# curioloop/rafting

Hardware: AMD Instinct MI355X
Metric: raft-group decisions/sec (AppendEntries+vote) (higher is better)
Workload: dtype int64

## Files before the change

include/raftgpu.h:

```cpp
#ifndef RAFTGPU_H
#define RAFTGPU_H

#include <stdint.h>
#include <stddef.h>

#ifdef __cplusplus
extern "C" {
#endif

#define RG_ABI_VERSION      6
#define RG_MIN_CLUSTER      2
#define RG_MAX_CLUSTER      15
#define RG_MAX_COMPACT_CLUSTER 7
#define RG_TERM_RUNS        4
#define RG_NO_NODE          (-1)

enum { RG_FOLLOWER = 0, RG_CANDIDATE = 1, RG_LEADER = 2 };

enum {
    RG_EV_NONE          = 0,
    RG_EV_AE_REQ        = 1,
    RG_EV_AE_ACK        = 2,
    RG_EV_IS_ACK        = 3,
    RG_EV_RV_REQ        = 4,
    RG_EV_PV_REQ        = 5,
    RG_EV_RV_REPLY      = 6,
    RG_EV_PV_REPLY      = 7,
    RG_EV_TIMEOUT       = 8,
    RG_EV_CLIENT_APPEND = 9,
    RG_EV_LOG_FLUSH     = 10,
    RG_EV_IS_REQ        = 11
};
#define RG_EV_IS_REQ_DEFINED 1

#define RG_HDR_KIND(h)        ((uint32_t)(h) & 0xFu)
#define RG_HDR_SLOT(h)        (((uint32_t)(h) >> 4) & 0xFu)
#define RG_HDR_FLAG(h)        (((uint32_t)(h) >> 8) & 0x1u)
#define RG_HDR_HINT(h)        (((uint32_t)(h) >> 9) & 0x1u)
#define RG_HDR_N(h)           ((uint32_t)(h) >> 12)
#define RG_HDR_MAKE(kind, slot, flag, n) \
    (((uint32_t)(kind) & 0xFu) | (((uint32_t)(slot) & 0xFu) << 4) | (((uint32_t)(flag) & 1u) << 8) | ((uint32_t)(n) << 12))
#define RG_HDR_HINT_BIT       (1u << 9)
#define RG_HDR_SAME_TERM      (1u << 10)
#define RG_MAX_ENTRIES        ((1u << 20) - 1)
#define RG_MAX_AE_ENTRIES     200u

typedef struct { uint32_t hdr; uint32_t aux; } rg_ev_head_t;
typedef struct { int64_t  x;   int64_t  y;   } rg_ev_pair_t;

typedef struct {
    int64_t  resp_term;
    uint32_t flags;
    uint32_t role_epoch;
} rg_reply_t;

typedef struct {
    int64_t commit_index;
    int64_t log_from;
} rg_logfx_t;

typedef struct {
    int64_t term;
    int32_t voted_for;
    int32_t role;
} rg_persist_t;

#define RG_F_SUCCESS      (1u << 0)
#define RG_F_REPLIED      (1u << 1)
#define RG_F_PERSIST      (1u << 2)
#define RG_F_ROLE_CHANGED (1u << 3)
#define RG_F_RESET_TIMER  (1u << 4)
#define RG_F_COMMIT       (1u << 5)
#define RG_F_LOG_TRUNC    (1u << 6)
#define RG_F_LOG_APPEND   (1u << 7)
#define RG_F_EMIT_SHIFT   8
#define RG_F_EMIT_MASK    (3u << 8)
#define RG_EMIT_NONE      0u
#define RG_EMIT_PREVOTE   1u
#define RG_EMIT_REQVOTE   2u
#define RG_EMIT_HEARTBEAT 3u
#define RG_F_ROLE_SHIFT   10
#define RG_F_ROLE_MASK    (3u << 10)
#define RG_F_TIMER_MUTED  (1u << 12)
#define RG_F_WIDE_VALUES  (1u << 13)
#define RG_F_STATUS_SHIFT 16
#define RG_F_STATUS(f)    (((f) >> RG_F_STATUS_SHIFT) & 0xFFu)
#define RG_F_EMIT(f)      (((f) & RG_F_EMIT_MASK) >> RG_F_EMIT_SHIFT)
#define RG_F_ROLE(f)      (((f) & RG_F_ROLE_MASK) >> RG_F_ROLE_SHIFT)

enum {
    RG_OK                       = 0,
    RG_A_TWO_LEADERS            = 1,
    RG_A_PREV_ZERO_MISMATCH     = 2,
    RG_A_EPOCH_TERM_MISMATCH    = 3,
    RG_A_IMPOSSIBLE_LOG         = 4,
    RG_A_COMMIT_ROLLBACK        = 5,
    RG_A_LOG_NOT_CONTINUOUS     = 6,
    RG_A_LEADER_SELF_AE         = 7,
    RG_A_SAME_TERM_LEADER       = 8,
    RG_A_LEADER_NOT_SELF_VOTE   = 9,
    RG_A_CAND_SELF_RV           = 10,
    RG_A_CAND_NOT_SELF_VOTE     = 11,
    RG_A_LEADER_UNCHANGED       = 12,
    RG_A_CAND_BALLOT            = 13,
    RG_A_MATCH_ROLLBACK         = 14,
    RG_A_IMPOSSIBLE_REPLICATION = 15,
    RG_NPE_MAJOR_NULL           = 16,
    RG_DROPPED_STALE_ROLE       = 17,
    RG_NOT_LEADER               = 18,
    RG_FLUSH_OUT_OF_BOUNDS      = 19,
    RG_A_INSTALL_BEFORE_AE      = 20,
    RG_A_NO_DOWNGRADE           = 21,
    RG_NEED_HOST                = 32,
    RG_SKIPPED_AFTER_NEED_HOST  = 33,
    RG_BAD_EVENT                = 34,
    RG_UNSUPPORTED_LOG_STATE    = 35
};

enum { RG_MEM_HOST = 0, RG_MEM_DEVICE = 1 };

typedef struct {
    uint32_t            rounds;
    uint32_t            count;
    const uint32_t     *gid;
    const rg_ev_head_t *head;
    const rg_ev_pair_t *ab;
    const rg_ev_pair_t *cd;
    const int64_t      *entry_terms;
    uint64_t            entry_count;
    const rg_ev_pair_t *hint;
} rg_batch_t;

typedef struct {
    rg_reply_t   *reply;
    rg_logfx_t   *logfx;
    rg_persist_t *persist;
} rg_outcome_t;

typedef struct {
    int64_t  *current_term;
    int32_t  *voted_for;
    int32_t  *role;
    int32_t  *current_leader;
    uint8_t  *timeout_detected;
    uint8_t  *repl_prepared;
    uint32_t *role_epoch;
    int32_t  *votes;
    uint32_t *elected_epoch;
    int64_t  *elected_term;
    int64_t  *commit_index;
    int64_t  *epoch_index;
    int64_t  *epoch_term;
    int64_t  *first_index;
    int64_t  *last_index;
    uint32_t *run_count;
    uint32_t *run_offset;
    int64_t  *run_start;
    int64_t  *run_term;
    int64_t  *peer_last_epoch;
    int64_t  *peer_next_index;
    int64_t  *peer_match_index;
    int32_t  *peer_rejection;
    uint8_t  *peer_pending;
} rg_group_state_t;

typedef struct rg_table rg_table_t;

int         rg_abi_version(void);
int         rg_table_create(int device, uint32_t groups, uint32_t cluster, uint32_t self_slot,
                            int pre_vote, rg_table_t **out);
int         rg_table_destroy(rg_table_t *t);
const char *rg_last_error(const rg_table_t *t);
enum { RG_OPT_REQUIRE_FENCED_TIMEOUTS = 1,
       RG_OPT_AUTO_INDEX_BASE = 2,
       RG_OPT_COMPACT_ANY_CLUSTER = 3,
       RG_OPT_DEVICE_IN_FLIGHT = 4 };
int         rg_table_option(rg_table_t *t, int option, int value);
uint32_t    rg_table_groups(const rg_table_t *t);
uint32_t    rg_table_cluster(const rg_table_t *t);

int rg_load_state(rg_table_t *t, uint32_t first, uint32_t count, const rg_group_state_t *src);
int rg_read_state(rg_table_t *t, uint32_t first, uint32_t count, rg_group_state_t *dst);

int rg_submit(rg_table_t *t, const rg_batch_t *in, const rg_outcome_t *out, int memspace);
int rg_sync(rg_table_t *t);

#define RG_PIPELINE_DEPTH 2
int rg_submit_async(rg_table_t *t, const rg_batch_t *in, const rg_outcome_t *out);
int rg_submit_wait(rg_table_t *t);

typedef struct { int32_t a, b, c, d; } rg_ev_quad32_t;
typedef struct {
    uint32_t              rounds, count;
    const uint32_t       *gid;
    const rg_ev_head_t   *head;
    const rg_ev_quad32_t *abcd;
    const int32_t        *entry_terms;
    uint64_t              entry_count;
} rg_batch32_t;
typedef struct {
    rg_reply_t   *reply;
    rg_logfx_t   *logfx;
    rg_persist_t *persist;
    uint32_t     *counts;
    uint32_t      logfx_cap, persist_cap;
} rg_outcome_packed_t;
int rg_submit_async_packed(rg_table_t *t, const rg_batch32_t *in, const rg_outcome_packed_t *out);

typedef struct rg_tick rg_tick_t;
int rg_tick_create(rg_table_t *t, const rg_batch32_t *in, const rg_outcome_packed_t *out, rg_tick_t **tick);
int rg_tick_launch(rg_tick_t *tick);
int rg_tick_wait(rg_tick_t *tick);
int rg_tick_destroy(rg_tick_t *tick);

int rg_submit32(rg_table_t *t, const rg_batch32_t *in, const rg_outcome_t *out, int memspace);
int64_t rg_batch32_pack(const rg_batch_t *in, rg_ev_head_t *head, rg_ev_quad32_t *abcd, int32_t *entry_terms);

int rg_index_base_set(rg_table_t *t, uint32_t first, uint32_t count, const int64_t *base);
int rg_index_base_get(rg_table_t *t, uint32_t first, uint32_t count, int64_t *base);
int rg_index_base_advance(const rg_batch_t *in, int32_t window, uint32_t groups, int64_t *index_base);
int rg_index_base_advance32(const rg_batch32_t *in, int32_t window, uint32_t groups, int64_t *index_base);
int64_t rg_batch32_pack_rel(const rg_batch_t *in, const int64_t *index_base, rg_ev_head_t *head, rg_ev_quad32_t *abcd, int32_t *entry_terms);
typedef struct { int32_t resp_term; uint32_t flags; int32_t commit_index; int32_t log_from; } rg_out32_t;
typedef struct { int32_t term; int32_t voted_for; uint32_t role_epoch; int32_t role; } rg_persist32_t;
typedef struct {
    rg_out32_t     *row;
    rg_persist32_t *persist;
    rg_outcome_t    wide;
} rg_outcome32_t;
int rg_submit32c(rg_table_t *t, const rg_batch32_t *in, const rg_outcome32_t *out, int memspace);
int rg_submit32c_sparse(rg_table_t *t, const rg_batch32_t *in, const rg_outcome32_t *out, int memspace);
int rg_submit32c_sparse_rounds(rg_table_t *t, const rg_batch32_t *in, const rg_outcome32_t *out, int memspace);
int rg_outcome32_unpack(const rg_outcome32_t *in, uint32_t rounds, uint32_t count, uint32_t *role_epoch, const rg_outcome_t *out);
int rg_outcome32_unpack_rel(const rg_outcome32_t *in, uint32_t rounds, uint32_t count, uint32_t *role_epoch, const int64_t *index_base, const rg_outcome_t *out);
const char *rg_step_kernel(rg_table_t *t, uint32_t count);

enum {
    RG_SEND_NONE      = 0,
    RG_SEND_APPEND    = 1,
    RG_SEND_SNAPSHOT  = 2,
    RG_SEND_GATED     = 3,
    RG_SEND_NEED_HOST = 4
};
#define RG_REPLICATE_LIMIT 50
#define RG_IN_FLIGHT_LIMIT 20

typedef struct {
    int64_t  term;
    int64_t  leader_commit;
    int64_t  epoch_index;
    int64_t  epoch_term;
    uint32_t role_epoch;
    uint32_t is_leader;
    uint64_t reserved;
} rg_send_head_t;

#define RG_SENT_TRIGGERED  1u
#define RG_SENT_HEARTBEAT  2u

typedef struct {
    int64_t  prev_index;
    int64_t  prev_term;
    int64_t  last_index;
    uint32_t count;
    uint32_t kind;
} rg_send_t;

int rg_replicate(rg_table_t *t, uint32_t count, const uint32_t *gid, const uint8_t *heartbeat, const uint16_t *in_flight,
                 rg_send_head_t *head, rg_send_t *send, int memspace);

int rg_timers_configure(rg_table_t *t, int64_t election_ms, int64_t heartbeat_ms, uint64_t seed);
int rg_timers_update(rg_table_t *t, uint32_t rounds, uint32_t count, const uint32_t *gid, const rg_reply_t *reply,
                     const int64_t *now, int memspace);
int rg_timers_expired(rg_table_t *t, int64_t now, uint32_t *out_gid, uint32_t capacity, uint32_t *out_count, int memspace);
int rg_timers_expired_epochs(rg_table_t *t, int64_t now, uint32_t *out_gid, uint32_t *out_epoch, uint32_t capacity, uint32_t *out_count,
                             int memspace);
int rg_timers_update32(rg_table_t *t, uint32_t rounds, const rg_out32_t *row, const rg_persist32_t *persist32, const int64_t *now, int memspace);
int rg_timers_arm(rg_table_t *t, int64_t now);
int rg_timers_read(rg_table_t *t, uint32_t first, uint32_t count, int64_t *deadline);

int rg_health_update(rg_table_t *t, uint32_t rounds, uint32_t count, const uint32_t *gid, const rg_ev_head_t *head,
                     const rg_reply_t *reply, const int64_t *now, int memspace);
int rg_health_update32(rg_table_t *t, uint32_t rounds, const rg_ev_head_t *head, const rg_out32_t *row, const int64_t *now, int memspace);
#define RG_HEALTH_NO_REQUEST 4u
int rg_health_failure(rg_table_t *t, uint32_t n, const uint32_t *gid, const uint8_t *slot, const uint8_t *flags, int64_t now);
int rg_ready(rg_table_t *t, int64_t now, int32_t critical_point, int64_t cool_down_ms, uint8_t *ready, int memspace);
int rg_health_read(rg_table_t *t, uint32_t first, uint32_t count, int64_t *request_success, int64_t *request_failure,
                   int32_t *recent_failure);
int rg_in_flight_read(rg_table_t *t, uint32_t first, uint32_t count, uint16_t *in_flight);
int rg_in_flight_set(rg_table_t *t, uint32_t first, uint32_t count, const uint16_t *in_flight);

typedef struct {
    uint32_t              rounds;
    const rg_ev_head_t   *head;
    const rg_ev_quad32_t *abcd;
    const int32_t        *entry_terms;
    uint64_t              entry_capacity;
    const int64_t        *now;
    const uint8_t        *heartbeat;
    const uint16_t       *in_flight;
    int32_t               critical_point;
    int64_t               cool_down_ms;
    rg_out32_t           *row;
    rg_persist32_t       *persist32;
    uint32_t             *expired_gid;
    uint32_t             *expired_epoch;
    uint32_t             *expired_count;
    uint32_t              expired_capacity;
    rg_send_head_t       *send_head;
    rg_send_t            *send;
    uint8_t              *ready;
} rg_tick2_io_t;
typedef struct rg_tick2 rg_tick2_t;
int rg_tick2_create(rg_table_t *t, const rg_tick2_io_t *io, rg_tick2_t **tick);
typedef struct {
    const uint32_t *gid;
    const uint32_t *count;
    uint32_t        capacity;
} rg_tick2_rows_t;
int rg_tick2_create_sparse(rg_table_t *t, const rg_tick2_io_t *io, const rg_tick2_rows_t *rows, rg_tick2_t **tick);
typedef struct {
    const uint32_t *gid;
    const uint32_t *count;
    const uint32_t *rounds;
    uint32_t        capacity;
} rg_tick2_rounds_t;
int rg_tick2_create_sparse_rounds(rg_table_t *t, const rg_tick2_io_t *io, const rg_tick2_rounds_t *rows, rg_tick2_t **tick);
int rg_tick2_launch(rg_tick2_t *tick);
int rg_tick2_wait(rg_tick2_t *tick);
int rg_tick2_destroy(rg_tick2_t *tick);

typedef struct {
    const uint32_t       *count;
    uint32_t              capacity;
    const uint32_t       *gid;
    const rg_ev_head_t   *head;
    const rg_ev_quad32_t *abcd;
    const uint32_t       *expired_gid, *expired_epoch, *expired_count;
    uint32_t              expired_capacity;
} rg_arrivals_t;
typedef struct {
    uint32_t        capacity;
    uint32_t        max_rounds;
    uint32_t       *gid, *count, *rounds;
    rg_ev_head_t   *head;
    rg_ev_quad32_t *abcd;
    uint32_t       *origin;
    uint32_t       *deferred;
    uint32_t        deferred_capacity;
    uint32_t       *stats;
} rg_assembled_t;
typedef struct rg_assembler rg_assembler_t;
int rg_assembler_create(rg_table_t *t, uint32_t max_events, uint32_t max_expired, rg_assembler_t **a);
int rg_assemble32(rg_assembler_t *a, const rg_arrivals_t *in, const rg_assembled_t *out, int memspace);
int rg_assembler_destroy(rg_assembler_t *a);

int rg_host_alloc(rg_table_t *t, size_t bytes, void **hptr);
int rg_host_free(rg_table_t *t, void *hptr);
int rg_dev_alloc(rg_table_t *t, size_t bytes, void **dptr);
int rg_dev_free(rg_table_t *t, void *dptr);
int rg_copy_to_device(rg_table_t *t, void *dst, const void *src, size_t bytes);
int rg_copy_to_host(rg_table_t *t, void *dst, const void *src, size_t bytes);
void *rg_stream(rg_table_t *t);

int rg_timing_enable(rg_table_t *t, int on);
int rg_timing_read(rg_table_t *t, uint64_t *launches, double *total_ms, int reset);
int rg_timing_begin(rg_table_t *t);
int rg_timing_end(rg_table_t *t, double *elapsed_ms);
#define RG_NUM_COUNTERS 8
int rg_counters_read(rg_table_t *t, uint64_t counters[RG_NUM_COUNTERS], int reset);
int rg_wide_body_workgroups(rg_table_t *t, uint64_t *count, int reset);
int rg_copy_bandwidth(rg_table_t *t, size_t bytes, int iters, double *gbps);

#ifdef __cplusplus
}
#endif
#endif
```

rafting_amd/abi.py:

```python
import ctypes as C

import numpy as np

ABI_VERSION = 6
MIN_CLUSTER, MAX_CLUSTER, MAX_COMPACT_CLUSTER = 2, 15, 7
TERM_RUNS = 4
NO_NODE = -1

FOLLOWER, CANDIDATE, LEADER = 0, 1, 2

EV_NONE, EV_AE_REQ, EV_AE_ACK, EV_IS_ACK, EV_RV_REQ, EV_PV_REQ = 0, 1, 2, 3, 4, 5
EV_RV_REPLY, EV_PV_REPLY, EV_TIMEOUT, EV_CLIENT_APPEND, EV_LOG_FLUSH, EV_IS_REQ = 6, 7, 8, 9, 10, 11
MAX_AE_ENTRIES = 200
PIPELINE_DEPTH = 2
HDR_HINT_BIT = 1 << 9
HDR_SAME_TERM = 1 << 10

F_SUCCESS, F_REPLIED, F_PERSIST, F_ROLE_CHANGED = 1 << 0, 1 << 1, 1 << 2, 1 << 3
F_RESET_TIMER, F_COMMIT, F_LOG_TRUNC, F_LOG_APPEND = 1 << 4, 1 << 5, 1 << 6, 1 << 7
F_EMIT_SHIFT, F_EMIT_MASK = 8, 3 << 8
EMIT_NONE, EMIT_PREVOTE, EMIT_REQVOTE, EMIT_HEARTBEAT = 0, 1, 2, 3
F_ROLE_SHIFT, F_ROLE_MASK = 10, 3 << 10
F_TIMER_MUTED = 1 << 12
F_WIDE_VALUES = 1 << 13
F_STATUS_SHIFT = 16

OK = 0
A_TWO_LEADERS, A_PREV_ZERO_MISMATCH, A_EPOCH_TERM_MISMATCH, A_IMPOSSIBLE_LOG = 1, 2, 3, 4
A_COMMIT_ROLLBACK, A_LOG_NOT_CONTINUOUS, A_LEADER_SELF_AE, A_SAME_TERM_LEADER = 5, 6, 7, 8
A_LEADER_NOT_SELF_VOTE, A_CAND_SELF_RV, A_CAND_NOT_SELF_VOTE, A_LEADER_UNCHANGED = 9, 10, 11, 12
A_CAND_BALLOT, A_MATCH_ROLLBACK, A_IMPOSSIBLE_REPLICATION, NPE_MAJOR_NULL = 13, 14, 15, 16
DROPPED_STALE_ROLE, NOT_LEADER, FLUSH_OUT_OF_BOUNDS = 17, 18, 19
A_INSTALL_BEFORE_AE, A_NO_DOWNGRADE = 20, 21
NEED_HOST, SKIPPED_AFTER_NEED_HOST, BAD_EVENT, UNSUPPORTED_LOG_STATE = 32, 33, 34, 35

MEM_HOST, MEM_DEVICE = 0, 1
OPT_REQUIRE_FENCED_TIMEOUTS = 1
OPT_AUTO_INDEX_BASE = 2
OPT_COMPACT_ANY_CLUSTER = 3
OPT_DEVICE_IN_FLIGHT = 4
SENT_TRIGGERED, SENT_HEARTBEAT = 1, 2
HEALTH_UNREACHABLE, HEALTH_REJECT, HEALTH_NO_REQUEST = 1, 2, 4
NUM_COUNTERS = 8

HEAD_DT = np.dtype([("hdr", "<u4"), ("aux", "<u4")])
PAIR_DT = np.dtype([("x", "<i8"), ("y", "<i8")])
REPLY_DT = np.dtype([("resp_term", "<i8"), ("flags", "<u4"), ("role_epoch", "<u4")])
LOGFX_DT = np.dtype([("commit_index", "<i8"), ("log_from", "<i8")])
PERSIST_DT = np.dtype([("term", "<i8"), ("voted_for", "<i4"), ("role", "<i4")])
SEND_HEAD_DT = np.dtype([("term", "<i8"), ("leader_commit", "<i8"), ("epoch_index", "<i8"), ("epoch_term", "<i8"),
                         ("role_epoch", "<u4"), ("is_leader", "<u4"), ("reserved", "<u8")])
SEND_DT = np.dtype([("prev_index", "<i8"), ("prev_term", "<i8"), ("last_index", "<i8"), ("count", "<u4"), ("kind", "<u4")])
SEND_NONE, SEND_APPEND, SEND_SNAPSHOT, SEND_GATED, SEND_NEED_HOST = 0, 1, 2, 3, 4
REPLICATE_LIMIT, IN_FLIGHT_LIMIT = 50, 20
assert SEND_HEAD_DT.itemsize == 48 and SEND_DT.itemsize == 32
assert HEAD_DT.itemsize == 8 and PAIR_DT.itemsize == 16 and REPLY_DT.itemsize == 16
assert LOGFX_DT.itemsize == 16 and PERSIST_DT.itemsize == 16


def hdr_make(kind, slot=0, flag=0, n=0):
    return (
        (np.uint32(kind) & np.uint32(0xF))
        | ((np.asarray(slot).astype(np.uint32) & np.uint32(0xF)) << np.uint32(4))
        | ((np.asarray(flag).astype(np.uint32) & np.uint32(1)) << np.uint32(8))
        | (np.asarray(n).astype(np.uint32) << np.uint32(12))
    ).astype(np.uint32)


def flags_status(flags):
    return (np.asarray(flags) >> F_STATUS_SHIFT) & 0xFF


def flags_role(flags):
    return (np.asarray(flags) & F_ROLE_MASK) >> F_ROLE_SHIFT


def flags_emit(flags):
    return (np.asarray(flags) & F_EMIT_MASK) >> F_EMIT_SHIFT


class CBatch(C.Structure):
    _fields_ = [
        ("rounds", C.c_uint32),
        ("count", C.c_uint32),
        ("gid", C.c_void_p),
        ("head", C.c_void_p),
        ("ab", C.c_void_p),
        ("cd", C.c_void_p),
        ("entry_terms", C.c_void_p),
        ("entry_count", C.c_uint64),
        ("hint", C.c_void_p),
    ]


class COutcome(C.Structure):
    _fields_ = [("reply", C.c_void_p), ("logfx", C.c_void_p), ("persist", C.c_void_p)]


class CBatch32(C.Structure):
    _fields_ = [("rounds", C.c_uint32), ("count", C.c_uint32), ("gid", C.c_void_p), ("head", C.c_void_p), ("abcd", C.c_void_p),
                ("entry_terms", C.c_void_p), ("entry_count", C.c_uint64)]


class COutcome32(C.Structure):
    _fields_ = [("row", C.c_void_p), ("persist", C.c_void_p), ("wide", COutcome)]


class COutcomePacked(C.Structure):
    _fields_ = [("reply", C.c_void_p), ("logfx", C.c_void_p), ("persist", C.c_void_p), ("counts", C.c_void_p),
                ("logfx_cap", C.c_uint32), ("persist_cap", C.c_uint32)]


class CTick2Io(C.Structure):
    _fields_ = [("rounds", C.c_uint32), ("head", C.c_void_p), ("abcd", C.c_void_p), ("entry_terms", C.c_void_p), ("entry_capacity", C.c_uint64),
                ("now", C.c_void_p), ("heartbeat", C.c_void_p), ("in_flight", C.c_void_p), ("critical_point", C.c_int32), ("cool_down_ms", C.c_int64),
                ("row", C.c_void_p), ("persist32", C.c_void_p), ("expired_gid", C.c_void_p), ("expired_epoch", C.c_void_p), ("expired_count", C.c_void_p),
                ("expired_capacity", C.c_uint32), ("send_head", C.c_void_p), ("send", C.c_void_p), ("ready", C.c_void_p)]


class CTick2Rows(C.Structure):
    _fields_ = [("gid", C.c_void_p), ("count", C.c_void_p), ("capacity", C.c_uint32)]


class CTick2Rounds(C.Structure):
    _fields_ = [("gid", C.c_void_p), ("count", C.c_void_p), ("rounds", C.c_void_p), ("capacity", C.c_uint32)]


class CArrivals(C.Structure):
    _fields_ = [("count", C.c_void_p), ("capacity", C.c_uint32), ("gid", C.c_void_p), ("head", C.c_void_p), ("abcd", C.c_void_p),
                ("expired_gid", C.c_void_p), ("expired_epoch", C.c_void_p), ("expired_count", C.c_void_p), ("expired_capacity", C.c_uint32)]


class CAssembled(C.Structure):
    _fields_ = [("capacity", C.c_uint32), ("max_rounds", C.c_uint32), ("gid", C.c_void_p), ("count", C.c_void_p), ("rounds", C.c_void_p),
                ("head", C.c_void_p), ("abcd", C.c_void_p), ("origin", C.c_void_p), ("deferred", C.c_void_p), ("deferred_capacity", C.c_uint32),
                ("stats", C.c_void_p)]


ORIGIN_NONE, ORIGIN_EXPIRED = 0xFFFFFFFF, 0x80000000
EXPIRED_UNTRUSTED = 0xFFFFFFFF


_STATE_FIELDS = [
    ("current_term", np.int64, 1),
    ("voted_for", np.int32, 1),
    ("role", np.int32, 1),
    ("current_leader", np.int32, 1),
    ("timeout_detected", np.uint8, 1),
    ("repl_prepared", np.uint8, 1),
    ("role_epoch", np.uint32, 1),
    ("votes", np.int32, 1),
    ("elected_epoch", np.uint32, 1),
    ("elected_term", np.int64, 1),
    ("commit_index", np.int64, 1),
    ("epoch_index", np.int64, 1),
    ("epoch_term", np.int64, 1),
    ("first_index", np.int64, 1),
    ("last_index", np.int64, 1),
    ("run_count", np.uint32, 1),
    ("run_offset", np.uint32, 1),
    ("run_start", np.int64, "runs"),
    ("run_term", np.int64, "runs"),
    ("peer_last_epoch", np.int64, "peers"),
    ("peer_next_index", np.int64, "peers"),
    ("peer_match_index", np.int64, "peers"),
    ("peer_rejection", np.int32, "peers"),
    ("peer_pending", np.uint8, "peers"),
]


class CGroupState(C.Structure):
    _fields_ = [(name, C.c_void_p) for name, _, _ in _STATE_FIELDS]


def _ptr(a):
    return None if a is None else a.ctypes.data


class GroupState:

    def __init__(self, count, cluster, runs_total=None):
        self.count, self.cluster, self.followers = count, cluster, cluster - 1
        nruns = count * TERM_RUNS if runs_total is None else runs_total
        for name, dt, shape in _STATE_FIELDS:
            n = count if shape == 1 else (nruns if shape == "runs" else count * self.followers)
            setattr(self, name, np.zeros(n, dtype=dt))
        self.voted_for[:] = NO_NODE
        self.current_leader[:] = NO_NODE
        self.role_epoch[:] = 1
        self.votes[:] = 1
        self.run_offset[:] = np.arange(count, dtype=np.uint32) * TERM_RUNS if runs_total is None else 0

    def set_log(self, g, first, runs, last):
# ... 157 lines not shown
```

rafting_amd/csrc/raftgpu.cpp:

```cpp
#include <hip/hip_runtime.h>

#include <algorithm>
#include <cstdarg>
#include <cstdint>
#include <cstdio>
#include <cstdlib>
#include <cstring>
#include <string>
#include <unordered_map>
#include <vector>

#include "rg_device.hpp"
#include "rg_assemble.hpp"

using rg::DevTable;
using rg::I64x2;

struct Staging {
    void *ptr = nullptr;
    size_t cap = 0;
};

struct PipeSlot {
    Staging gid, head, ab, cd, hint, terms, reply, logfx, persist;
    Staging abcd32, terms32, counts;
    hipEvent_t up = nullptr, done = nullptr, down = nullptr;
};

struct rg_table {
    int device = 0;
    uint32_t G = 0, P = 0, self = 0, F = 0;
    int pre_vote = 0;
    hipStream_t stream = nullptr;
    DevTable dt{};
    unsigned long long *counters = nullptr;
    unsigned long long *wide_bodies = nullptr;
    size_t counter_slots = 0;
    int fast_paths = 1;
    int force_wide = 0;
    int require_fence = 0;
    int has_bases = 0;
    int auto_window = 0;
    int compact_any_cluster = 0;
    Staging st_abcd32, st_terms32, st_out32, st_persist32;
    int lanes = -1;
    uint32_t simds = 1024;
    Staging st_gid, st_head, st_ab, st_cd, st_hint, st_terms, st_reply, st_logfx, st_persist, st_hb, st_fl, st_sh, st_ss;
    bool timing = false;
    std::vector<std::pair<hipEvent_t, hipEvent_t>> ev_pool;
    size_t ev_used = 0;
    uint64_t t_launches = 0;
    double t_total_ms = 0.0;
    hipEvent_t region0 = nullptr, region1 = nullptr;
    int64_t *timer_deadline = nullptr;
    uint32_t *timer_epoch = nullptr;
    unsigned long long *tick_masks = nullptr;
    uint32_t *tick_ticket = nullptr;
    uint64_t config_gen = 0;
    std::vector<struct rg_tick *> ticks;
    std::vector<struct rg_tick2 *> ticks2;
    std::vector<struct rg_assembler *> assemblers;
    uint32_t *timer_counts = nullptr;
    int64_t election_ms = 900, heartbeat_ms = 300;
    uint64_t timer_seed = 0;
    Staging st_tgid, st_hgid, st_hslot, st_hflag, st_ready;
    int64_t *health_ok = nullptr, *health_fail = nullptr;
    int32_t *health_recent = nullptr;
    uint16_t *in_flight = nullptr;
    Staging st_hdone;
    hipStream_t s_in = nullptr, s_out = nullptr;
    PipeSlot pipe[RG_PIPELINE_DEPTH];
    uint64_t pipe_head = 0, pipe_tail = 0;
    std::string err;
};

static thread_local std::string g_create_err;

static int fail(rg_table *t, int code, const char *fmt, ...)
{
    char buf[512];
    va_list ap;
    va_start(ap, fmt);
    vsnprintf(buf, sizeof buf, fmt, ap);
    va_end(ap);
    if (t) t->err = buf; else g_create_err = buf;
    return code;
}

#define HIP_TRY(t, expr)                                                                              \
    do {                                                                                              \
        hipError_t e_ = (expr);                                                                       \
        if (e_ != hipSuccess) return fail((t), -2, "%s failed: %s", #expr, hipGetErrorString(e_));    \
    } while (0)

static int wait_oldest(rg_table *t)
{
    if (t->pipe_tail == t->pipe_head) return 1;
    HIP_TRY(t, hipEventSynchronize(t->pipe[t->pipe_tail % RG_PIPELINE_DEPTH].down));
    t->pipe_tail += 1;
    return 0;
}

static int bind(rg_table *t, bool drain = true)
{
    HIP_TRY(t, hipSetDevice(t->device));
    while (drain && t->pipe_tail != t->pipe_head)
        if (int rc = wait_oldest(t); rc < 0) return rc;
    return 0;
}

static int reserve(rg_table *t, Staging &s, size_t bytes)
{
    if (bytes <= s.cap) return 0;
    if (s.ptr) HIP_TRY(t, hipFree(s.ptr));
    s.ptr = nullptr; s.cap = 0;
    size_t cap = bytes + bytes / 4 + 4096;
    HIP_TRY(t, hipMalloc(&s.ptr, cap));
    s.cap = cap;
    return 0;
}

static int drain_timing(rg_table *t)
{
    if (t->ev_used == 0) return 0;
    HIP_TRY(t, hipStreamSynchronize(t->stream));
    for (size_t i = 0; i < t->ev_used; i++) {
        float ms = 0.f;
        HIP_TRY(t, hipEventElapsedTime(&ms, t->ev_pool[i].first, t->ev_pool[i].second));
        t->t_total_ms += ms;
        t->t_launches += 1;
    }
    t->ev_used = 0;
    return 0;
}

extern "C" {

int rg_abi_version(void) { return RG_ABI_VERSION; }

const char *rg_last_error(const rg_table_t *t) { return t ? t->err.c_str() : g_create_err.c_str(); }
uint32_t rg_table_groups(const rg_table_t *t) { return t ? t->G : 0; }
uint32_t rg_table_cluster(const rg_table_t *t) { return t ? t->P : 0; }

int rg_table_option(rg_table_t *t, int option, int value)
{
    if (!t) return -1;
    switch (option) {
    case RG_OPT_REQUIRE_FENCED_TIMEOUTS:
        if (t->require_fence != (value != 0)) t->config_gen += 1;
        t->require_fence = value != 0;
        return 0;
    case RG_OPT_AUTO_INDEX_BASE:
        if (value < 0 || value >= (1 << 30)) return fail(t, -1, "rg_table_option: RG_OPT_AUTO_INDEX_BASE window %d outside [0, 2^30)", value);
        if (t->auto_window != value) t->config_gen += 1;
        if (value != 0 && !t->has_bases) t->has_bases = 1;
        t->auto_window = value;
        return 0;
    case RG_OPT_COMPACT_ANY_CLUSTER:
        if (value != 0 && value != 1) return fail(t, -1, "rg_table_option: RG_OPT_COMPACT_ANY_CLUSTER takes 0 or 1 (%d given)", value);
        if (t->compact_any_cluster != value) t->config_gen += 1;
        t->compact_any_cluster = value;
        return 0;
    case RG_OPT_DEVICE_IN_FLIGHT: {
        if (value != 0 && value != 1) return fail(t, -1, "rg_table_option: RG_OPT_DEVICE_IN_FLIGHT takes 0 or 1 (%d given)", value);
        if ((t->in_flight != nullptr) == (value == 1)) return 0;
        if (bind(t)) return -2;
        HIP_TRY(t, hipStreamSynchronize(t->stream));
        if (value == 1) {
            const size_t bytes = (size_t)t->G * t->F * sizeof(uint16_t);
            uint16_t *c = nullptr;
            HIP_TRY(t, hipMalloc((void **)&c, bytes));
            if (hipError_t e = hipMemsetAsync(c, 0, bytes, t->stream); e != hipSuccess || (e = hipStreamSynchronize(t->stream)) != hipSuccess) {
                (void)hipFree(c);
                return fail(t, -2, "rg_table_option: RG_OPT_DEVICE_IN_FLIGHT: %s", hipGetErrorString(e));
            }
            t->in_flight = c;
        } else {
            HIP_TRY(t, hipFree(t->in_flight));
            t->in_flight = nullptr;
        }
        t->config_gen += 1;
        return 0;
    }
    default: return fail(t, -1, "rg_table_option: unknown option %d", option);
    }
}

static void tick_release(struct rg_tick *k);
static void tick2_release(struct rg_tick2 *k);
static void assembler_release(struct rg_assembler *a);

int rg_table_destroy(rg_table_t *t)
{
    if (!t) return 0;
    (void)hipSetDevice(t->device);
    if (t->stream) (void)hipStreamSynchronize(t->stream);
    for (struct rg_tick *k : t->ticks) tick_release(k);
    for (struct rg_tick2 *k : t->ticks2) tick2_release(k);
    for (struct rg_assembler *a : t->assemblers) assembler_release(a);
    t->ticks.clear(); t->ticks2.clear(); t->assemblers.clear();
    void *cols[] = {t->dt.term_commit, t->dt.epoch, t->dt.window, t->dt.ident, t->dt.elect, t->dt.runs,
                    t->dt.peer_en, t->dt.peer_m, t->dt.ibase, t->wide_bodies, t->counters, t->st_gid.ptr, t->st_head.ptr, t->st_ab.ptr,
                    t->st_cd.ptr, t->st_hint.ptr, t->st_terms.ptr, t->st_reply.ptr, t->st_logfx.ptr,
                    t->st_persist.ptr, t->st_hb.ptr, t->st_fl.ptr, t->st_sh.ptr, t->st_ss.ptr, t->timer_deadline, t->timer_epoch, t->tick_masks, t->tick_ticket,
                    t->timer_counts, t->st_tgid.ptr, t->st_hgid.ptr, t->st_hslot.ptr, t->st_hflag.ptr, t->st_ready.ptr, t->health_ok,
                    t->health_fail, t->health_recent, t->in_flight, t->st_hdone.ptr, t->st_abcd32.ptr, t->st_terms32.ptr, t->st_out32.ptr, t->st_persist32.ptr};
    for (void *c : cols) if (c) (void)hipFree(c);
    for (PipeSlot &sl : t->pipe) {
        if (sl.down) (void)hipEventSynchronize(sl.down);
        for (Staging *st : {&sl.gid, &sl.head, &sl.ab, &sl.cd, &sl.hint, &sl.terms, &sl.reply, &sl.logfx, &sl.persist, &sl.abcd32, &sl.terms32, &sl.counts})
            if (st->ptr) (void)hipFree(st->ptr);
        for (hipEvent_t ev : {sl.up, sl.done, sl.down}) if (ev) (void)hipEventDestroy(ev);
    }
    if (t->s_in) (void)hipStreamDestroy(t->s_in);
    if (t->s_out) (void)hipStreamDestroy(t->s_out);
    for (auto &e : t->ev_pool) { (void)hipEventDestroy(e.first); (void)hipEventDestroy(e.second); }
    if (t->region0) { (void)hipEventDestroy(t->region0); (void)hipEventDestroy(t->region1); }
    if (t->stream) (void)hipStreamDestroy(t->stream);
    delete t;
    return 0;
}

int rg_table_create(int device, uint32_t groups, uint32_t cluster, uint32_t self_slot, int pre_vote, rg_table_t **out)
{
    if (!out) return fail(nullptr, -1, "rg_table_create: out is NULL");
    *out = nullptr;
    if (groups == 0) return fail(nullptr, -1, "rg_table_create: groups must be > 0");
    if (cluster < RG_MIN_CLUSTER || cluster > RG_MAX_CLUSTER)
        return fail(nullptr, -1, "rg_table_create: cluster size %u outside [%d, %d]", cluster, RG_MIN_CLUSTER, RG_MAX_CLUSTER);
    if (self_slot >= cluster) return fail(nullptr, -1, "rg_table_create: self_slot %u >= cluster %u", self_slot, cluster);
    int ndev = 0;
    hipError_t e = hipGetDeviceCount(&ndev);
    if (e != hipSuccess || ndev == 0)
        return fail(nullptr, -2, "rg_table_create: no HIP device (%s) — libraftgpu has no CPU path", hipGetErrorString(e));
    if (device < 0 || device >= ndev) return fail(nullptr, -1, "rg_table_create: device %d of %d", device, ndev);

    rg_table *t = new rg_table();
    t->device = device; t->G = groups; t->P = cluster; t->self = self_slot; t->F = cluster - 1;
    t->pre_vote = pre_vote != 0;
#define CREATE_TRY(expr)                                                                   \
    do {                                                                                   \
        hipError_t e2_ = (expr);                                                           \
        if (e2_ != hipSuccess) {                                                           \
            fail(nullptr, -2, "%s failed: %s", #expr, hipGetErrorString(e2_));             \
            rg_table_destroy(t);                                                           \
            return -2;                                                                     \
        }                                                                                  \
    } while (0)
    CREATE_TRY(hipSetDevice(device));
    CREATE_TRY(hipStreamCreateWithFlags(&t->stream, hipStreamNonBlocking));
    const size_t G = groups, F = t->F;
    CREATE_TRY(hipMalloc((void **)&t->dt.term_commit, G * sizeof(I64x2)));
    CREATE_TRY(hipMalloc((void **)&t->dt.epoch, G * sizeof(I64x2)));
    CREATE_TRY(hipMalloc((void **)&t->dt.window, G * sizeof(I64x2)));
    CREATE_TRY(hipMalloc((void **)&t->dt.ident, G * sizeof(rg::Ident)));
    CREATE_TRY(hipMalloc((void **)&t->dt.elect, G * sizeof(rg::Elect)));
    CREATE_TRY(hipMalloc((void **)&t->dt.runs, G * rg::K * sizeof(I64x2)));
    CREATE_TRY(hipMalloc((void **)&t->dt.peer_en, G * F * sizeof(I64x2)));
    CREATE_TRY(hipMalloc((void **)&t->dt.peer_m, G * F * sizeof(rg::Match)));
    CREATE_TRY(hipMalloc((void **)&t->dt.ibase, G * sizeof(int64_t)));
    CREATE_TRY(hipMalloc((void **)&t->wide_bodies, sizeof(unsigned long long)));
    CREATE_TRY(hipMemsetAsync(t->wide_bodies, 0, sizeof(unsigned long long), t->stream));
    {
        hipDeviceProp_t prop;
        CREATE_TRY(hipGetDeviceProperties(&prop, device));
        t->simds = (uint32_t)prop.multiProcessorCount * 4u;
    }
    t->lanes = -1;
    if (const char *e = getenv("RG_SPLIT")) t->lanes = atoi(e) != 0 ? 0 : 64;
    if (const char *e = getenv("RG_FAST")) t->fast_paths = atoi(e) != 0;
    if (const char *e = getenv("RG_FORCE_WIDE")) t->force_wide = atoi(e) != 0;
    t->counter_slots = (G + 63) / 64 + 1;
    CREATE_TRY(hipMalloc((void **)&t->counters, t->counter_slots * RG_NUM_COUNTERS * sizeof(unsigned long long)));
    t->dt.groups = groups;
    CREATE_TRY(hipMalloc((void **)&t->timer_deadline, G * sizeof(int64_t)));
    CREATE_TRY(hipMalloc((void **)&t->timer_counts, ((G + 255) / 256 * 4 + 1) * sizeof(uint32_t)));
    CREATE_TRY(hipMemsetAsync(t->timer_deadline, 0, G * sizeof(int64_t), t->stream));
    CREATE_TRY(hipMalloc((void **)&t->tick_masks, ((G + 255) / 256 * 4) * sizeof(unsigned long long)));
    CREATE_TRY(hipMemsetAsync(t->tick_masks, 0, ((G + 255) / 256 * 4) * sizeof(unsigned long long), t->stream));
    CREATE_TRY(hipMalloc((void **)&t->tick_ticket, sizeof(uint32_t)));
    CREATE_TRY(hipMemsetAsync(t->tick_ticket, 0, sizeof(uint32_t), t->stream));
    CREATE_TRY(hipMalloc((void **)&t->timer_epoch, G * sizeof(uint32_t)));
    CREATE_TRY(hipMemsetAsync(t->timer_epoch, 0, G * sizeof(uint32_t), t->stream));
    CREATE_TRY(hipMalloc((void **)&t->health_ok, G * F * sizeof(int64_t)));
    CREATE_TRY(hipMalloc((void **)&t->health_fail, G * F * sizeof(int64_t)));
    CREATE_TRY(hipMalloc((void **)&t->health_recent, G * F * sizeof(int32_t)));
    CREATE_TRY(hipMemsetAsync(t->health_ok, 0, G * F * sizeof(int64_t), t->stream));
    CREATE_TRY(hipMemsetAsync(t->health_fail, 0, G * F * sizeof(int64_t), t->stream));
    CREATE_TRY(hipMemsetAsync(t->health_recent, 0, G * F * sizeof(int32_t), t->stream));
    CREATE_TRY(hipMemsetAsync(t->dt.term_commit, 0, G * sizeof(I64x2), t->stream));
    CREATE_TRY(hipMemsetAsync(t->dt.epoch, 0, G * sizeof(I64x2), t->stream));
    CREATE_TRY(hipMemsetAsync(t->dt.window, 0, G * sizeof(I64x2), t->stream));
    CREATE_TRY(hipMemsetAsync(t->dt.runs, 0, G * rg::K * sizeof(I64x2), t->stream));
    CREATE_TRY(hipMemsetAsync(t->dt.peer_en, 0, G * F * sizeof(I64x2), t->stream));
    CREATE_TRY(hipMemsetAsync(t->dt.peer_m, 0, G * F * sizeof(rg::Match), t->stream));
    CREATE_TRY(hipMemsetAsync(t->dt.ibase, 0, G * sizeof(int64_t), t->stream));
    CREATE_TRY(hipMemsetAsync(t->counters, 0, t->counter_slots * RG_NUM_COUNTERS * sizeof(unsigned long long), t->stream));
    {
        std::vector<rg::Ident> id(G, rg::Ident{RG_NO_NODE, RG_NO_NODE, 1u, 0u});
        std::vector<rg::Elect> el(G, rg::Elect{0, 0u, 1});
        CREATE_TRY(hipMemcpyAsync(t->dt.ident, id.data(), G * sizeof(rg::Ident), hipMemcpyHostToDevice, t->stream));
        CREATE_TRY(hipMemcpyAsync(t->dt.elect, el.data(), G * sizeof(rg::Elect), hipMemcpyHostToDevice, t->stream));
        CREATE_TRY(hipStreamSynchronize(t->stream));
    }
#undef CREATE_TRY
    *out = t;
    return 0;
}


static int step_lanes(const rg_table *t, uint32_t count)
{
    if (t->lanes >= 0) return t->lanes;
    const uint32_t wavefronts = (count + 63u) / 64u;
    return wavefronts <= t->simds ? 0 : 64;
}

static bool state_complete(const rg_group_state_t *s)
{
    return s->current_term && s->voted_for && s->role && s->current_leader && s->timeout_detected && s->repl_prepared &&
           s->role_epoch && s->votes && s->elected_epoch && s->elected_term && s->commit_index && s->epoch_index &&
           s->epoch_term && s->first_index && s->last_index && s->run_count && s->run_offset && s->run_start && s->run_term &&
           s->peer_last_epoch && s->peer_next_index && s->peer_match_index && s->peer_rejection && s->peer_pending;
}

int rg_load_state(rg_table_t *t, uint32_t first, uint32_t count, const rg_group_state_t *s)
{
    if (!t) return -1;
    if (!s || !state_complete(s)) return fail(t, -1, "rg_load_state: src or one of its columns is NULL");
    if ((uint64_t)first + count > t->G) return fail(t, -1, "rg_load_state: range [%u, %u) exceeds %u groups", first, first + count, t->G);
    if (count == 0) return 0;
    if (bind(t)) return -2;
    const size_t n = count, F = t->F, G = t->G;
    std::vector<I64x2> tc(n), ep(n), win(n), runs(n * rg::K), en(n * F);
    std::vector<rg::Ident> id(n);
    std::vector<rg::Elect> el(n);
    std::vector<rg::Match> pm(n * F);
    for (size_t i = 0; i < n; i++) {
        const int32_t role = s->role[i];
        if (role < RG_FOLLOWER || role > RG_LEADER) return fail(t, -1, "rg_load_state: group %zu role %d", first + i, role);
        if (s->voted_for[i] < RG_NO_NODE || s->voted_for[i] >= (int32_t)t->P || s->current_leader[i] < RG_NO_NODE ||
            s->current_leader[i] >= (int32_t)t->P)
            return fail(t, -1, "rg_load_state: group %zu node slot out of range", first + i);
        const uint32_t total = s->run_count[i], off = s->run_offset[i];
        const uint32_t rc = total > (uint32_t)rg::K ? (uint32_t)rg::K : total;
        int64_t fi = 0, la = 0;
        if (total) {
            fi = s->first_index[i]; la = s->last_index[i];
            if (s->run_start[off] != fi || la < s->run_start[off + total - 1])
                return fail(t, -1, "rg_load_state: group %zu runs do not span [first,last]", first + i);
            if (fi != s->epoch_index[i] && fi != s->epoch_index[i] + 1)
                return fail(t, -1, "rg_load_state: group %zu first index %lld is neither epoch.index nor epoch.index+1",
                            first + i, (long long)fi);
            for (uint32_t k = 1; k < total; k++)
                if (s->run_start[off + k] <= s->run_start[off + k - 1] || s->run_term[off + k] == s->run_term[off + k - 1])
                    return fail(t, -1, "rg_load_state: group %zu runs are not maximal ascending runs", first + i);
        }
        tc[i] = I64x2{s->current_term[i], s->commit_index[i]};
        ep[i] = I64x2{s->epoch_index[i], s->epoch_term[i]};
        win[i] = I64x2{fi, la};
        uint32_t pend = 0;
        for (size_t j = 0; j < F; j++) {
            en[j * n + i] = I64x2{s->peer_last_epoch[i * F + j], s->peer_next_index[i * F + j]};
            pm[j * n + i] = rg::Match{s->peer_match_index[i * F + j], s->peer_rejection[i * F + j], 0};
            if (s->peer_pending[i * F + j]) pend |= 1u << j;
        }
        for (uint32_t k = 0; k < (uint32_t)rg::K; k++) {
            const bool have = k < rc;
            runs[(size_t)k * n + i] = have ? I64x2{s->run_start[off + total - rc + k], s->run_term[off + total - rc + k]} : I64x2{0, 0};
        }
        const uint32_t meta = (uint32_t)role | (s->timeout_detected[i] ? rg::META_TD : 0u) |
                              (s->repl_prepared[i] ? rg::META_PREP : 0u) | (rc << rg::META_RC_SHIFT) |
                              (pend << rg::META_PEND_SHIFT);
        id[i] = rg::Ident{s->voted_for[i], s->current_leader[i], s->role_epoch[i], meta};
        el[i] = rg::Elect{s->elected_term[i], s->elected_epoch[i], s->votes[i]};
    }
    hipStream_t st = t->stream;
    HIP_TRY(t, hipMemcpyAsync(t->dt.term_commit + first, tc.data(), n * sizeof(I64x2), hipMemcpyHostToDevice, st));
    HIP_TRY(t, hipMemcpyAsync(t->dt.epoch + first, ep.data(), n * sizeof(I64x2), hipMemcpyHostToDevice, st));
    HIP_TRY(t, hipMemcpyAsync(t->dt.window + first, win.data(), n * sizeof(I64x2), hipMemcpyHostToDevice, st));
    HIP_TRY(t, hipMemcpyAsync(t->dt.ident + first, id.data(), n * sizeof(rg::Ident), hipMemcpyHostToDevice, st));
    HIP_TRY(t, hipMemcpyAsync(t->dt.elect + first, el.data(), n * sizeof(rg::Elect), hipMemcpyHostToDevice, st));
    for (size_t k = 0; k < (size_t)rg::K; k++)
        HIP_TRY(t, hipMemcpyAsync(t->dt.runs + k * G + first, runs.data() + k * n, n * sizeof(I64x2), hipMemcpyHostToDevice, st));
    for (size_t j = 0; j < F; j++) {
        HIP_TRY(t, hipMemcpyAsync(t->dt.peer_en + j * G + first, en.data() + j * n, n * sizeof(I64x2), hipMemcpyHostToDevice, st));
        HIP_TRY(t, hipMemcpyAsync(t->dt.peer_m + j * G + first, pm.data() + j * n, n * sizeof(rg::Match), hipMemcpyHostToDevice, st));
    }
    HIP_TRY(t, hipMemsetAsync(t->timer_deadline + first, 0, n * sizeof(int64_t), st));
    HIP_TRY(t, hipMemcpyAsync(t->timer_epoch + first, s->role_epoch, n * sizeof(uint32_t), hipMemcpyHostToDevice, st));
    for (size_t j = 0; j < F; j++) {
        HIP_TRY(t, hipMemsetAsync(t->health_ok + j * G + first, 0, n * sizeof(int64_t), st));
        HIP_TRY(t, hipMemsetAsync(t->health_fail + j * G + first, 0, n * sizeof(int64_t), st));
        HIP_TRY(t, hipMemsetAsync(t->health_recent + j * G + first, 0, n * sizeof(int32_t), st));
        if (t->in_flight) HIP_TRY(t, hipMemsetAsync(t->in_flight + j * G + first, 0, n * sizeof(uint16_t), st));
    }
    HIP_TRY(t, hipStreamSynchronize(st));
    return 0;
}

int rg_read_state(rg_table_t *t, uint32_t first, uint32_t count, rg_group_state_t *d)
{
    if (!t) return -1;
    if (!d || !state_complete(d)) return fail(t, -1, "rg_read_state: dst or one of its columns is NULL");
    if ((uint64_t)first + count > t->G) return fail(t, -1, "rg_read_state: range exceeds %u groups", t->G);
    if (count == 0) return 0;
    if (bind(t)) return -2;
    const size_t n = count, F = t->F, G = t->G;
    std::vector<I64x2> tc(n), ep(n), win(n), runs(n * rg::K), en(n * F);
    std::vector<rg::Ident> id(n);
    std::vector<rg::Elect> el(n);
    std::vector<rg::Match> pm(n * F);
    hipStream_t st = t->stream;
    HIP_TRY(t, hipMemcpyAsync(tc.data(), t->dt.term_commit + first, n * sizeof(I64x2), hipMemcpyDeviceToHost, st));
    HIP_TRY(t, hipMemcpyAsync(ep.data(), t->dt.epoch + first, n * sizeof(I64x2), hipMemcpyDeviceToHost, st));
    HIP_TRY(t, hipMemcpyAsync(win.data(), t->dt.window + first, n * sizeof(I64x2), hipMemcpyDeviceToHost, st));
    HIP_TRY(t, hipMemcpyAsync(id.data(), t->dt.ident + first, n * sizeof(rg::Ident), hipMemcpyDeviceToHost, st));
    HIP_TRY(t, hipMemcpyAsync(el.data(), t->dt.elect + first, n * sizeof(rg::Elect), hipMemcpyDeviceToHost, st));
    for (size_t k = 0; k < (size_t)rg::K; k++)
        HIP_TRY(t, hipMemcpyAsync(runs.data() + k * n, t->dt.runs + k * G + first, n * sizeof(I64x2), hipMemcpyDeviceToHost, st));
    for (size_t j = 0; j < F; j++) {
        HIP_TRY(t, hipMemcpyAsync(en.data() + j * n, t->dt.peer_en + j * G + first, n * sizeof(I64x2), hipMemcpyDeviceToHost, st));
        HIP_TRY(t, hipMemcpyAsync(pm.data() + j * n, t->dt.peer_m + j * G + first, n * sizeof(rg::Match), hipMemcpyDeviceToHost, st));
    }
    HIP_TRY(t, hipStreamSynchronize(st));
    for (size_t i = 0; i < n; i++) {
        const uint32_t meta = id[i].meta;
        const uint32_t rc = (meta >> rg::META_RC_SHIFT) & 7u;
        d->current_term[i] = tc[i].x; d->commit_index[i] = tc[i].y;
        d->epoch_index[i] = ep[i].x; d->epoch_term[i] = ep[i].y;
        d->first_index[i] = rc ? win[i].x : 0; d->last_index[i] = rc ? win[i].y : 0;
        d->voted_for[i] = id[i].voted_for; d->current_leader[i] = id[i].leader; d->role_epoch[i] = id[i].role_epoch;
        d->role[i] = (int32_t)(meta & rg::META_ROLE);
        d->timeout_detected[i] = (meta & rg::META_TD) ? 1 : 0;
        d->repl_prepared[i] = (meta & rg::META_PREP) ? 1 : 0;
        d->elected_term[i] = el[i].elected_term; d->elected_epoch[i] = el[i].elected_epoch; d->votes[i] = el[i].votes;
        d->run_count[i] = rc;
        d->run_offset[i] = (uint32_t)(i * rg::K);
        for (uint32_t k = 0; k < (uint32_t)rg::K; k++) {
            d->run_start[i * rg::K + k] = k < rc ? runs[(size_t)k * n + i].x : 0;
            d->run_term[i * rg::K + k] = k < rc ? runs[(size_t)k * n + i].y : 0;
        }
        const uint32_t pend = (meta >> rg::META_PEND_SHIFT) & rg::META_PEND_MASK;
        for (size_t j = 0; j < F; j++) {
            d->peer_last_epoch[i * F + j] = en[j * n + i].x;
            d->peer_next_index[i * F + j] = en[j * n + i].y;
            d->peer_match_index[i * F + j] = pm[j * n + i].match_index;
            d->peer_rejection[i * F + j] = pm[j * n + i].rejection;
            d->peer_pending[i * F + j] = (pend >> j) & 1u;
        }
// ... 749 lines not shown
    p.reply = (rg_reply_t *)t->st_reply.ptr; p.logfx = (I64x2 *)t->st_logfx.ptr; p.persist = (rg_persist_t *)t->st_persist.ptr;
    HIP_TRY(t, hipMemsetAsync(t->st_logfx.ptr, 0, rows * sizeof(I64x2), s));
    HIP_TRY(t, hipMemsetAsync(t->st_persist.ptr, 0, rows * sizeof(rg_persist_t), s));
    if (int rc = launch(t, p, sparse)) return rc;
    HIP_TRY(t, hipMemcpyAsync(out->reply, t->st_reply.ptr, rows * sizeof(rg_reply_t), hipMemcpyDeviceToHost, s));
    HIP_TRY(t, hipMemcpyAsync(out->logfx, t->st_logfx.ptr, rows * sizeof(I64x2), hipMemcpyDeviceToHost, s));
    HIP_TRY(t, hipMemcpyAsync(out->persist, t->st_persist.ptr, rows * sizeof(rg_persist_t), hipMemcpyDeviceToHost, s));
    HIP_TRY(t, hipStreamSynchronize(s));
    return 0;
}

int rg_submit32(rg_table_t *t, const rg_batch32_t *in, const rg_outcome_t *out, int memspace)
{
    if (!t) return -1;
    if (int rc = compact_ok(t, "rg_submit32")) return rc;
    if (!in || !out) return fail(t, -1, "rg_submit32: NULL batch or outcome");
    if (!in->head || !in->abcd) return fail(t, -1, "rg_submit32: head and abcd are required");
    rg_batch_t wide{};
    wide.rounds = in->rounds; wide.count = in->count; wide.gid = in->gid; wide.head = in->head;
    wide.ab = wide.cd = reinterpret_cast<const rg_ev_pair_t *>(in->abcd);
    wide.entry_terms = reinterpret_cast<const int64_t *>(in->entry_terms); wide.entry_count = in->entry_count;
    if (int rc = check_batch(t, &wide, out, memspace == RG_MEM_HOST)) return rc;
    if (in->count == 0) return 0;
    if (bind(t)) return -2;
    const bool sparse = in->gid != nullptr;
    const size_t rows = (size_t)in->rounds * in->count;
    rg::StepParams p = step_params(t, &wide);
    if (memspace == RG_MEM_DEVICE) {
        p.gid = in->gid; p.head = in->head; p.abcd32 = (const rg::I32x4 *)in->abcd;
        p.entry_terms32 = in->entry_count ? in->entry_terms : nullptr;
        p.reply = out->reply; p.logfx = (I64x2 *)out->logfx; p.persist = out->persist;
        return launch(t, p, sparse);
    }
    if (memspace != RG_MEM_HOST) return fail(t, -1, "rg_submit32: unknown memspace %d", memspace);
    hipStream_t s = t->stream;
    if (reserve(t, t->st_head, rows * sizeof(rg_ev_head_t)) || reserve(t, t->st_abcd32, rows * sizeof(rg_ev_quad32_t)) ||
        reserve(t, t->st_reply, rows * sizeof(rg_reply_t)) || reserve(t, t->st_logfx, rows * sizeof(I64x2)) ||
        reserve(t, t->st_persist, rows * sizeof(rg_persist_t)))
        return -2;
    HIP_TRY(t, hipMemcpyAsync(t->st_head.ptr, in->head, rows * sizeof(rg_ev_head_t), hipMemcpyHostToDevice, s));
    HIP_TRY(t, hipMemcpyAsync(t->st_abcd32.ptr, in->abcd, rows * sizeof(rg_ev_quad32_t), hipMemcpyHostToDevice, s));
    p.head = (const rg_ev_head_t *)t->st_head.ptr; p.abcd32 = (const rg::I32x4 *)t->st_abcd32.ptr;
    if (sparse) {
        if (reserve(t, t->st_gid, in->count * sizeof(uint32_t))) return -2;
        HIP_TRY(t, hipMemcpyAsync(t->st_gid.ptr, in->gid, in->count * sizeof(uint32_t), hipMemcpyHostToDevice, s));
        p.gid = (const uint32_t *)t->st_gid.ptr;
    }
    if (in->entry_count) {
        if (reserve(t, t->st_terms32, in->entry_count * sizeof(int32_t))) return -2;
        HIP_TRY(t, hipMemcpyAsync(t->st_terms32.ptr, in->entry_terms, in->entry_count * sizeof(int32_t), hipMemcpyHostToDevice, s));
        p.entry_terms32 = (const int32_t *)t->st_terms32.ptr;
    }
    p.reply = (rg_reply_t *)t->st_reply.ptr; p.logfx = (I64x2 *)t->st_logfx.ptr; p.persist = (rg_persist_t *)t->st_persist.ptr;
    HIP_TRY(t, hipMemsetAsync(t->st_logfx.ptr, 0, rows * sizeof(I64x2), s));
    HIP_TRY(t, hipMemsetAsync(t->st_persist.ptr, 0, rows * sizeof(rg_persist_t), s));
    if (int rc = launch(t, p, sparse)) return rc;
    HIP_TRY(t, hipMemcpyAsync(out->reply, t->st_reply.ptr, rows * sizeof(rg_reply_t), hipMemcpyDeviceToHost, s));
    HIP_TRY(t, hipMemcpyAsync(out->logfx, t->st_logfx.ptr, rows * sizeof(I64x2), hipMemcpyDeviceToHost, s));
    HIP_TRY(t, hipMemcpyAsync(out->persist, t->st_persist.ptr, rows * sizeof(rg_persist_t), hipMemcpyDeviceToHost, s));
    HIP_TRY(t, hipStreamSynchronize(s));
    return 0;
}

int rg_wide_body_workgroups(rg_table_t *t, uint64_t *count, int reset)
{
    if (!t || !count) return -1;
    if (bind(t)) return -2;
    unsigned long long v = 0;
    HIP_TRY(t, hipMemcpyAsync(&v, t->wide_bodies, sizeof v, hipMemcpyDeviceToHost, t->stream));
    if (reset) HIP_TRY(t, hipMemsetAsync(t->wide_bodies, 0, sizeof v, t->stream));
    HIP_TRY(t, hipStreamSynchronize(t->stream));
    *count = v;
    return 0;
}

int rg_index_base_set(rg_table_t *t, uint32_t first, uint32_t count, const int64_t *base)
{
    if (!t) return -1;
    if (!base) return fail(t, -1, "rg_index_base_set: NULL base");
    if ((uint64_t)first + count > t->G) return fail(t, -1, "rg_index_base_set: groups [%u, %u) of %u", first, first + count, t->G);
    for (uint32_t i = 0; i < count; i++)
        if (base[i] < 0) return fail(t, -1, "rg_index_base_set: base[%u] = %lld is negative", i, (long long)base[i]);
    for (uint32_t i = 0; i < count; i++)
        if (base[i] != 0 && !t->has_bases) { t->has_bases = 1; t->config_gen += 1; }
    if (count == 0) return 0;
    if (bind(t)) return -2;
    HIP_TRY(t, hipMemcpyAsync(t->dt.ibase + first, base, (size_t)count * sizeof(int64_t), hipMemcpyHostToDevice, t->stream));
    HIP_TRY(t, hipStreamSynchronize(t->stream));
    return 0;
}

int rg_index_base_get(rg_table_t *t, uint32_t first, uint32_t count, int64_t *base)
{
    if (!t) return -1;
    if (!base) return fail(t, -1, "rg_index_base_get: NULL base");
    if ((uint64_t)first + count > t->G) return fail(t, -1, "rg_index_base_get: groups [%u, %u) of %u", first, first + count, t->G);
    if (count == 0) return 0;
    if (bind(t)) return -2;
    HIP_TRY(t, hipMemcpyAsync(base, t->dt.ibase + first, (size_t)count * sizeof(int64_t), hipMemcpyDeviceToHost, t->stream));
    HIP_TRY(t, hipStreamSynchronize(t->stream));
    return 0;
}

extern "C++" template <class Flush>
int advance_bases(uint32_t rounds, uint32_t count, const uint32_t *gid, const rg_ev_head_t *head, int32_t window, uint32_t groups, int64_t *index_base,
                         Flush flush)
{
    if (!head || !index_base || window < 1 || window >= (1 << 30)) return -1;
    if (gid ? count > groups : count != groups) return -2;
    if (gid)
        for (uint32_t i = 0; i < count; i++)
            if (gid[i] >= groups) return -2;
    std::vector<int64_t> top(gid ? count : groups, 0);
    for (uint32_t r = 0; r < rounds; r++)
        for (uint32_t i = 0; i < count; i++) {
            const size_t row = (size_t)r * count + i;
            if (RG_HDR_KIND(head[row].hdr) != RG_EV_LOG_FLUSH) continue;
            const int64_t a = flush(row, gid ? gid[i] : i);
            if (a > top[i]) top[i] = a;
        }
    for (uint32_t i = 0; i < (uint32_t)top.size(); i++) {
        int64_t &base = index_base[gid ? gid[i] : i];
        if (top[i] - window > base) base = top[i] - window;
    }
    return 0;
}

int rg_index_base_advance(const rg_batch_t *in, int32_t window, uint32_t groups, int64_t *index_base)
{
    if (!in || !in->ab) return -1;
    return advance_bases(in->rounds, in->count, in->gid, in->head, window, groups, index_base, [&](size_t row, uint32_t) { return (int64_t)in->ab[row].x; });
}

int rg_index_base_advance32(const rg_batch32_t *in, int32_t window, uint32_t groups, int64_t *index_base)
{
    if (!in || !in->abcd) return -1;
    return advance_bases(in->rounds, in->count, in->gid, in->head, window, groups, index_base, [&](size_t row, uint32_t g) {
        const int32_t a = in->abcd[row].a;
        return a <= 0 ? (int64_t)0 : (int64_t)a + index_base[g];
    });
}

static uint32_t host_index_fields(uint32_t kind)
{
    switch (kind) {
    case RG_EV_AE_REQ: return 0xAu;
    case RG_EV_AE_ACK: return 0x6u;
    case RG_EV_IS_ACK: case RG_EV_RV_REQ: case RG_EV_PV_REQ: case RG_EV_IS_REQ: return 0x2u;
    case RG_EV_LOG_FLUSH: return 0x1u;
    default: return 0u;
    }
}

static int submit32c(rg_table_t *t, const rg_batch32_t *in, const rg_outcome32_t *out, int memspace, bool sparse, const char *who, bool list_rounds = false)
{
    if (!t) return -1;
    if (int rc = compact_ok(t, who)) return rc;
    if (!in || !out) return fail(t, -1, "%s: NULL batch or outcome", who);
    if (!in->head || !in->abcd || !out->row || !out->persist) return fail(t, -1, "%s: head, abcd, row and persist are required", who);
    if (!sparse && in->gid) return fail(t, -1, "rg_submit32c: dense batches only (gid must be NULL); a list of groups goes through rg_submit32c_sparse");
    if (sparse && !in->gid) return fail(t, -1, "%s: gid is required (dense batches go through rg_submit32c)", who);
    const int wides = (out->wide.reply != nullptr) + (out->wide.logfx != nullptr) + (out->wide.persist != nullptr);
    if (wides != 0 && wides != 3) return fail(t, -1, "%s: the overflow columns come as all three or none", who);
    rg_batch_t wide{};
    wide.rounds = in->rounds; wide.count = in->count; wide.gid = in->gid; wide.head = in->head;
    wide.ab = wide.cd = reinterpret_cast<const rg_ev_pair_t *>(in->abcd);
    wide.entry_terms = reinterpret_cast<const int64_t *>(in->entry_terms); wide.entry_count = in->entry_count;
    rg_reply_t dummy_r; rg_logfx_t dummy_l; rg_persist_t dummy_p;
    const rg_outcome_t shape{&dummy_r, &dummy_l, &dummy_p};
    if (int rc = check_batch(t, &wide, &shape, memspace == RG_MEM_HOST, list_rounds)) return rc;
    if (in->count == 0) return 0;
    if (bind(t)) return -2;
    const size_t rows = (size_t)in->rounds * in->count;
    rg::StepParams p = step_params(t, &wide);
    if (memspace == RG_MEM_DEVICE) {
        p.gid = in->gid; p.head = in->head; p.abcd32 = (const rg::I32x4 *)in->abcd;
        p.entry_terms32 = in->entry_count ? in->entry_terms : nullptr;
        p.out32 = (rg::I32x4 *)out->row; p.persist32 = (rg::I32x4 *)out->persist;
        p.reply = out->wide.reply; p.logfx = (I64x2 *)out->wide.logfx; p.persist = out->wide.persist;
        return launch(t, p, sparse);
    }
    if (memspace != RG_MEM_HOST) return fail(t, -1, "%s: unknown memspace %d", who, memspace);
    hipStream_t s = t->stream;
    if (reserve(t, t->st_head, rows * sizeof(rg_ev_head_t)) || reserve(t, t->st_abcd32, rows * sizeof(rg_ev_quad32_t)) ||
        reserve(t, t->st_out32, rows * sizeof(rg_out32_t)) || reserve(t, t->st_persist32, rows * sizeof(rg_persist32_t)))
        return -2;
    if (wides && (reserve(t, t->st_reply, rows * sizeof(rg_reply_t)) || reserve(t, t->st_logfx, rows * sizeof(I64x2)) ||
                  reserve(t, t->st_persist, rows * sizeof(rg_persist_t))))
        return -2;
    HIP_TRY(t, hipMemcpyAsync(t->st_head.ptr, in->head, rows * sizeof(rg_ev_head_t), hipMemcpyHostToDevice, s));
    HIP_TRY(t, hipMemcpyAsync(t->st_abcd32.ptr, in->abcd, rows * sizeof(rg_ev_quad32_t), hipMemcpyHostToDevice, s));
    p.head = (const rg_ev_head_t *)t->st_head.ptr; p.abcd32 = (const rg::I32x4 *)t->st_abcd32.ptr;
    if (sparse) {
        if (reserve(t, t->st_gid, in->count * sizeof(uint32_t))) return -2;
        HIP_TRY(t, hipMemcpyAsync(t->st_gid.ptr, in->gid, in->count * sizeof(uint32_t), hipMemcpyHostToDevice, s));
        p.gid = (const uint32_t *)t->st_gid.ptr;
    }
    if (in->entry_count) {
        if (reserve(t, t->st_terms32, in->entry_count * sizeof(int32_t))) return -2;
        HIP_TRY(t, hipMemcpyAsync(t->st_terms32.ptr, in->entry_terms, in->entry_count * sizeof(int32_t), hipMemcpyHostToDevice, s));
        p.entry_terms32 = (const int32_t *)t->st_terms32.ptr;
    }
    p.out32 = (rg::I32x4 *)t->st_out32.ptr; p.persist32 = (rg::I32x4 *)t->st_persist32.ptr;
    HIP_TRY(t, hipMemsetAsync(t->st_persist32.ptr, 0, rows * sizeof(rg_persist32_t), s));
    if (wides) {
        p.reply = (rg_reply_t *)t->st_reply.ptr; p.logfx = (I64x2 *)t->st_logfx.ptr; p.persist = (rg_persist_t *)t->st_persist.ptr;
        HIP_TRY(t, hipMemsetAsync(t->st_reply.ptr, 0, rows * sizeof(rg_reply_t), s));
        HIP_TRY(t, hipMemsetAsync(t->st_logfx.ptr, 0, rows * sizeof(I64x2), s));
        HIP_TRY(t, hipMemsetAsync(t->st_persist.ptr, 0, rows * sizeof(rg_persist_t), s));
    }
    if (int rc = launch(t, p, sparse)) return rc;
    HIP_TRY(t, hipMemcpyAsync(out->row, t->st_out32.ptr, rows * sizeof(rg_out32_t), hipMemcpyDeviceToHost, s));
    HIP_TRY(t, hipMemcpyAsync(out->persist, t->st_persist32.ptr, rows * sizeof(rg_persist32_t), hipMemcpyDeviceToHost, s));
    if (wides) {
        HIP_TRY(t, hipMemcpyAsync(out->wide.reply, t->st_reply.ptr, rows * sizeof(rg_reply_t), hipMemcpyDeviceToHost, s));
        HIP_TRY(t, hipMemcpyAsync(out->wide.logfx, t->st_logfx.ptr, rows * sizeof(I64x2), hipMemcpyDeviceToHost, s));
        HIP_TRY(t, hipMemcpyAsync(out->wide.persist, t->st_persist.ptr, rows * sizeof(rg_persist_t), hipMemcpyDeviceToHost, s));
    }
    HIP_TRY(t, hipStreamSynchronize(s));
    return 0;
}

int rg_submit32c(rg_table_t *t, const rg_batch32_t *in, const rg_outcome32_t *out, int memspace)
{
    return submit32c(t, in, out, memspace, false, "rg_submit32c");
}

int rg_submit32c_sparse(rg_table_t *t, const rg_batch32_t *in, const rg_outcome32_t *out, int memspace)
{
    return submit32c(t, in, out, memspace, true, "rg_submit32c_sparse");
}

int rg_submit32c_sparse_rounds(rg_table_t *t, const rg_batch32_t *in, const rg_outcome32_t *out, int memspace)
{
    return submit32c(t, in, out, memspace, true, "rg_submit32c_sparse_rounds", true);
}

int rg_outcome32_unpack(const rg_outcome32_t *in, uint32_t rounds, uint32_t count, uint32_t *role_epoch, const rg_outcome_t *out)
{
    return rg_outcome32_unpack_rel(in, rounds, count, role_epoch, nullptr, out);
}

int rg_outcome32_unpack_rel(const rg_outcome32_t *in, uint32_t rounds, uint32_t count, uint32_t *role_epoch, const int64_t *index_base, const rg_outcome_t *out)
{
    if (!in || !in->row || !in->persist || !role_epoch || !out || !out->reply || !out->logfx || !out->persist) return -1;
    auto absolute = [&](int32_t v, uint32_t i) { return v == 0 ? (int64_t)0 : (int64_t)v + (index_base ? index_base[i] : 0); };
    for (uint32_t r = 0; r < rounds; r++) {
        for (uint32_t i = 0; i < count; i++) {
            const size_t row = (size_t)r * count + i;
            const rg_out32_t c = in->row[row];
            const uint32_t flags = c.flags & ~RG_F_WIDE_VALUES;
            const bool has_lfx = (flags & (RG_F_COMMIT | RG_F_LOG_APPEND | RG_F_LOG_TRUNC)) != 0 || RG_F_STATUS(flags) == RG_NEED_HOST;
            const bool has_from = (flags & (RG_F_LOG_APPEND | RG_F_LOG_TRUNC)) != 0 || RG_F_STATUS(flags) == RG_NEED_HOST;
            const bool has_per = (flags & RG_F_PERSIST) != 0;
            if (c.flags & RG_F_WIDE_VALUES) {
                if (!in->wide.reply || !in->wide.logfx || !in->wide.persist) return -3;
                out->reply[row] = in->wide.reply[row];
                out->logfx[row] = has_lfx ? in->wide.logfx[row] : rg_logfx_t{0, 0};
                out->persist[row] = has_per ? in->wide.persist[row] : rg_persist_t{0, 0, 0};
                if (out->reply[row].flags != flags) return -4;
                role_epoch[i] = out->reply[row].role_epoch;
                continue;
            }
            if (has_per) role_epoch[i] = in->persist[row].role_epoch;
            out->reply[row] = rg_reply_t{(flags & RG_F_REPLIED) ? (int64_t)c.resp_term : 0, flags, role_epoch[i]};
            out->logfx[row] = has_lfx ? rg_logfx_t{absolute(c.commit_index, i), has_from ? absolute(c.log_from, i) : 0} : rg_logfx_t{0, 0};
            out->persist[row] = has_per ? rg_persist_t{(int64_t)in->persist[row].term, in->persist[row].voted_for, in->persist[row].role}
                                        : rg_persist_t{0, 0, 0};
        }
    }
    return 0;
}

int64_t rg_batch32_pack(const rg_batch_t *in, rg_ev_head_t *head, rg_ev_quad32_t *abcd, int32_t *entry_terms)
{
    return rg_batch32_pack_rel(in, nullptr, head, abcd, entry_terms);
}

int64_t rg_batch32_pack_rel(const rg_batch_t *in, const int64_t *index_base, rg_ev_head_t *head, rg_ev_quad32_t *abcd, int32_t *entry_terms)
{
    if (!in || !in->head || !in->ab || !in->cd || !head || !abcd) return -1;
    if (in->hint) return -2;
    const size_t rows = (size_t)in->rounds * in->count;
    auto fits = [](int64_t v) { return v >= 0 && v < (int64_t)1 << 31; };
    uint64_t out_terms = 0;
    for (size_t r = 0; r < rows; r++) {
        const uint32_t hdr = in->head[r].hdr & ~(RG_HDR_HINT_BIT | RG_HDR_SAME_TERM | (1u << 11)), aux = in->head[r].aux;
        int64_t a = in->ab[r].x, b = in->ab[r].y, c = in->cd[r].x, d = in->cd[r].y;
        if (RG_HDR_KIND(hdr) == RG_EV_NONE) a = b = c = d = 0;
        if (index_base) {
            const size_t i = r % in->count;
            const int64_t base = index_base[in->gid ? in->gid[i] : i];
            const uint32_t ix = host_index_fields(RG_HDR_KIND(hdr));
            int64_t *f[4] = {&a, &b, &c, &d};
            for (int k = 0; k < 4; k++)
                if (((ix >> k) & 1u) && *f[k] != 0) { if (*f[k] <= base) return -3; *f[k] -= base; }
        }
        if (!fits(a) || !fits(b) || !fits(c) || !fits(d)) return -3;
        abcd[r] = rg_ev_quad32_t{(int32_t)a, (int32_t)b, (int32_t)c, (int32_t)d};
        head[r].hdr = hdr; head[r].aux = aux;
        const uint32_t n = RG_HDR_N(hdr);
        if (RG_HDR_KIND(hdr) != RG_EV_AE_REQ || n == 0) continue;
        if (!in->entry_terms || (uint64_t)aux + n > in->entry_count) { head[r].aux = 0xFFFFFFFFu; continue; }
        const int64_t *e = in->entry_terms + aux;
        bool same = true;
        for (uint32_t k = 0; k < n; k++) { if (!fits(e[k])) return -3; same = same && e[k] == e[0]; }
        if (same) {
            head[r].hdr = hdr | RG_HDR_SAME_TERM; head[r].aux = (uint32_t)e[0];
        } else {
            if (!entry_terms) return -4;
            head[r].aux = (uint32_t)out_terms;
            for (uint32_t k = 0; k < n; k++) entry_terms[out_terms + k] = (int32_t)e[k];
            out_terms += n;
        }
    }
    return (int64_t)out_terms;
}

int rg_replicate(rg_table_t *t, uint32_t count, const uint32_t *gid, const uint8_t *heartbeat, const uint16_t *in_flight,
                 rg_send_head_t *head, rg_send_t *send, int memspace)
{
    if (!t) return -1;
    if (!head || !send) return fail(t, -1, "rg_replicate: head and send are required");
    if (gid ? count > t->G : count != t->G) return fail(t, -1, "rg_replicate: %u rows for %u groups", count, t->G);
    if (count == 0) return 0;
    if (bind(t)) return -2;
    rg::ReplicateParams p{};
    p.t = t->dt; p.count = count;
    if (memspace == RG_MEM_DEVICE) {
        p.gid = gid; p.heartbeat = heartbeat; p.in_flight = in_flight; p.head = head; p.send = send;
        HIP_TRY(t, rg::launch_replicate(p, (int)t->F, t->stream));
        return 0;
// ... 269 lines not shown
        if (reserve(t, t->st_hdone, n * sizeof(uint16_t))) return -2;
        HIP_TRY(t, hipMemcpyAsync(t->st_hdone.ptr, done.data(), n * sizeof(uint16_t), hipMemcpyHostToDevice, s));
    }
    HIP_TRY(t, rg::launch_health_failure(p, n, (const uint32_t *)t->st_hgid.ptr, (const uint8_t *)t->st_hslot.ptr,
                                         (const uint8_t *)t->st_hflag.ptr, t->in_flight ? (const uint16_t *)t->st_hdone.ptr : nullptr, s));
    HIP_TRY(t, hipStreamSynchronize(s));
    return 0;
}

int rg_ready(rg_table_t *t, int64_t now, int32_t critical_point, int64_t cool_down_ms, uint8_t *ready, int memspace)
{
    if (!t || !ready) return -1;
    if (bind(t)) return -2;
    hipStream_t s = t->stream;
    uint8_t *d_ready = ready;
    if (memspace == RG_MEM_HOST) {
        if (reserve(t, t->st_ready, t->G)) return -2;
        d_ready = (uint8_t *)t->st_ready.ptr;
    } else if (memspace != RG_MEM_DEVICE) {
        return fail(t, -1, "rg_ready: unknown memspace %d", memspace);
    }
    HIP_TRY(t, rg::launch_ready(health_params(t), now, critical_point, cool_down_ms, d_ready, s));
    if (memspace == RG_MEM_HOST) {
        HIP_TRY(t, hipMemcpyAsync(ready, d_ready, t->G, hipMemcpyDeviceToHost, s));
        HIP_TRY(t, hipStreamSynchronize(s));
    }
    return 0;
}

int rg_health_read(rg_table_t *t, uint32_t first, uint32_t count, int64_t *request_success, int64_t *request_failure,
                   int32_t *recent_failure)
{
    if (!t || !request_success || !request_failure || !recent_failure) return -1;
    if ((uint64_t)first + count > t->G) return fail(t, -1, "rg_health_read: range exceeds %u groups", t->G);
    if (count == 0) return 0;
    if (bind(t)) return -2;
    const size_t n = count, F = t->F, G = t->G;
    std::vector<int64_t> ok(n * F), fl(n * F);
    std::vector<int32_t> rc(n * F);
    for (size_t j = 0; j < F; j++) {
        HIP_TRY(t, hipMemcpyAsync(ok.data() + j * n, t->health_ok + j * G + first, n * sizeof(int64_t), hipMemcpyDeviceToHost, t->stream));
        HIP_TRY(t, hipMemcpyAsync(fl.data() + j * n, t->health_fail + j * G + first, n * sizeof(int64_t), hipMemcpyDeviceToHost, t->stream));
        HIP_TRY(t, hipMemcpyAsync(rc.data() + j * n, t->health_recent + j * G + first, n * sizeof(int32_t), hipMemcpyDeviceToHost, t->stream));
    }
    HIP_TRY(t, hipStreamSynchronize(t->stream));
    for (size_t i = 0; i < n; i++)
        for (size_t j = 0; j < F; j++) {
            request_success[i * F + j] = ok[j * n + i]; request_failure[i * F + j] = fl[j * n + i]; recent_failure[i * F + j] = rc[j * n + i];
        }
    return 0;
}

static int in_flight_copy(rg_table_t *t, uint32_t first, uint32_t count, uint16_t *out, const uint16_t *in, const char *who)
{
    if (!t) return -1;
    if (!t->in_flight) return fail(t, -1, "%s: the table does not keep in-flight counts (rg_table_option RG_OPT_DEVICE_IN_FLIGHT is 0)", who);
    if (!out && !in) return fail(t, -1, "%s: in_flight is NULL", who);
    if ((uint64_t)first + count > t->G) return fail(t, -1, "%s: range exceeds %u groups", who, t->G);
    if (count == 0) return 0;
    if (bind(t)) return -2;
    const size_t n = count, F = t->F, G = t->G;
    std::vector<uint16_t> col(n * F);
    if (in)
        for (size_t i = 0; i < n; i++)
            for (size_t j = 0; j < F; j++) col[j * n + i] = in[i * F + j];
    for (size_t j = 0; j < F; j++) {
        if (in) HIP_TRY(t, hipMemcpyAsync(t->in_flight + j * G + first, col.data() + j * n, n * sizeof(uint16_t), hipMemcpyHostToDevice, t->stream));
        else    HIP_TRY(t, hipMemcpyAsync(col.data() + j * n, t->in_flight + j * G + first, n * sizeof(uint16_t), hipMemcpyDeviceToHost, t->stream));
    }
    HIP_TRY(t, hipStreamSynchronize(t->stream));
    if (out)
        for (size_t i = 0; i < n; i++)
            for (size_t j = 0; j < F; j++) out[i * F + j] = col[j * n + i];
    return 0;
}

int rg_in_flight_read(rg_table_t *t, uint32_t first, uint32_t count, uint16_t *in_flight)
{
    return in_flight_copy(t, first, count, in_flight, nullptr, "rg_in_flight_read");
}

int rg_in_flight_set(rg_table_t *t, uint32_t first, uint32_t count, const uint16_t *in_flight)
{
    return in_flight_copy(t, first, count, nullptr, in_flight, "rg_in_flight_set");
}

const char *rg_step_kernel(rg_table_t *t, uint32_t count)
{
    if (!t) return "";
    return step_lanes(t, count) == 0 ? "rg::step_split_kernel" : "rg::step_kernel";
}

int rg_sync(rg_table_t *t)
{
    if (!t) return -1;
    if (bind(t)) return -2;
    HIP_TRY(t, hipStreamSynchronize(t->stream));
    return 0;
}


int rg_host_alloc(rg_table_t *t, size_t bytes, void **hptr)
{
    if (!t || !hptr) return -1;
    if (bind(t)) return -2;
    HIP_TRY(t, hipHostMalloc(hptr, bytes ? bytes : 16, hipHostMallocDefault));
    return 0;
}

int rg_host_free(rg_table_t *t, void *hptr)
{
    if (!t) return -1;
    if (bind(t)) return -2;
    HIP_TRY(t, hipStreamSynchronize(t->stream));
    HIP_TRY(t, hipHostFree(hptr));
    return 0;
}

int rg_dev_alloc(rg_table_t *t, size_t bytes, void **dptr)
{
    if (!t || !dptr) return -1;
    if (bind(t)) return -2;
    HIP_TRY(t, hipMalloc(dptr, bytes ? bytes : 16));
    return 0;
}

int rg_dev_free(rg_table_t *t, void *dptr)
{
    if (!t) return -1;
    if (bind(t)) return -2;
    HIP_TRY(t, hipStreamSynchronize(t->stream));
    HIP_TRY(t, hipFree(dptr));
    return 0;
}

int rg_copy_to_device(rg_table_t *t, void *dst, const void *src, size_t bytes)
{
    if (!t) return -1;
    if (bind(t)) return -2;
    HIP_TRY(t, hipMemcpyAsync(dst, src, bytes, hipMemcpyHostToDevice, t->stream));
    HIP_TRY(t, hipStreamSynchronize(t->stream));
    return 0;
}

int rg_copy_to_host(rg_table_t *t, void *dst, const void *src, size_t bytes)
{
    if (!t) return -1;
    if (bind(t)) return -2;
    HIP_TRY(t, hipMemcpyAsync(dst, src, bytes, hipMemcpyDeviceToHost, t->stream));
    HIP_TRY(t, hipStreamSynchronize(t->stream));
    return 0;
}

void *rg_stream(rg_table_t *t) { return t ? (void *)t->stream : nullptr; }


int rg_timing_enable(rg_table_t *t, int on)
{
    if (!t) return -1;
    if (bind(t)) return -2;
    if (drain_timing(t)) return -2;
    t->timing = on != 0;
    return 0;
}

int rg_timing_read(rg_table_t *t, uint64_t *launches, double *total_ms, int reset)
{
    if (!t) return -1;
    if (bind(t)) return -2;
    if (drain_timing(t)) return -2;
    if (launches) *launches = t->t_launches;
    if (total_ms) *total_ms = t->t_total_ms;
    if (reset) { t->t_launches = 0; t->t_total_ms = 0.0; }
    return 0;
}

int rg_timing_begin(rg_table_t *t)
{
    if (!t) return -1;
    if (bind(t)) return -2;
    if (!t->region0) { HIP_TRY(t, hipEventCreate(&t->region0)); HIP_TRY(t, hipEventCreate(&t->region1)); }
    HIP_TRY(t, hipEventRecord(t->region0, t->stream));
    return 0;
}

int rg_timing_end(rg_table_t *t, double *elapsed_ms)
{
    if (!t || !elapsed_ms) return -1;
    if (bind(t)) return -2;
    if (!t->region0) return fail(t, -1, "rg_timing_end without rg_timing_begin");
    HIP_TRY(t, hipEventRecord(t->region1, t->stream));
    HIP_TRY(t, hipEventSynchronize(t->region1));
    float ms = 0.f;
    HIP_TRY(t, hipEventElapsedTime(&ms, t->region0, t->region1));
    *elapsed_ms = ms;
    return 0;
}

int rg_counters_read(rg_table_t *t, uint64_t counters[RG_NUM_COUNTERS], int reset)
{
    if (!t || !counters) return -1;
    if (bind(t)) return -2;
    const size_t n = t->counter_slots * RG_NUM_COUNTERS;
    std::vector<unsigned long long> host(n);
    HIP_TRY(t, hipMemcpyAsync(host.data(), t->counters, n * sizeof(unsigned long long), hipMemcpyDeviceToHost, t->stream));
    if (reset) HIP_TRY(t, hipMemsetAsync(t->counters, 0, n * sizeof(unsigned long long), t->stream));
    HIP_TRY(t, hipStreamSynchronize(t->stream));
#ifdef RG_PROBE_HWID
    if (const char *path = getenv("RG_DUMP_COUNTERS")) {
        if (FILE *f = fopen(path, "wb")) { fwrite(host.data(), sizeof(unsigned long long), n, f); fclose(f); }
    }
#endif
    for (int i = 0; i < RG_NUM_COUNTERS; i++) counters[i] = 0;
    for (size_t s = 0; s < t->counter_slots; s++)
        for (int i = 0; i < RG_NUM_COUNTERS; i++) counters[i] += host[s * RG_NUM_COUNTERS + i];
    return 0;
}

int rg_copy_bandwidth(rg_table_t *t, size_t bytes, int iters, double *gbps)
{
    if (!t || !gbps || iters < 1) return -1;
    if (bind(t)) return -2;
    bytes &= ~(size_t)15;
    if (bytes == 0) return fail(t, -1, "rg_copy_bandwidth: bytes must be >= 16");
    void *src = nullptr, *dst = nullptr;
    HIP_TRY(t, hipMalloc(&src, bytes));
    HIP_TRY(t, hipMalloc(&dst, bytes));
    HIP_TRY(t, hipMemsetAsync(src, 1, bytes, t->stream));
    hipEvent_t a, b;
    HIP_TRY(t, hipEventCreate(&a));
    HIP_TRY(t, hipEventCreate(&b));
    HIP_TRY(t, rg::launch_copy(src, dst, bytes, t->stream));
    HIP_TRY(t, hipEventRecord(a, t->stream));
    for (int i = 0; i < iters; i++) HIP_TRY(t, rg::launch_copy(src, dst, bytes, t->stream));
    HIP_TRY(t, hipEventRecord(b, t->stream));
    HIP_TRY(t, hipStreamSynchronize(t->stream));
    float ms = 0.f;
    HIP_TRY(t, hipEventElapsedTime(&ms, a, b));
    *gbps = 2.0 * (double)bytes * iters / ((double)ms * 1e-3) / 1e9;
    (void)hipEventDestroy(a); (void)hipEventDestroy(b);
    (void)hipFree(src); (void)hipFree(dst);
    return 0;
}

}
```

rafting_amd/csrc/rg_device.hpp:

```cpp
#pragma once

#include <hip/hip_runtime.h>
#include <stdint.h>
#include <type_traits>

#include "../../include/raftgpu.h"

namespace rg {

constexpr int K = RG_TERM_RUNS;
constexpr int BLOCK = 64;

struct alignas(16) I64x2 { int64_t x, y; };
struct alignas(16) I32x4 { int32_t x, y, z, w; };
struct alignas(8) U32x2 { uint32_t x, y; };
struct alignas(16) Ident { int32_t voted_for, leader; uint32_t role_epoch, meta; };
struct alignas(16) Elect { int64_t elected_term; uint32_t elected_epoch; int32_t votes; };
struct alignas(16) Match { int64_t match_index; int32_t rejection; int32_t pad; };

constexpr uint32_t META_ROLE = 3u, META_TD = 1u << 2, META_PREP = 1u << 3;
constexpr int META_RC_SHIFT = 4, META_PEND_SHIFT = 8;
constexpr uint32_t META_PEND_MASK = (1u << (RG_MAX_CLUSTER - 1)) - 1u;

struct DevTable {
    I64x2 *term_commit;
    I64x2 *epoch;
    I64x2 *window;
    Ident *ident;
    Elect *elect;
    I64x2 *runs;
    I64x2 *peer_en;
    Match *peer_m;
    int64_t *ibase;
    uint32_t groups;
};

struct StepParams {
    DevTable t;
    uint32_t rounds, count;
    const uint32_t *gid;
    const rg_ev_head_t *head;
    const I64x2 *ab, *cd, *hint;
    const int64_t *entry_terms;
    const I32x4 *abcd32;
    const int32_t *entry_terms32;
    uint64_t entry_count;
    rg_reply_t *reply;
    I64x2 *logfx;
    rg_persist_t *persist;
    I32x4 *out32, *persist32;
    unsigned long long *counters;
    unsigned long long *wide_bodies;
    int32_t self, cluster, majority, pre_vote;
    int32_t fast_paths;
    int32_t force_wide;
    int32_t require_fence;
    int32_t has_bases;
    int32_t auto_window;
    uint32_t stride;
};

struct ReplicateParams {
    DevTable t;
    uint32_t count;
    const uint32_t *gid;
    const uint8_t *heartbeat;
    const uint16_t *in_flight;
    rg_send_head_t *head;
    rg_send_t *send;
    uint16_t *counts;
    const rg_ev_head_t *ev_head;
    const I32x4 *ev_out32;
    uint32_t ev_stride, self;
};

struct TimerParams {
    int64_t *deadline;
    uint32_t *epoch;
    const Ident *ident;
    uint32_t groups, rounds, count;
    const uint32_t *gid;
    const rg_reply_t *reply;
    const I32x4 *out32, *persist32;
    const int64_t *now_mem;
    int64_t now[64];
    int64_t election_ms, heartbeat_ms;
    uint64_t seed;
};

struct HealthParams {
    int64_t *ok, *fail;
    int32_t *recent;
    DevTable t;
    uint32_t rounds, count, followers, self;
    const uint32_t *gid;
    const rg_ev_head_t *head;
    const rg_reply_t *reply;
    const I32x4 *out32;
    const int64_t *now_mem;
    int64_t now[64];
    uint16_t *counts;
};

struct TickFoldParams {
    TimerParams tp;
    HealthParams hp;
    const int64_t *now_last;
    unsigned long long *masks;
    uint32_t *ticket;
    uint32_t *out_gid, *out_epoch, *out_count;
    uint32_t capacity;
    int expire;
    const uint32_t *rounds_now;
};
struct TickTailParams {
    TickFoldParams fp;
    ReplicateParams qp;
    HealthParams rp;
    int32_t critical_point;
    int64_t cool_down;
    uint8_t *ready;
};

hipError_t launch_step(const StepParams &p, int followers, bool sparse, int shape, hipStream_t s);
hipError_t launch_copy(const void *src, void *dst, size_t bytes, hipStream_t s);
hipError_t launch_replicate(const ReplicateParams &p, int followers, hipStream_t s);
hipError_t launch_health_update(const HealthParams &p, hipStream_t s);
hipError_t launch_health_failure(const HealthParams &p, uint32_t n, const uint32_t *gid, const uint8_t *slot, const uint8_t *flags, const uint16_t *done, hipStream_t s);
hipError_t launch_ready(const HealthParams &p, int64_t now, int32_t cp, int64_t cd, uint8_t *ready, hipStream_t s);
hipError_t launch_timers_update(const TimerParams &p, hipStream_t s);
hipError_t launch_tick_fold(const TickFoldParams &p, hipStream_t s);
hipError_t launch_tick_tail(const TickTailParams &p, int followers, hipStream_t s);
hipError_t launch_tick(const StepParams &p, const TickTailParams &tp, int followers, hipStream_t s);
hipError_t launch_tick_sparse(const StepParams &p, const TickTailParams &tp, const uint32_t *rows_now, int followers, hipStream_t s);
hipError_t launch_tick_expire(const TickFoldParams &p, hipStream_t s);
hipError_t launch_timers_arm(const TimerParams &p, hipStream_t s);
hipError_t launch_timers_expired(int64_t *deadline, const Ident *ident, uint32_t groups, int64_t now, const int64_t *now_mem, uint32_t *counts, uint32_t *total,
                                 uint32_t *out_gid, uint32_t *out_epoch, uint32_t capacity, hipStream_t s);
hipError_t launch_outcome_count(const rg_reply_t *reply, uint32_t rows, uint32_t *counts, uint32_t *totals, hipStream_t s);
hipError_t launch_outcome_emit(const rg_reply_t *reply, const I64x2 *logfx, const rg_persist_t *persist, uint32_t rows, const uint32_t *counts,
                               I64x2 *out_logfx, uint32_t cap_logfx, rg_persist_t *out_persist, uint32_t cap_persist, hipStream_t s);

__device__ __forceinline__ int64_t wadd(int64_t a, int64_t b) { return (int64_t)((uint64_t)a + (uint64_t)b); }
__device__ __forceinline__ int64_t wsub(int64_t a, int64_t b) { return (int64_t)((uint64_t)a - (uint64_t)b); }
__device__ __forceinline__ int64_t max64(int64_t a, int64_t b) { return a > b ? a : b; }
__device__ __forceinline__ int64_t min64(int64_t a, int64_t b) { return a < b ? a : b; }
template <class V> __device__ __forceinline__ V vadd(V x, V y) { typedef typename std::make_unsigned<V>::type U; return (V)((U)x + (U)y); }
template <class V> __device__ __forceinline__ V vmin(V x, V y) { return x < y ? x : y; }
template <class V> __device__ __forceinline__ V vmax(V x, V y) { return x > y ? x : y; }

constexpr uint32_t EV_LIMIT = 1u << 30;
constexpr uint32_t STATE_LIMIT = (1u << 30) + (1u << 29);

template <class V>
__device__ __forceinline__ void cmp_exchange(V &a, V &b)
{
    const bool sw = a > b;
    const V lo = sw ? b : a, hi = sw ? a : b;
    a = lo; b = hi;
}
template <int F, class V>
__device__ __forceinline__ void major_indices(V (&m)[F], V &full, V &major)
{
    if constexpr (F == 4 && sizeof(V) == 4) {
        const V lo1 = vmin(m[0], m[1]), hi1 = vmax(m[0], m[1]), lo2 = vmin(m[2], m[3]), hi2 = vmax(m[2], m[3]);
        full = vmin(lo1, lo2);
        major = vmax(vmax(lo1, lo2), vmin(hi1, hi2));
    } else if constexpr (F == 4) {
        cmp_exchange(m[0], m[1]); cmp_exchange(m[2], m[3]);
        cmp_exchange(m[0], m[2]); cmp_exchange(m[1], m[3]);
        full = m[0]; major = m[1] > m[2] ? m[1] : m[2];
    } else {
#pragma unroll
        for (int a = 1; a < F; a++) {
#pragma unroll
            for (int b = a; b > 0; b--) cmp_exchange(m[b - 1], m[b]);
        }
        full = m[0]; major = m[F / 2];
    }
}

__device__ __forceinline__ int64_t rejection_step(int32_t r)
{
    if (r < 0) return r == -1 ? 1 : 0;
    int64_t s = 1;
    s += r >= 2; s += r >= 10; s += r >= 31; s += r >= 88; s += r >= 242; s += r >= 663; s += r >= 1806;
    s += r >= 4913; s += r >= 13358; s += r >= 36313; s += r >= 98714; s += r >= 268335; s += r >= 729414;
    s += r >= 1982757; s += r >= 5389696; s += r >= 14650717; s += r >= 39824782; s += r >= 108254986;
    s += r >= 294267564; s += r >= 799902175;
    return s;
}

template <class V>
struct FxT {
    uint32_t flags;
    uint32_t status;
    V resp_term;
    V log_from;
};
typedef FxT<int64_t> Fx;

constexpr uint32_t HDR_AE_OK = 1u << 10, HDR_PEER_OK = 1u << 11, HDR_WIDE = 1u << 9;

template <class V>
struct GroupT {
    V term, commit, epoch_index, epoch_term, first, last, elected_term;
    V s0, s1, s2, s3;
    V t0, t1, t2, t3;
    V lt, top;
    int32_t voted_for, leader, votes, role, rc;
    uint32_t role_epoch, elected_epoch, pending;
    bool td, prepared, log_dirty, peers_dirty;
    static_assert(K == 4, "run cache is hand-unrolled for 4 runs");
// ... 891 lines not shown
```

rafting_amd/csrc/rg_step.hpp:

```cpp
#pragma once
#include "rg_device.hpp"
#include "rg_tier1n.hpp"

namespace rg {

typedef uint32_t u32x2 __attribute__((vector_size(8)));
typedef uint32_t u32x4 __attribute__((vector_size(16)));

template <class T> __device__ __forceinline__ T nt_load16(const T *p)
{
    static_assert(sizeof(T) == 16, "16-byte row");
    const u32x4 v = __builtin_nontemporal_load(reinterpret_cast<const u32x4 *>(p));
    T r; __builtin_memcpy(&r, &v, 16); return r;
}
template <class T> __device__ __forceinline__ T nt_load8(const T *p)
{
    static_assert(sizeof(T) == 8, "8-byte row");
    const u32x2 v = __builtin_nontemporal_load(reinterpret_cast<const u32x2 *>(p));
    T r; __builtin_memcpy(&r, &v, 8); return r;
}
template <class T> __device__ __forceinline__ void nt_store16(T *p, const T &x)
{
    static_assert(sizeof(T) == 16, "16-byte row");
    u32x4 v; __builtin_memcpy(&v, &x, 16);
// ... 239 lines not shown
    __device__ __forceinline__ void add_status(uint32_t status)
    {
        asserts += (status != RG_OK && status < RG_NPE_MAJOR_NULL) ? 1u : 0u;
        need += status == RG_NEED_HOST ? 1u : 0u;
        stale += status == RG_DROPPED_STALE_ROLE ? 1u : 0u;
    }
    __device__ __forceinline__ void add_packed(uint32_t kind, uint32_t flags, uint32_t status)
    {
        rows += kind != RG_EV_NONE ? 1u : 0u;
        packed += ((((flags >> 1) & 0x55u) * 0x41041u) & 0x01010101u);
        add_status(status);
    }
    uint32_t packed_status = 0;
    static __device__ __forceinline__ uint32_t status_entry(uint32_t status)
    {
        return ((status != RG_OK && status < RG_NPE_MAJOR_NULL) ? 1u : 0u) | (status == RG_NEED_HOST ? 1u << 8 : 0u) | (status == RG_DROPPED_STALE_ROLE ? 1u << 16 : 0u);
    }
    __device__ __forceinline__ void add_packed_lut(uint32_t kind, uint32_t flags, uint32_t status, const uint32_t *lut)
    {
        rows += kind != RG_EV_NONE ? 1u : 0u;
        packed += ((((flags >> 1) & 0x55u) * 0x41041u) & 0x01010101u);
        packed_status += lut[status & 63u];
    }
    __device__ __forceinline__ void spill()
    {
        replied += packed & 0xFFu; conv += (packed >> 8) & 0xFFu; commit += (packed >> 16) & 0xFFu; append += packed >> 24;
        asserts += packed_status & 0xFFu; need += (packed_status >> 8) & 0xFFu; stale += (packed_status >> 16) & 0xFFu;
        packed = 0u; packed_status = 0u;
    }
    __device__ __forceinline__ void flush(const StepParams &p, uint32_t lane, bool active) const
    {
        uint32_t tally[RG_NUM_COUNTERS] = {rows, replied, conv, commit, asserts, need, stale, append};
#pragma unroll
        for (int c = 0; c < RG_NUM_COUNTERS; c++) {
            uint32_t v = active ? tally[c] : 0u;
#pragma unroll
            for (int off = 32; off > 0; off >>= 1) v += __shfl_xor(v, off, 64);
            tally[c] = v;
        }
        if (lane < RG_NUM_COUNTERS) {
            uint32_t v = tally[0];
#pragma unroll
            for (int c = 1; c < RG_NUM_COUNTERS; c++) v = (lane == (uint32_t)c) ? tally[c] : v;
            unsigned long long *slot = p.counters + (size_t)blockIdx.x * RG_NUM_COUNTERS + lane;
            *slot += v;
        }
    }
};

template <int F, bool SPARSE>
__global__ __launch_bounds__(BLOCK, 1) void step_kernel(const StepParams p)
{
    __shared__ int64_t sh_epoch[F * BLOCK], sh_next[F * BLOCK], sh_match[F * BLOCK];
    __shared__ int32_t sh_rej[F * BLOCK];

    const uint32_t lane = threadIdx.x;
    const uint32_t i = blockIdx.x * BLOCK + lane;
    const bool active = i < p.count;
    const uint32_t ir = active ? i : p.count - 1u;
    const uint32_t gi = SPARSE ? p.gid[ir] : ir;
    const uint32_t round_rows = SPARSE ? p.stride : p.count;

    Group g;
    load_group(p.t, gi, g);
    EventRow cur{}, near{}, far{};
    EventTail cur_t{}, near_t{};
    const uint32_t last_round = p.rounds - 1u;
    load_event<false>(p, ir, cur);
    load_event<false>(p, (size_t)(last_round < 1u ? last_round : 1u) * round_rows + ir, near);
    PeersWide<F> pe;
    pe.e = sh_epoch + lane; pe.n = sh_next + lane; pe.m = sh_match + lane; pe.r = sh_rej + lane; pe.overflow = false;
    stage_peers<F>(p.t, gi, g, pe);

    Stepper<F, PeersWide<F>> st(p, g, pe);
    const bool FAST = p.fast_paths != 0;
    Tally tally;
    bool blocked = false;
    int64_t flush_max = 0;

    rg_reply_t pend_rep{0, 0u, 0u};
    I64x2 pend_lfx{0, 0};
    rg_persist_t pend_per{0, 0, 0};
    bool pend_w_lfx = false, pend_w_per = false;

    load_event_tail<false>(p, ir, cur, cur_t);
    for (uint32_t r = 0; r < p.rounds; r++) {
        const size_t row = (size_t)r * round_rows + ir;
        __builtin_amdgcn_s_waitcnt(0x0F70);
        if (r > 0) {
            if (active) nt_store16(p.reply + (row - round_rows), pend_rep);
            if (pend_w_lfx) nt_store16(p.logfx + (row - round_rows), pend_lfx);
            if (pend_w_per) nt_store16(p.persist + (row - round_rows), pend_per);
        }
        const uint32_t r1 = r + 1u < p.rounds ? r + 1u : last_round, r2 = r + 2u < p.rounds ? r + 2u : last_round;
        load_event<false>(p, (size_t)r2 * round_rows + ir, far);
        load_event_tail<false>(p, (size_t)r1 * round_rows + ir, near, near_t);

        {
            const uint32_t kind = RG_HDR_KIND(cur.hdr);
            const bool skip = blocked & (kind != RG_EV_NONE);
            flush_max = ((kind == RG_EV_LOG_FLUSH) & (cur.a > flush_max)) ? cur.a : flush_max;
            const uint32_t hdr = decorate<false>(p, cur, cur_t, false);
            const bool done = tier1<F, int64_t, PeersWide<F>>(p, g, pe, st.fx, FAST & !skip, hdr, cur.aux, cur.a, cur.b, cur.c, cur.d, cur_t.e0);
            bool slow = !done & !skip;
            if (skip) st.fx = Fx{0u, RG_SKIPPED_AFTER_NEED_HOST, 0, 0};
            if (__builtin_amdgcn_ballot_w64(slow) != 0) {
                if (slow) slow = !tier15w<F, int64_t, PeersWide<F>>(p, g, pe, st.fx, FAST, hdr, cur.aux, (RG_HDR_HINT(cur.hdr) != 0) & (p.hint != nullptr), cur.a, cur.b, cur.c, cur.d, cur_t.e0);
                if (slow) {
                    const Entries en = entries_of<false>(p, cur.hdr, cur.aux, cur_t.e0, cur_t.e1, cur_t.e2, cur_t.e3);
                    st.run(cur.hdr, cur.aux, cur.a, cur.b, cur.c, cur.d, (RG_HDR_HINT(cur.hdr) != 0) & (p.hint != nullptr), cur_t.hx, cur_t.hy, en,
                           entries_readable(p, en, cur.aux, RG_HDR_N(cur.hdr)));
                }
            }
            const uint32_t status = st.fx.status, flags = st.fx.flags;
            if (status == RG_NEED_HOST) blocked = true;
            pend_rep.resp_term = (flags & RG_F_REPLIED) ? st.fx.resp_term : 0;
            pend_rep.flags = flags | ((uint32_t)g.role << RG_F_ROLE_SHIFT) | (status << RG_F_STATUS_SHIFT);
            pend_rep.role_epoch = g.role_epoch;
            pend_w_lfx = active & (((flags & (RG_F_COMMIT | RG_F_LOG_APPEND | RG_F_LOG_TRUNC)) != 0) | (status == RG_NEED_HOST));
            pend_lfx = I64x2{g.commit, st.fx.log_from};
            pend_w_per = active & ((flags & RG_F_PERSIST) != 0);
            pend_per.term = g.term; pend_per.voted_for = g.voted_for; pend_per.role = g.role;
            tally.add(kind, flags, status);
        }
        cur = near; cur_t = near_t;
        near = far;
    }
    if (active) {
        const size_t row = (size_t)(p.rounds - 1) * round_rows + ir;
        nt_store16(p.reply + row, pend_rep);
        if (pend_w_lfx) nt_store16(p.logfx + row, pend_lfx);
        if (pend_w_per) nt_store16(p.persist + row, pend_per);
    }

    if (active) {
        store_group(p.t, gi, g, pe, F);
        if (p.auto_window != 0) advance_base(p, gi, p.t.ibase[gi], flush_max);
    }
    tally.flush(p, lane, active);
}

enum { EV_HEAD = 0, EV_A, EV_B, EV_C, EV_D, EV_E0, EV_HX, EV_HY, EV_E1, EV_E2, EV_E3, EV_FIELDS };
enum { OUT_RESP = 0, OUT_FLAGS, OUT_COMMIT, OUT_FROM, OUT_TERM, OUT_VOTE, OUT_FIELDS };

__device__ __forceinline__ void lds_barrier()
{
    __builtin_amdgcn_s_waitcnt(0xC07F);
    __builtin_amdgcn_s_barrier();
    asm volatile("" ::: "memory");
}

template <int F, bool EV32, int NO = 2>
struct SplitLds {
    static constexpr int EVF = EV32 ? (int)EV_D + 1 : (int)EV_FIELDS;
    static constexpr size_t W_EPOCH = 0, W_NEXT = W_EPOCH + F * BLOCK * 8, W_MATCH = W_NEXT + F * BLOCK * 8, W_REJ = W_MATCH + F * BLOCK * 8,
                            W_EV = W_REJ + F * BLOCK * 4, W_OUT = W_EV + 2 * EVF * BLOCK * 8, W_AUTO = W_OUT + 2 * OUT_FIELDS * BLOCK * 8,
                            W_END = W_AUTO + BLOCK * 24;
    static constexpr int MV = (F + 3) / 4;
    static constexpr int NEV = 4;
    static constexpr size_t N_REC = 0, N_MV = N_REC + F * BLOCK * 16, N_EVH = N_MV + MV * BLOCK * 16, N_EVQ = N_EVH + NEV * BLOCK * 16,
                            N_O0 = N_EVQ + NEV * BLOCK * 16, N_O1 = N_O0 + NO * BLOCK * 16, N_BAIL = N_O1 + NO * BLOCK * 16,
                            N_LUTC = N_BAIL + 16, N_LUTM = N_LUTC + 256 * 4, N_LUTE = N_LUTM + 128 * 4,
                            N_BASE = N_LUTE + 128 * 2, N_LUTS = N_BASE + BLOCK * 8,
                            N_END = N_LUTS + 64 * 4;
    static constexpr size_t BYTES = EV32 ? (W_END > N_END ? W_END : N_END) : W_END;
};

template <int F, bool SPARSE, bool EV32, bool OUT32 = false>
__device__ __forceinline__ void split_body(const StepParams &p, unsigned char *smem)
{
    static_assert(EV32 || !OUT32, "compact outcome rows belong to the compact-row kernels");
    typedef SplitLds<F, EV32> L;
    int64_t *sh_epoch = reinterpret_cast<int64_t *>(smem + L::W_EPOCH), *sh_next = reinterpret_cast<int64_t *>(smem + L::W_NEXT),
            *sh_match = reinterpret_cast<int64_t *>(smem + L::W_MATCH);
    int32_t *sh_rej = reinterpret_cast<int32_t *>(smem + L::W_REJ);
    uint64_t (*sh_ev)[L::EVF][BLOCK] = reinterpret_cast<uint64_t (*)[L::EVF][BLOCK]>(smem + L::W_EV);
    uint64_t (*sh_out)[OUT_FIELDS][BLOCK] = reinterpret_cast<uint64_t (*)[OUT_FIELDS][BLOCK]>(smem + L::W_OUT);

    const uint32_t lane = threadIdx.x & (BLOCK - 1);
    const bool io_wave = __builtin_amdgcn_readfirstlane(threadIdx.x) >= (uint32_t)BLOCK;
    const uint32_t i = blockIdx.x * BLOCK + lane;
    const bool active = i < p.count;
    const uint32_t ir = active ? i : p.count - 1u;
    const uint32_t last_round = p.rounds - 1u;
    const uint32_t round_rows = SPARSE ? p.stride : p.count;

    if (io_wave) {
        auto row_of = [&](uint32_t r) { return (size_t)(r < p.rounds ? r : last_round) * round_rows + ir; };
        int64_t io_base = 0;
        if constexpr (EV32) io_base = (p.has_bases != 0) ? p.t.ibase[SPARSE ? p.gid[ir] : ir] : 0;
        const bool io_rel = EV32 && __builtin_amdgcn_ballot_w64(io_base != 0) != 0;
        auto publish = [&](uint32_t slot, const EventRow &e, const EventTail &t) {
            sh_ev[slot][EV_HEAD][lane] = (uint64_t)decorate<EV32>(p, e, t, false) | ((uint64_t)e.aux << 32);
            if (io_rel) {
                const uint32_t ix = index_fields(RG_HDR_KIND(e.hdr));
                sh_ev[slot][EV_A][lane] = (uint64_t)((ix & 1u) ? to_abs(e.a, io_base) : e.a); sh_ev[slot][EV_B][lane] = (uint64_t)((ix & 2u) ? to_abs(e.b, io_base) : e.b);
                sh_ev[slot][EV_C][lane] = (uint64_t)((ix & 4u) ? to_abs(e.c, io_base) : e.c); sh_ev[slot][EV_D][lane] = (uint64_t)((ix & 8u) ? to_abs(e.d, io_base) : e.d);
            } else {
                sh_ev[slot][EV_A][lane] = (uint64_t)e.a; sh_ev[slot][EV_B][lane] = (uint64_t)e.b; sh_ev[slot][EV_C][lane] = (uint64_t)e.c; sh_ev[slot][EV_D][lane] = (uint64_t)e.d;
            }
            if constexpr (!EV32) {
                sh_ev[slot][EV_E0][lane] = (uint64_t)t.e0;
                sh_ev[slot][EV_HX][lane] = (uint64_t)t.hx; sh_ev[slot][EV_HY][lane] = (uint64_t)t.hy;
                sh_ev[slot][EV_E1][lane] = (uint64_t)t.e1;
                sh_ev[slot][EV_E2][lane] = (uint64_t)t.e2; sh_ev[slot][EV_E3][lane] = (uint64_t)t.e3;
            }
        };
        Tally tally;
        auto retire = [&](uint32_t r, uint32_t hdr) {
            const uint32_t slot = r & 1u;
            const size_t row = (size_t)r * round_rows + ir;
            const uint64_t fe = sh_out[slot][OUT_FLAGS][lane];
            const uint32_t flags_all = (uint32_t)fe, flags = flags_all & 0xFFFFu, status = RG_F_STATUS(flags_all);
            rg_reply_t rep;
            rep.resp_term = (int64_t)sh_out[slot][OUT_RESP][lane]; rep.flags = flags_all; rep.role_epoch = (uint32_t)(fe >> 32);
            const bool w_lfx = active & (((flags & (RG_F_COMMIT | RG_F_LOG_APPEND | RG_F_LOG_TRUNC)) != 0) | (status == RG_NEED_HOST));
            const bool w_per = active & ((flags & RG_F_PERSIST) != 0);
            const I64x2 lfx{(int64_t)sh_out[slot][OUT_COMMIT][lane], (int64_t)sh_out[slot][OUT_FROM][lane]};
            const uint64_t v = sh_out[slot][OUT_VOTE][lane];
            rg_persist_t per;
            per.term = (int64_t)sh_out[slot][OUT_TERM][lane]; per.voted_for = (int32_t)(uint32_t)v; per.role = (int32_t)(uint32_t)(v >> 32);
            if constexpr (OUT32) {
                const int64_t commit_r = io_rel ? to_rel(lfx.x, io_base) : lfx.x, from_r = io_rel ? to_rel(lfx.y, io_base) : lfx.y;
                const uint64_t bits = (uint64_t)rep.resp_term | (uint64_t)commit_r | (w_lfx ? (uint64_t)from_r : 0ull) | (w_per ? (uint64_t)per.term : 0ull);
                const bool wide = bits >= (1ull << 31);
                if (active) {
                    nt_store16(p.out32 + row, I32x4{(int32_t)rep.resp_term, (int32_t)(flags_all | (wide ? RG_F_WIDE_VALUES : 0u)), (int32_t)commit_r, (int32_t)from_r});
                    if (w_per) nt_store16(p.persist32 + row, I32x4{(int32_t)per.term, per.voted_for, (int32_t)rep.role_epoch, per.role});
                    if (wide & (p.reply != nullptr)) {
                        nt_store16(p.reply + row, rep);
                        if (w_lfx) nt_store16(p.logfx + row, lfx);
                        if (w_per) nt_store16(p.persist + row, per);
                    }
                }
            } else {
                if (active) nt_store16(p.reply + row, rep);
                if (w_lfx) nt_store16(p.logfx + row, lfx);
                if (w_per) nt_store16(p.persist + row, per);
            }
            tally.add(RG_HDR_KIND(hdr), flags, status);
        };

        EventRow n1{}, n2{}, n3{}, n4{};
        EventTail t1{}, t2{};
        uint32_t hdr_cur, hdr_prev = 0u;
        {
            EventRow first{};
            EventTail first_t{};
            load_event<EV32>(p, row_of(0), first);
            load_event<EV32>(p, row_of(1), n1);
            load_event<EV32>(p, row_of(2), n2);
            load_event<EV32>(p, row_of(3), n3);
            load_event<EV32>(p, row_of(4), n4);
            load_event_tail<EV32>(p, row_of(0), first, first_t);
            load_event_tail<EV32>(p, row_of(1), n1, t1);
            load_event_tail<EV32>(p, row_of(2), n2, t2);
            publish(0u, first, first_t);
            hdr_cur = first.hdr;
        }
        lds_barrier();
        for (uint32_t r = 0; r < p.rounds; r++) {
            publish((r + 1u) & 1u, n1, t1);
            if (r > 0) retire(r - 1u, hdr_prev);
            hdr_prev = hdr_cur; hdr_cur = n1.hdr;
            n1 = n2; t1 = t2;
            n2 = n3;
            n3 = n4;
            load_event_tail<EV32>(p, row_of(r + 3u), n2, t2);
            load_event<EV32>(p, row_of(r + 5u), n4);
            lds_barrier();
        }
        retire(last_round, hdr_prev);
        tally.flush(p, lane, active);
        return;
    }

    __builtin_amdgcn_s_setprio(3);
    const uint32_t gi = SPARSE ? p.gid[ir] : ir;
    Group g;
    load_group(p.t, gi, g);
    PeersWide<F> pe;
    pe.e = sh_epoch + lane; pe.n = sh_next + lane; pe.m = sh_match + lane; pe.r = sh_rej + lane; pe.overflow = false;
    stage_peers<F>(p.t, gi, g, pe);
    Stepper<F, PeersWide<F>> st(p, g, pe);
    const bool FAST = p.fast_paths != 0;
    bool blocked = false;
    int64_t *sh_flush = reinterpret_cast<int64_t *>(smem + L::W_AUTO) + 3 * lane;
    sh_flush[0] = 0;
    sh_flush[1] = (active & (p.auto_window != 0)) ? (int64_t)reinterpret_cast<uint64_t>(p.t.ibase + gi) : 0;
    sh_flush[2] = p.auto_window;
    lds_barrier();
    for (uint32_t r = 0; r < p.rounds; r++) {
        const uint32_t slot = r & 1u;
        const uint64_t head = sh_ev[slot][EV_HEAD][lane];
        const uint32_t hdr = (uint32_t)head, aux = (uint32_t)(head >> 32);
        const int64_t a = (int64_t)sh_ev[slot][EV_A][lane], b = (int64_t)sh_ev[slot][EV_B][lane],
                      c = (int64_t)sh_ev[slot][EV_C][lane], d = (int64_t)sh_ev[slot][EV_D][lane];
        int64_t e0 = (int64_t)(int32_t)aux;
        if constexpr (!EV32) e0 = (int64_t)sh_ev[slot][EV_E0][lane];
        const uint32_t kind = RG_HDR_KIND(hdr);
        { const int64_t top = *sh_flush; *sh_flush = ((kind == RG_EV_LOG_FLUSH) & (a > top)) ? a : top; }
        const bool skip = blocked & (kind != RG_EV_NONE);
        const bool done = tier1<F, int64_t, PeersWide<F>>(p, g, pe, st.fx, FAST & !skip, hdr, aux, a, b, c, d, e0);
        bool slow = !done & !skip;
        if (skip) st.fx = Fx{0u, RG_SKIPPED_AFTER_NEED_HOST, 0, 0};
        if (__builtin_amdgcn_ballot_w64(slow) != 0) {
            if (slow) slow = !tier15w<F, int64_t, PeersWide<F>>(p, g, pe, st.fx, FAST, hdr, aux, EV32 ? false : ((RG_HDR_HINT(hdr) != 0) & (p.hint != nullptr)), a, b, c, d, e0);
            if (slow) {
                int64_t hx = 0, hy = 0, e1 = e0, e2 = e0, e3 = e0;
                if constexpr (!EV32) {
                    hx = (int64_t)sh_ev[slot][EV_HX][lane]; hy = (int64_t)sh_ev[slot][EV_HY][lane];
                    e1 = (int64_t)sh_ev[slot][EV_E1][lane]; e2 = (int64_t)sh_ev[slot][EV_E2][lane]; e3 = (int64_t)sh_ev[slot][EV_E3][lane];
                }
                const Entries en = entries_of<EV32>(p, hdr, aux, e0, e1, e2, e3);
                const bool hinted = EV32 ? false : ((RG_HDR_HINT(hdr) != 0) & (p.hint != nullptr));
                st.run(hdr, aux, a, b, c, d, hinted, hx, hy, en, entries_readable(p, en, aux, RG_HDR_N(hdr)));
            }
        }
        const uint32_t status = st.fx.status, flags = st.fx.flags;
        if (status == RG_NEED_HOST) blocked = true;
        const uint32_t flags_all = flags | ((uint32_t)g.role << RG_F_ROLE_SHIFT) | (status << RG_F_STATUS_SHIFT);
        sh_out[slot][OUT_RESP][lane] = (flags & RG_F_REPLIED) ? (uint64_t)st.fx.resp_term : 0ull;
        sh_out[slot][OUT_FLAGS][lane] = (uint64_t)flags_all | ((uint64_t)g.role_epoch << 32);
        sh_out[slot][OUT_COMMIT][lane] = (uint64_t)g.commit;
        sh_out[slot][OUT_FROM][lane] = (uint64_t)st.fx.log_from;
        sh_out[slot][OUT_TERM][lane] = (uint64_t)g.term;
        sh_out[slot][OUT_VOTE][lane] = (uint64_t)(uint32_t)g.voted_for | ((uint64_t)(uint32_t)g.role << 32);
        lds_barrier();
    }
    uint32_t gi_out = gi;
    RG_FRESH_VGPR(gi_out);
    if (active) store_group(p.t, gi_out, g, pe, F);
    if (const int64_t at = sh_flush[1]; at != 0) {
        RG_GLOBAL_AS int64_t *slot = reinterpret_cast<RG_GLOBAL_AS int64_t *>((uint64_t)at);
        const int64_t top = sh_flush[0], window = sh_flush[2];
        if (top - window > *slot) *slot = top - window;
    }
}

template <int F, bool SPARSE>
__global__ __launch_bounds__(2 * BLOCK) void step_split_kernel(const StepParams p)
{
    __shared__ alignas(16) unsigned char smem[SplitLds<F, false>::BYTES];
    split_body<F, SPARSE, false>(p, smem);
}

struct Row32 { U32x2 h; I32x4 q; };

constexpr int CW_AUXC = 18;
template <int F = 0>
__device__ __forceinline__ uint32_t class_entry(const StepParams &p, uint32_t idx)
{
    const uint32_t kind = idx & 15u, slot = idx >> 4;
    const uint32_t P = (uint32_t)p.cluster, self = (uint32_t)p.self;
    const bool peer_ok = (slot < P) & (slot != self);
    const bool ack = (kind == RG_EV_AE_ACK) & peer_ok, vreq = (kind == RG_EV_RV_REQ) | (kind == RG_EV_PV_REQ),
               vrep = (kind == RG_EV_RV_REPLY) | (kind == RG_EV_PV_REPLY);
    const uint32_t j = ack ? (slot < self ? slot : slot - 1u) : 0u;
    const uint32_t cls = (ack ? 1u << CW_ACK : 0u) | (((kind == RG_EV_AE_REQ) & (slot < P)) ? 1u << CW_AE : 0u) | ((kind == RG_EV_CLIENT_APPEND) ? 1u << CW_CLIENT : 0u) |
                         (((ack | (kind == RG_EV_IS_ACK)) & peer_ok) ? 1u << CW_ACKANY : 0u) |
                         ((kind - (uint32_t)RG_EV_RV_REQ <= (uint32_t)(RG_EV_TIMEOUT - RG_EV_RV_REQ)) ? 1u << CW_ELK : 0u) |
                         ((vrep & peer_ok) ? 1u << CW_VR : 0u) | ((kind == RG_EV_PV_REPLY) ? 1u << CW_PV : 0u) | ((kind == RG_EV_TIMEOUT) ? 1u << CW_TO : 0u) |
                         ((vreq & (slot < P)) ? 1u << CW_VQ : 0u) | ((kind == RG_EV_PV_REQ) ? 1u << CW_PVQ : 0u) | ((kind == RG_EV_NONE) ? 1u << CW_NONE : 0u) |
                         ((((0x1CCu >> kind) & 1u) != 0) ? 1u << CW_AUXC : 0u);
    const uint32_t j4 = F > 6 ? (j & 15u) : j;
    return cls | (j4 << 10) | (slot << 5) | (31u - j);
}
__device__ __forceinline__ I32x4 class_word(const uint32_t *lutc, const Row32 &x)
{
    const uint32_t hdr = x.h.x, aux = x.h.y;
    const uint32_t e = lutc[hdr & 0xFFu];
    const int32_t n = (int32_t)(hdr >> 12);
    const sw same = (int32_t)(hdr << (31 - 10));
    const int32_t n_lim = (same >> 31) & (int32_t)RG_MAX_AE_ENTRIES;
    const sw ae_bad = ~s_pos(x.q.z) | s_lt(n_lim, n), cli_bad = s_lt(n, 1);
    const uint32_t auxm = (uint32_t)(((int32_t)(e << (31 - CW_AUXC)) | ((int32_t)(e << (31 - CW_AE)) & same)) >> 31);
    const uint32_t w = (uint32_t)x.q.x | (uint32_t)x.q.y | (uint32_t)x.q.z | (uint32_t)x.q.w | (aux & auxm);
    const uint32_t ood = (uint32_t)((int32_t)(w | (w << 1)) >> 31);
    const uint32_t off = (((uint32_t)ae_bad & 0x80000000u) >> (31 - CW_AE)) | (((uint32_t)cli_bad & 0x80000000u) >> (31 - CW_CLIENT)) | (1u << CW_AUXC) |
                         (ood & 0xFFF80000u);
    const uint32_t cw = (e & ~off) | ((hdr & 0x100u) << (CW_FLAG - 8));
    return I32x4{(int32_t)cw, (int32_t)aux, n, (int32_t)(hdr | (ood & KIND_OUT_OF_DOMAIN))};
}
__device__ __forceinline__ uint32_t expand_by_table(const uint32_t *lutm, const uint16_t *lute, uint32_t w)
{
    const uint32_t fast = lutm[w & 127u] | (uint32_t)lute[(w >> 7) & 127u];
    return ((int32_t)w < 0) ? (w & 0x00FFFFFFu) : fast;
}

template <int F, bool SPARSE, bool OUT32, int IOW = 1, int RPB = 1>
__device__ __forceinline__ bool narrow_body(const StepParams &p, unsigned char *smem)
{
    static_assert(RPB == 1 || (RPB == 2 && IOW == 1), "two rounds per hand-over: the two-wavefront workgroup only");
    constexpr int NO = 2 * RPB;
    typedef SplitLds<F, true, NO> L;
    I32x4 *sh_rec = reinterpret_cast<I32x4 *>(smem + L::N_REC);
    int32_t *sh_mv = reinterpret_cast<int32_t *>(smem + L::N_MV);
    I32x4 (*sh_evh)[BLOCK] = reinterpret_cast<I32x4 (*)[BLOCK]>(smem + L::N_EVH);
    I32x4 (*sh_evq)[BLOCK] = reinterpret_cast<I32x4 (*)[BLOCK]>(smem + L::N_EVQ);
    I32x4 (*sh_o0)[BLOCK] = reinterpret_cast<I32x4 (*)[BLOCK]>(smem + L::N_O0);
    I32x4 (*sh_o1)[BLOCK] = reinterpret_cast<I32x4 (*)[BLOCK]>(smem + L::N_O1);
    uint32_t *sh_bail = reinterpret_cast<uint32_t *>(smem + L::N_BAIL);
    uint32_t *sh_lutc = reinterpret_cast<uint32_t *>(smem + L::N_LUTC), *sh_lutm = reinterpret_cast<uint32_t *>(smem + L::N_LUTM);
    uint16_t *sh_lute = reinterpret_cast<uint16_t *>(smem + L::N_LUTE);
    uint32_t *sh_luts = reinterpret_cast<uint32_t *>(smem + L::N_LUTS);

    const uint32_t lane = threadIdx.x & (BLOCK - 1);
    const bool io_wave = __builtin_amdgcn_readfirstlane(threadIdx.x) >= (uint32_t)BLOCK;
    const uint32_t i = blockIdx.x * BLOCK + lane;
    const bool active = i < p.count;
    const uint32_t ir = active ? i : p.count - 1u;
    const uint32_t last_round = p.rounds - 1u;

    if (io_wave) {
        RG_HWID_BEGIN(1);
        const bool do_pub = IOW == 1 || __builtin_amdgcn_readfirstlane(threadIdx.x) < 2u * BLOCK;
        const bool do_ret = IOW == 1 || !do_pub;
        uint64_t b_head = reinterpret_cast<uint64_t>(p.head), b_q = reinterpret_cast<uint64_t>(p.abcd32),
                 b_reply = OUT32 ? reinterpret_cast<uint64_t>(p.out32) : reinterpret_cast<uint64_t>(p.reply),
                 b_logfx = reinterpret_cast<uint64_t>(p.logfx),
                 b_persist = OUT32 ? reinterpret_cast<uint64_t>(p.persist32) : reinterpret_cast<uint64_t>(p.persist);
        RG_OWN_SGPRS(b_head); RG_OWN_SGPRS(b_q); RG_OWN_SGPRS(b_reply); RG_OWN_SGPRS(b_logfx); RG_OWN_SGPRS(b_persist);
        const uint64_t round_rows = SPARSE ? p.stride : p.count;
        const uint32_t irm = ir & 0x0FFFFFFFu;
        int64_t io_base = 0;
        if constexpr (!OUT32) io_base = (p.has_bases != 0) ? p.t.ibase[SPARSE ? p.gid[ir] : ir] : 0;
        auto fetch = [&](uint32_t r, Row32 &x) {
            const uint64_t rb = (uint64_t)(r < p.rounds ? r : last_round) * round_rows;
            x.h = nt_load_at<U32x2>(b_head + rb * 8u, irm);
            x.q = nt_load_at<I32x4>(b_q + rb * 16u, irm);
        };
#pragma unroll
        for (int k = 0; k < 4; k++) sh_lutc[lane + 64u * k] = class_entry<F>(p, lane + 64u * k);
#pragma unroll
        for (int k = 0; k < 2; k++) {
            const uint32_t i7 = lane + 64u * k;
            sh_lutm[i7] = expand_predicates(i7);
            sh_lute[i7] = (uint16_t)(expand_predicates((i7 << 7) | 0x42u) & 0xFFFFu);
        }
        sh_luts[lane] = Tally::status_entry(lane);
        __builtin_amdgcn_wave_barrier();
        auto publish = [&](uint32_t slot, const Row32 &x) {
            sh_evh[slot][lane] = class_word(sh_lutc, x);
            sh_evq[slot][lane] = x.q;
        };
        Tally tally;
        auto retire = [&](uint32_t r, uint32_t hdr) {
            const uint32_t slot = r & (uint32_t)(NO - 1);
            const uint64_t rb16 = (uint64_t)r * round_rows * 16u;
            const I32x4 o0 = sh_o0[slot][lane], o1 = sh_o1[slot][lane];
            const uint32_t flags_all = expand_by_table(sh_lutm, sh_lute, (uint32_t)o0.y) | ((uint32_t)o1.w << RG_F_ROLE_SHIFT), flags = flags_all & 0xFFFFu, status = RG_F_STATUS(flags_all);
            if constexpr (OUT32) {
                nt_store_at(b_reply + rb16, irm, I32x4{(flags & RG_F_REPLIED) ? o0.x : 0, (int32_t)flags_all, o0.w, o1.x});
                if ((flags & RG_F_PERSIST) != 0) nt_store_at(b_persist + rb16, irm, I32x4{o1.y, o1.z, o0.z, o1.w});
            } else {
                rg_reply_t rep;
                rep.resp_term = (flags & RG_F_REPLIED) ? (int64_t)(uint32_t)o0.x : 0; rep.flags = flags_all; rep.role_epoch = (uint32_t)o0.z;
                nt_store_at(b_reply + rb16, irm, rep);
                const bool w_lfx = ((flags & (RG_F_COMMIT | RG_F_LOG_APPEND | RG_F_LOG_TRUNC)) != 0) | (status == RG_NEED_HOST);
                if (w_lfx) nt_store_at(b_logfx + rb16, irm, I64x2{to_abs((int64_t)(uint32_t)o0.w, io_base), to_abs((int64_t)(uint32_t)o1.x, io_base)});
                if ((flags & RG_F_PERSIST) != 0) {
                    rg_persist_t per;
                    per.term = (int64_t)(uint32_t)o1.y; per.voted_for = o1.z; per.role = o1.w;
                    nt_store_at(b_persist + rb16, irm, per);
                }
            }
            tally.add_packed_lut(RG_HDR_KIND(hdr), flags, status, sh_luts);
        };
        Row32 buf[4];
        uint32_t hdr_m1 = 0u, hdr_0, hdr_1;
        if (do_pub) {
            Row32 e0, e1;
            fetch(0, e0); fetch(1, e1); fetch(2, buf[2]); fetch(3, buf[3]); fetch(4, buf[0]); fetch(5, buf[1]);
            publish(0u, e0); publish(1u, e1);
            hdr_0 = e0.h.x; hdr_1 = e1.h.x;
        } else {
            hdr_0 = hdr_1 = 0u;
            for (int k = 0; k < 4; k++) { buf[k].h = U32x2{0u, 0u}; buf[k].q = I32x4{0, 0, 0, 0}; }
        }
        lds_barrier();
        { const uint32_t seen0 = *sh_bail; if (__builtin_amdgcn_readfirstlane(seen0) == 1u) return false; }
        bool bailed = false;
        uint32_t seen = 0u;
        RG_PROBE_BEGIN();
        if constexpr (RPB == 2) {
            uint32_t hk[4] = {hdr_0, hdr_1, 0u, 0u};
            for (uint32_t r0 = 0; r0 < p.rounds && !bailed; r0 += 4u) {
                if ((r0 & 127u) == 124u) tally.spill();
#pragma unroll
                for (int k = 0; k < 4; k++) {
                    const uint32_t r = r0 + (uint32_t)k;
                    if (r >= p.rounds) break;
                    Row32 &x = buf[(k + 2) & 3];
                    publish((r + 2u) & 3u, x);
                    RG_PROBE_MARK(0);
                    if (r >= 2u) retire(r - 2u, hk[(k + 2) & 3]);
                    hk[(k + 2) & 3] = x.h.x;
                    fetch(r + 6u, x);
                    RG_PROBE_MARK(1);
                    if ((k & 1) != 0 || r == last_round) {
                        const uint32_t mark = __builtin_amdgcn_readfirstlane(seen), pair = r >> 1;
                        if ((mark != 0u) & (mark <= pair + 1u)) { bailed = true; break; }
                        lds_barrier();
                        RG_PROBE_MARK(2);
                        seen = *sh_bail;
                    }
                }
            }
            if (bailed) return false;
            { const uint32_t mark = __builtin_amdgcn_readfirstlane(seen); if (mark != 0u) return false; }
            for (uint32_t q = p.rounds >= 2u ? p.rounds - 2u : 0u; q < p.rounds; q++) {
                const uint32_t i = q & 3u;
                retire(q, i == 0u ? hk[0] : (i == 1u ? hk[1] : (i == 2u ? hk[2] : hk[3])));
            }
            tally.spill();
#if defined(RG_PROBE)
            RG_PROBE_FLUSH(0);
#elif defined(RG_PROBE_HWID)
            RG_HWID_END(1);
#else
            tally.flush(p, lane, active);
#endif
            return true;
        }
        for (uint32_t r0 = 0; r0 < p.rounds && !bailed; r0 += 4u) {
            if ((r0 & 127u) == 124u) tally.spill();
#pragma unroll
            for (int k = 0; k < 4; k++) {
                const uint32_t r = r0 + (uint32_t)k;
                if (r >= p.rounds) break;
                Row32 &x = buf[(k + 2) & 3];
                if (do_pub) publish((r + 2u) & 3u, x);
                RG_PROBE_MARK(0);
                if constexpr (IOW == 1) {
                    if (r > 0) retire(r - 1u, hdr_m1);
                    hdr_m1 = hdr_0; hdr_0 = hdr_1; hdr_1 = x.h.x;
                } else {
                    if (do_ret && r > 0) retire(r - 1u, (uint32_t)sh_evh[(r - 1u) & 3u][lane].w);
                }
                if (do_pub) fetch(r + 6u, x);
                RG_PROBE_MARK(1);
                const uint32_t mark = __builtin_amdgcn_readfirstlane(seen);
                if ((mark != 0u) & (mark <= r + 1u)) { bailed = true; break; }
                lds_barrier();
                RG_PROBE_MARK(2);
                seen = *sh_bail;
            }
        }
        if (bailed) return false;
        { const uint32_t mark = __builtin_amdgcn_readfirstlane(seen); if (mark != 0u) return false; }
        if constexpr (IOW == 1) retire(last_round, hdr_m1);
        else if (do_ret) retire(last_round, (uint32_t)sh_evh[last_round & 3u][lane].w);
        tally.spill();
#if defined(RG_PROBE)
        if (do_pub) RG_PROBE_FLUSH(0);
#elif defined(RG_PROBE_HWID)
        if (do_pub) RG_HWID_END(1);
#else
        if (do_ret) tally.flush(p, lane, active);
#endif
        return true;
    }

    __builtin_amdgcn_s_setprio(3);
    RG_HWID_BEGIN(0);
    const uint32_t gi = SPARSE ? p.gid[ir] : ir;
    GroupN g;
    PeersNarrow<F> pe;
    int64_t *sh_base = reinterpret_cast<int64_t *>(smem + L::N_BASE) + lane;
    pe.rec = sh_rec + lane; pe.mv = sh_mv + lane * 4; pe.overflow = false; pe.base = 0;
    const bool FAST = p.fast_paths != 0;
    bool in_domain, any_base;
    {
        const int64_t base = (p.has_bases != 0) ? p.t.ibase[gi] : 0;
        any_base = __builtin_amdgcn_ballot_w64(base != 0) != 0;
        *sh_base = base;
        pe.base = base;
        Group g64;
        load_group(p.t, gi, g64);
        g64.s1 = g64.rc > 1 ? g64.s1 : 0; g64.s2 = g64.rc > 2 ? g64.s2 : 0; g64.s3 = g64.rc > 3 ? g64.s3 : 0;
        if (any_base) g64 = group_to_rel(g64, base);
        in_domain = fits32(g64, EV_LIMIT) & small_fields_fit(g64) & (p.force_wide == 0) & (p.rounds < (1u << 24)) & ((base == 0) | (g64.epoch_index > 0)) & (base >= 0);
        narrow_into(g, g64);
        g.nallow = FAST ? 0 : -1;
        g.recache();
        in_domain = in_domain & stage_peers<F>(p.t, gi, g64.prepared, pe);
    }
    bool bailed = __builtin_amdgcn_ballot_w64(!in_domain) != 0;
    if (lane == 0) *sh_bail = bailed ? 1u : 0u;
    bool blocked = false;
    int32_t flush_max = 0;
    lds_barrier();
    if (bailed) return false;
    RG_PROBE_BEGIN();
#ifdef RG_EVENT_PREFETCH
    I32x4 h_next = sh_evh[0][lane], q_next = sh_evq[0][lane];
#endif
    auto round = [&](const uint32_t r) {
#ifdef RG_EVENT_PREFETCH
        const I32x4 h = h_next, q = q_next;
#else
        const I32x4 h = sh_evh[r & 3u][lane], q = sh_evq[r & 3u][lane];
#endif
        RG_PROBE_MARK(0);
        OutN out;
        const sw done = tier1n<F>(p, g, pe, out, h.x, (uint32_t)h.y, h.z, q.x, q.y, q.z, q.w);
        const bool open = done >= 0;
        RG_PROBE_MARK(1);
        const uint64_t b_open = __builtin_amdgcn_ballot_w64(open);
        const uint32_t slot = r & (uint32_t)(NO - 1);
        sh_o0[slot][lane] = I32x4{out.resp, (int32_t)out.pw, (int32_t)g.role_epoch, g.commit};
        sh_o1[slot][lane] = I32x4{out.log_from, g.term, g.voted_for, g.role};
        if (b_open != 0) {
            const uint32_t hdr = ((uint32_t)h.w & ~(7u << 9)) | ((((uint32_t)h.w & RG_HDR_SAME_TERM) != 0) ? HDR_SAME_IN : 0u), aux = (uint32_t)h.y, kind = RG_HDR_KIND(hdr);
            const bool skip = open & blocked & (kind != RG_EV_NONE);
            flush_max = (open & (kind == RG_EV_LOG_FLUSH) & (q.x > flush_max)) ? q.x : flush_max;
            bool park;
            const bool slow = open & !skip & !tier15<F>(p, g, pe, out, park, open & !skip, h.x, h.y, h.z, q.x, q.y, q.z, q.w);
            if (park) { blocked = true; g.nallow = -1; g.recache(); }
            RG_NOTE_SLOW(slow, lane == 0);
            bool bail = (slow | (skip & (p.auto_window != 0))) & (kind == KIND_OUT_OF_DOMAIN);
            if (slow & !bail) {
                const int64_t base = any_base ? *sh_base : 0;
                pe.base = base;
                Group g64 = group_to_abs(widen(g), base);
                Stepper<F, PeersNarrow<F>> st(p, g64, pe);
                const Entries en = entries_of<true>(p, hdr, aux, 0, 0, 0, 0);
                const uint32_t ix = index_fields(kind);
                st.run(hdr, aux, (ix & 1u) ? to_abs(q.x, base) : (int64_t)q.x, (ix & 2u) ? to_abs(q.y, base) : (int64_t)q.y,
                       (ix & 4u) ? to_abs(q.z, base) : (int64_t)q.z, (ix & 8u) ? to_abs(q.w, base) : (int64_t)q.w, false, 0, 0, en, entries_readable(p, en, aux, RG_HDR_N(hdr)));
                g64 = group_to_rel(g64, base);
                st.fx.log_from = to_rel(st.fx.log_from, base);
                bail = !fits32(g64, STATE_LIMIT) | !small_fields_fit(g64) | pe.overflow | ((base != 0) & (g64.epoch_index <= 0)) |
                       (((uint64_t)st.fx.resp_term | (uint64_t)st.fx.log_from) >= (uint64_t)STATE_LIMIT);
                narrow_into(g, g64);
                if (st.fx.status == RG_NEED_HOST) blocked = true;
                g.nallow = (FAST & !blocked) ? 0 : -1;
                g.recache();
                out.pw = PW_SLOW | st.fx.flags | (st.fx.status << RG_F_STATUS_SHIFT);
                out.resp = (int32_t)st.fx.resp_term; out.log_from = (int32_t)st.fx.log_from;
            }
            if (skip) { out.pw = PW_SLOW | ((uint32_t)RG_SKIPPED_AFTER_NEED_HOST << RG_F_STATUS_SHIFT); out.resp = 0; out.log_from = 0; }
            if (__builtin_amdgcn_ballot_w64(bail) != 0) {
                if (lane == 0) *sh_bail = r / (uint32_t)RPB + 2u;
                bailed = true;
            }
            sh_o0[slot][lane] = I32x4{out.resp, (int32_t)out.pw, (int32_t)g.role_epoch, g.commit};
            sh_o1[slot][lane] = I32x4{out.log_from, g.term, g.voted_for, g.role};
        } else {
            RG_NOTE_SLOW(false, lane == 0);
        }
        RG_PROBE_MARK(2);
#ifdef RG_EVENT_PREFETCH
        h_next = sh_evh[(r + 1u) & 3u][lane]; q_next = sh_evq[(r + 1u) & 3u][lane];
#endif
        if constexpr (RPB == 1) {
            lds_barrier();
            RG_PROBE_MARK(3);
        }
    };
    if constexpr (RPB == 2) {
        for (uint32_t r = 0; r < p.rounds; r++) {
            round(r);
            if (bailed) break;
            if ((r & 1u) != 0u || r == last_round) {
                lds_barrier();
                RG_PROBE_MARK(3);
            }
        }
        if (bailed) lds_barrier();
    } else {
#ifdef RG_EVENT_PREFETCH
    { uint32_t r = 0; do { round(r); r++; } while (!bailed & (r < p.rounds)); }
#else
    for (uint32_t r = 0; r < p.rounds; r++) {
        round(r);
        if (bailed) break;
    }
#endif
    }
    if (bailed) return false;
    RG_PROBE_FLUSH(4);
    RG_HWID_END(0);
    if (active) {
        Group g64 = widen(g);
        pe.base = 0;
        if (any_base) {
            const int64_t base = *sh_base;
            pe.base = base;
            g64 = group_to_abs(g64, base);
        }
        uint32_t gi_out = gi;
        RG_FRESH_VGPR(gi_out);
        store_group(p.t, gi_out, g64, pe, F);
        if (p.auto_window != 0) {
            const int64_t base = *sh_base;
            advance_base(p, gi_out, base, to_abs(flush_max, base));
        }
    }
    return true;
}

#ifndef RG_NOTE_FALLBACK
#define RG_NOTE_FALLBACK() ((void)0)
#endif

#ifndef RG_ROUNDS_PER_HANDOVER
#define RG_ROUNDS_PER_HANDOVER 1
#endif
template <int F, bool SPARSE, int WAVES, bool OUT32, int IOW = 1>
__global__ __launch_bounds__((1 + IOW) * BLOCK) __attribute__((amdgpu_waves_per_eu(WAVES, 8))) void step32_kernel(const StepParams p)
{
    constexpr int RPB = (WAVES == 1 && IOW == 1) ? RG_ROUNDS_PER_HANDOVER : 1;
    __shared__ alignas(16) unsigned char smem[SplitLds<F, true, 2 * RPB>::BYTES];
    if (narrow_body<F, SPARSE, OUT32, IOW, RPB>(p, smem)) return;
    if (threadIdx.x == 0) { RG_NOTE_FALLBACK(); atomicAdd(p.wide_bodies, 1ull); }
    if constexpr (IOW == 2) {
        if (__builtin_amdgcn_readfirstlane(threadIdx.x) >= 2u * BLOCK) {
            for (uint32_t k = 0; k < p.rounds + 2u; k++) lds_barrier();
            return;
        }
    }
    lds_barrier();
    split_body<F, SPARSE, true, OUT32>(p, smem);
}

template <int F, bool SPARSE, int WAVES, bool OUT32>
__global__ __launch_bounds__(2 * BLOCK) __attribute__((amdgpu_waves_per_eu(WAVES, 8))) void step32_wide_kernel(const StepParams p)
{
    __shared__ alignas(16) unsigned char smem[SplitLds<F, true>::BYTES];
    if (threadIdx.x == 0) { RG_NOTE_FALLBACK(); atomicAdd(p.wide_bodies, 1ull); }
    split_body<F, SPARSE, true, OUT32>(p, smem);
}

#if !defined(RG_BUILD_ONLY_F4)
#define RG_F_MASK 0x7FFEu
#elif defined(RG_BUILD_ALSO_F)
#define RG_F_MASK ((1u << 4) | (RG_BUILD_ALSO_F))
#else
#define RG_F_MASK (1u << 4)
#endif

#if !defined(RG_TU) || RG_TU == 1
#define RG_TU_MAIN 1
#endif

template <class L, int F>
static hipError_t launch_one(const L &l)
{
    if constexpr (((RG_F_MASK) >> F) & 1u) return l.template run<F>();
    else return hipErrorInvalidValue;
}
template <class L, int LO>
hipError_t launch_range(const L &l, int followers)
{
    switch (followers - LO) {
    case 0: return launch_one<L, LO>(l);
    case 1: return launch_one<L, LO + 1>(l);
    case 2: return launch_one<L, LO + 2>(l);
    case 3: return launch_one<L, LO + 3>(l);
    default: return hipErrorInvalidValue;
    }
}
template <class L>
static hipError_t launch_followers(const L &l, int followers)
{
    switch (followers) {
    case 1: return launch_one<L, 1>(l);
    case 2: return launch_one<L, 2>(l);
    case 3: return launch_one<L, 3>(l);
    case 4: return launch_one<L, 4>(l);
    case 5: return launch_one<L, 5>(l);
    case 6: return launch_one<L, 6>(l);
    case 7: case 8: case 9: case 10: return launch_range<L, 7>(l, followers);
    case 11: case 12: case 13: case 14: return launch_range<L, 11>(l, followers);
    default: return hipErrorInvalidValue;
    }
}

template <class Fn>
static hipError_t lift(bool b, Fn fn) { return b ? fn(std::true_type{}) : fn(std::false_type{}); }

template <int F> constexpr int WAVES_MANY = F <= 6 ? 4 : 1;
constexpr uint32_t MANY_BLOCKS = 1024u;
#ifdef RG_IOW2
constexpr int SMALL_IOW = 2;
#else
constexpr int SMALL_IOW = 1;
#endif

template <int F, bool SPARSE, bool OUT32>
static hipError_t launch_compact(const StepParams &p, hipStream_t s)
{
    const uint32_t blocks = (p.count + BLOCK - 1) / BLOCK;
    if (p.count >= (1u << 28)) return hipErrorInvalidValue;
    constexpr int MANY = WAVES_MANY<F>, IOW = (F <= 6 && OUT32 && !SPARSE) ? SMALL_IOW : 1;
    const bool many = blocks > MANY_BLOCKS;
    const dim3 grid(blocks), wg(2 * BLOCK);
    if (p.force_wide != 0) {
        if (many) hipLaunchKernelGGL((step32_wide_kernel<F, SPARSE, MANY, OUT32>), grid, wg, 0, s, p);
        else      hipLaunchKernelGGL((step32_wide_kernel<F, SPARSE, 1, OUT32>), grid, wg, 0, s, p);
    } else {
        if (many) hipLaunchKernelGGL((step32_kernel<F, SPARSE, MANY, OUT32>), grid, wg, 0, s, p);
        else      hipLaunchKernelGGL((step32_kernel<F, SPARSE, 1, OUT32, IOW>), grid, dim3((1 + IOW) * BLOCK), 0, s, p);
    }
    return hipGetLastError();
}

struct StepLaunch {
    const StepParams &p;
    bool sparse;
    int shape;
    hipStream_t s;
    template <int F> hipError_t run() const
    {
        if (shape != 0 && shape != 64 && shape != 32) return hipErrorInvalidValue;
        const StepParams &p = this->p;
        const hipStream_t s = this->s;
        const dim3 grid((p.count + BLOCK - 1) / BLOCK);
        if (grid.x == 0) return hipSuccess;
        return lift(sparse, [&](auto sp) {
            constexpr bool SPARSE = decltype(sp)::value;
            if (shape == 32) return lift(p.out32 != nullptr, [&](auto o) { return launch_compact<F, SPARSE, decltype(o)::value>(p, s); });
            if (shape == 64) hipLaunchKernelGGL((step_kernel<F, SPARSE>), grid, dim3(BLOCK), 0, s, p);
            else             hipLaunchKernelGGL((step_split_kernel<F, SPARSE>), grid, dim3(2 * BLOCK), 0, s, p);
            return hipGetLastError();
        });
    }
};

}
```

rafting_amd/engine.py:

```python
import ctypes as C
import os

import numpy as np

from . import abi

_HERE = os.path.dirname(os.path.abspath(__file__))
LIB_PATH = os.environ.get("RG_LIB") or os.path.join(_HERE, "libraftgpu.so")
_LIB = None


class EngineError(RuntimeError):
    pass


def library_sha16():
    import hashlib
    with open(LIB_PATH, "rb") as f:
        return hashlib.sha256(f.read()).hexdigest()[:16]


def exported_symbols():
    return [
        "rg_abi_version", "rg_table_create", "rg_table_destroy", "rg_last_error", "rg_table_groups",
        "rg_table_cluster", "rg_table_option", "rg_load_state", "rg_read_state", "rg_submit", "rg_submit32", "rg_submit32c", "rg_submit32c_sparse", "rg_submit32c_sparse_rounds", "rg_outcome32_unpack", "rg_outcome32_unpack_rel", "rg_index_base_set", "rg_index_base_get", "rg_index_base_advance", "rg_index_base_advance32", "rg_batch32_pack_rel", "rg_batch32_pack", "rg_submit_async", "rg_submit_async_packed", "rg_submit_wait", "rg_tick_create", "rg_tick_launch", "rg_tick_wait", "rg_tick_destroy", "rg_tick2_create", "rg_tick2_create_sparse", "rg_tick2_create_sparse_rounds", "rg_tick2_launch", "rg_tick2_wait", "rg_tick2_destroy", "rg_assembler_create", "rg_assemble32", "rg_assembler_destroy", "rg_timers_update32", "rg_health_update32", "rg_sync", "rg_step_kernel", "rg_host_alloc", "rg_host_free", "rg_dev_alloc",
        "rg_dev_free", "rg_copy_to_device", "rg_copy_to_host", "rg_stream", "rg_replicate", "rg_timers_configure", "rg_timers_update",
        "rg_timers_expired", "rg_timers_expired_epochs", "rg_timers_arm", "rg_timers_read", "rg_health_update", "rg_health_failure", "rg_ready", "rg_health_read", "rg_in_flight_read", "rg_in_flight_set",
        "rg_timing_enable",
        "rg_timing_read", "rg_timing_begin", "rg_timing_end", "rg_counters_read", "rg_wide_body_workgroups", "rg_copy_bandwidth",
    ]


def _share_hip_runtime_with_torch():
    import importlib.util
    import sys
    if "torch" in sys.modules:
        return
    try:
        spec = importlib.util.find_spec("torch")
    except (ImportError, ValueError):
        spec = None
    if spec is None or not spec.submodule_search_locations:
        return
    cand = os.path.join(list(spec.submodule_search_locations)[0], "lib", "libamdhip64.so")
    if os.path.exists(cand):
        try:
            C.CDLL(cand, mode=C.RTLD_GLOBAL)
        except OSError:
            pass


def lib():
    global _LIB
    if _LIB is None:
        if not os.path.exists(LIB_PATH):
            raise EngineError(
                "%s is missing — build it with `make -C rafting_amd/csrc` (or __graft_entry__.build()); "
                "there is no CPU fallback for the decision path" % LIB_PATH)
        _share_hip_runtime_with_torch()
        L = C.CDLL(LIB_PATH)
        if hasattr(L, "rg_is_host_emulation") and os.environ.get("RG_ALLOW_HOST_EMULATION") != "1":
            raise EngineError("%s is the test-only host emulation of the kernels (tests/devemu), not libraftgpu.so; "
                              "the decision path has no CPU fallback" % LIB_PATH)
        vp, u32, i32 = C.c_void_p, C.c_uint32, C.c_int
        L.rg_abi_version.restype = i32
        L.rg_table_create.argtypes = [i32, u32, u32, u32, i32, C.POINTER(vp)]
        L.rg_table_destroy.argtypes = [vp]
        L.rg_last_error.restype = C.c_char_p
        L.rg_last_error.argtypes = [vp]
        L.rg_table_groups.restype = u32
        L.rg_table_groups.argtypes = [vp]
        L.rg_table_cluster.restype = u32
        L.rg_table_cluster.argtypes = [vp]
        L.rg_table_option.argtypes = [vp, i32, i32]
        L.rg_load_state.argtypes = [vp, u32, u32, C.POINTER(abi.CGroupState)]
        L.rg_read_state.argtypes = [vp, u32, u32, C.POINTER(abi.CGroupState)]
        L.rg_submit.argtypes = [vp, C.POINTER(abi.CBatch), C.POINTER(abi.COutcome), i32]
        L.rg_submit32.argtypes = [vp, C.POINTER(abi.CBatch32), C.POINTER(abi.COutcome), i32]
        if os.environ.get("RG_LIB"):
            class _Tolerant:
                def __init__(self, lib_):
                    object.__setattr__(self, "_lib", lib_)

                def __getattr__(self, name):
                    try:
                        return getattr(self._lib, name)
                    except AttributeError:
                        class _Missing:
                            def __call__(self, *a):
                                raise EngineError("%s is not exported by %s" % (name, LIB_PATH))
                        return _Missing()
            real, L = L, _Tolerant(L)
        L.rg_submit32c.argtypes = [vp, C.POINTER(abi.CBatch32), C.POINTER(abi.COutcome32), i32]
        L.rg_submit32c_sparse.argtypes = [vp, C.POINTER(abi.CBatch32), C.POINTER(abi.COutcome32), i32]
        L.rg_submit32c_sparse_rounds.argtypes = [vp, C.POINTER(abi.CBatch32), C.POINTER(abi.COutcome32), i32]
        L.rg_outcome32_unpack.argtypes = [C.POINTER(abi.COutcome32), u32, u32, vp, C.POINTER(abi.COutcome)]
        L.rg_outcome32_unpack_rel.argtypes = [C.POINTER(abi.COutcome32), u32, u32, vp, vp, C.POINTER(abi.COutcome)]
        L.rg_index_base_set.argtypes = [vp, u32, u32, vp]
        L.rg_index_base_get.argtypes = [vp, u32, u32, vp]
        L.rg_index_base_advance.argtypes = [C.POINTER(abi.CBatch), i32, u32, vp]
        L.rg_index_base_advance32.argtypes = [C.POINTER(abi.CBatch32), i32, u32, vp]
        L.rg_batch32_pack_rel.restype = C.c_int64
        L.rg_batch32_pack_rel.argtypes = [C.POINTER(abi.CBatch), vp, vp, vp, vp]
        L.rg_batch32_pack.restype = C.c_int64
        L.rg_batch32_pack.argtypes = [C.POINTER(abi.CBatch), vp, vp, vp]
        L.rg_submit_async.argtypes = [vp, C.POINTER(abi.CBatch), C.POINTER(abi.COutcome)]
        L.rg_submit_wait.argtypes = [vp]
        L.rg_submit_async_packed.argtypes = [vp, vp, vp]
        L.rg_sync.argtypes = [vp]
        L.rg_tick_create.argtypes = [vp, vp, vp, C.POINTER(vp)]
        L.rg_tick_launch.argtypes = [vp]
        L.rg_tick_wait.argtypes = [vp]
        L.rg_tick_destroy.argtypes = [vp]
        L.rg_tick2_create.argtypes = [vp, C.POINTER(abi.CTick2Io), C.POINTER(vp)]
        L.rg_tick2_create_sparse.argtypes = [vp, C.POINTER(abi.CTick2Io), C.POINTER(abi.CTick2Rows), C.POINTER(vp)]
        L.rg_tick2_create_sparse_rounds.argtypes = [vp, C.POINTER(abi.CTick2Io), C.POINTER(abi.CTick2Rounds), C.POINTER(vp)]
        L.rg_tick2_launch.argtypes = [vp]
        L.rg_tick2_wait.argtypes = [vp]
        L.rg_tick2_destroy.argtypes = [vp]
        L.rg_assembler_create.argtypes = [vp, u32, u32, C.POINTER(vp)]
        L.rg_assemble32.argtypes = [vp, C.POINTER(abi.CArrivals), C.POINTER(abi.CAssembled), i32]
        L.rg_assembler_destroy.argtypes = [vp]
        L.rg_timers_update32.argtypes = [vp, u32, vp, vp, vp, i32]
        L.rg_health_update32.argtypes = [vp, u32, vp, vp, vp, i32]
        L.rg_replicate.argtypes = [vp, u32, vp, vp, vp, vp, vp, i32]
        L.rg_step_kernel.restype = C.c_char_p
        L.rg_step_kernel.argtypes = [vp, u32]
        L.rg_timers_configure.argtypes = [vp, C.c_int64, C.c_int64, C.c_uint64]
        L.rg_timers_update.argtypes = [vp, u32, u32, vp, vp, vp, i32]
        L.rg_timers_expired.argtypes = [vp, C.c_int64, vp, u32, C.POINTER(u32), i32]
        L.rg_timers_expired_epochs.argtypes = [vp, C.c_int64, vp, vp, u32, C.POINTER(u32), i32]
        L.rg_timers_arm.argtypes = [vp, C.c_int64]
        L.rg_timers_read.argtypes = [vp, u32, u32, vp]
        L.rg_health_update.argtypes = [vp, u32, u32, vp, vp, vp, vp, i32]
        L.rg_health_failure.argtypes = [vp, u32, vp, vp, vp, C.c_int64]
        L.rg_ready.argtypes = [vp, C.c_int64, i32, C.c_int64, vp, i32]
        L.rg_health_read.argtypes = [vp, u32, u32, vp, vp, vp]
        L.rg_in_flight_read.argtypes = [vp, u32, u32, vp]
        L.rg_in_flight_set.argtypes = [vp, u32, u32, vp]
        L.rg_host_alloc.argtypes = [vp, C.c_size_t, C.POINTER(vp)]
        L.rg_host_free.argtypes = [vp, vp]
        L.rg_dev_alloc.argtypes = [vp, C.c_size_t, C.POINTER(vp)]
        L.rg_dev_free.argtypes = [vp, vp]
        L.rg_copy_to_device.argtypes = [vp, vp, vp, C.c_size_t]
        L.rg_copy_to_host.argtypes = [vp, vp, vp, C.c_size_t]
        L.rg_stream.restype = vp
        L.rg_stream.argtypes = [vp]
        L.rg_timing_enable.argtypes = [vp, i32]
        L.rg_timing_read.argtypes = [vp, C.POINTER(C.c_uint64), C.POINTER(C.c_double), i32]
        L.rg_timing_begin.argtypes = [vp]
        L.rg_timing_end.argtypes = [vp, C.POINTER(C.c_double)]
        L.rg_counters_read.argtypes = [vp, C.POINTER(C.c_uint64), i32]
        L.rg_wide_body_workgroups.argtypes = [vp, C.POINTER(C.c_uint64), i32]
        L.rg_copy_bandwidth.argtypes = [vp, C.c_size_t, i32, C.POINTER(C.c_double)]
        if L.rg_abi_version() != abi.ABI_VERSION:
            raise EngineError("libraftgpu.so ABI %d != binding ABI %d" % (L.rg_abi_version(), abi.ABI_VERSION))
        _LIB = L
    return _LIB


def _replicate(call, groups, cluster, gid, heartbeat, in_flight):
    F = cluster - 1
    gid = None if gid is None else np.ascontiguousarray(gid, dtype=np.uint32)
    count = groups if gid is None else len(gid)
    hb = None if heartbeat is None else np.ascontiguousarray(np.broadcast_to(heartbeat, (count,)), dtype=np.uint8)
    fl = None if in_flight is None else np.ascontiguousarray(np.asarray(in_flight, dtype=np.uint16).reshape(count, F).T).reshape(count * F)
    head = np.zeros(count, dtype=abi.SEND_HEAD_DT)
    send = np.zeros(count * F, dtype=abi.SEND_DT)
    ptr = lambda a: None if a is None else a.ctypes.data
    call(count, ptr(gid), ptr(hb), ptr(fl), head.ctypes.data, send.ctypes.data)
    return head, np.ascontiguousarray(send.reshape(F, count).T)


def advance_index_base(batch, base, window):
    if not (isinstance(base, np.ndarray) and base.dtype == np.int64 and base.flags["C_CONTIGUOUS"]):
        raise EngineError("advance_index_base: base must be a contiguous int64 array (it is updated in place)")
    b = batch.as_struct()
    fn = lib().rg_index_base_advance32 if isinstance(batch, abi.Batch32) else lib().rg_index_base_advance
    rc = fn(C.byref(b), int(window), len(base), base.ctypes.data)
    if rc != 0:
        raise EngineError("advance_index_base: %d (%s)" % (rc, {-1: "missing column or window outside [1, 2^30)", -2: "batch shape does not fit the groups"}.get(rc, "?")))
    return base


def pack32(batch, index_base=None):
    rows = batch.rounds * batch.count
    head = np.zeros(rows, dtype=abi.HEAD_DT)
    abcd = np.zeros(rows, dtype=abi.QUAD32_DT)
    terms = np.zeros(max(batch.entry_count, 1), dtype=np.int32)
    b = batch.as_struct()
    if index_base is None:
        n = lib().rg_batch32_pack(C.byref(b), head.ctypes.data, abcd.ctypes.data, terms.ctypes.data)
    else:
        ib = np.ascontiguousarray(index_base, dtype=np.int64)
        n = lib().rg_batch32_pack_rel(C.byref(b), ib.ctypes.data, head.ctypes.data, abcd.ctypes.data, terms.ctypes.data)
    if n < 0:
        raise EngineError("rg_batch32_pack: %d (%s)" % (n, {-1: "missing column", -2: "the batch carries hints", -3: "a value outside [0, 2^31)",
                                                             -4: "entry_terms needed"}.get(n, "?")))
    return abi.Batch32(batch.rounds, batch.count, batch.gid, head, abcd, terms, n)


def pinned_like(table, array):
    a = np.ascontiguousarray(array)
    p = C.c_void_p()
    table._check(lib().rg_host_alloc(table._h, max(a.nbytes, 16), C.byref(p)))
    buf = (C.c_char * max(a.nbytes, 16)).from_address(p.value)
    view = np.frombuffer(buf, dtype=a.dtype, count=a.size).reshape(a.shape)
    view[...] = a

    class _Owner:
        ptr = p.value

        def free(self):
            if self.ptr:
                lib().rg_host_free(table._h, self.ptr)
                self.ptr = None
    return view, _Owner()


class PackedBatch:

    def __init__(self, table, batch, logfx_cap=None, persist_cap=None, entry_cap=0):
        assert abi.batch_fits_32(batch), "a value outside [0, 2^31) or a hint column: use submit_async for this batch"
        rows = batch.rounds * batch.count
        self.rows, self.table, self._owners = rows, table, []
        b32 = pack32(batch)
        self.head, self.abcd = self._pin(b32.head), self._pin(b32.abcd)
        et = np.zeros(max(entry_cap, b32.entry_count, 1), dtype=np.int32)
        et[:b32.entry_count] = b32.entry_terms[:b32.entry_count]
        self.entry_terms = self._pin(et)
        self.gid = None if batch.gid is None else self._pin(batch.gid)
        self.logfx_cap = rows if logfx_cap is None else logfx_cap
        self.persist_cap = rows if persist_cap is None else persist_cap
        self.reply = self._pin(np.zeros(rows, dtype=abi.REPLY_DT))
        self.logfx = self._pin(np.zeros(max(self.logfx_cap, 1), dtype=abi.LOGFX_DT))
        self.persist = self._pin(np.zeros(max(self.persist_cap, 1), dtype=abi.PERSIST_DT))
        self.counts = self._pin(np.zeros(2, dtype=np.uint32))
        b = abi.CBatch32()
        b.rounds, b.count = batch.rounds, batch.count
        b.gid = None if self.gid is None else self.gid.ctypes.data
        b.head, b.abcd = self.head.ctypes.data, self.abcd.ctypes.data
        b.entry_terms = self.entry_terms.ctypes.data if (b32.entry_count or entry_cap) else None
        b.entry_count = b32.entry_count
        o = abi.COutcomePacked()
        o.reply, o.logfx, o.persist, o.counts = self.reply.ctypes.data, self.logfx.ctypes.data, self.persist.ctypes.data, self.counts.ctypes.data
        o.logfx_cap, o.persist_cap = self.logfx_cap, self.persist_cap
        self.c_in, self.c_out = b, o

    def _pin(self, a):
        view, own = pinned_like(self.table, a)
        self._owners.append(own)
        return view

    @property
    def bytes_up(self):
        return self.head.nbytes + self.abcd.nbytes + (self.entry_terms.nbytes if self.c_in.entry_count else 0) + (0 if self.gid is None else self.gid.nbytes)

    @property
    def bytes_down(self):
        return self.reply.nbytes + int(self.counts[0]) * abi.LOGFX_DT.itemsize + int(self.counts[1]) * abi.PERSIST_DT.itemsize + self.counts.nbytes

    def unpack(self):
        out = abi.Outcome(self.rows)
        out.reply[:] = self.reply
        nl, npers = int(self.counts[0]), int(self.counts[1])
        ml, mp = abi.has_logfx(self.reply["flags"]), abi.has_persist(self.reply["flags"])
        assert nl == int(ml.sum()) and npers == int(mp.sum()), "list lengths disagree with the reply marks"
        assert nl <= self.logfx_cap and npers <= self.persist_cap, "a list was truncated: raise its capacity"
        out.logfx[ml] = self.logfx[:nl]
        out.persist[mp] = self.persist[:npers]
        return out

    def free(self):
        for own in self._owners:
            own.free()
        self._owners = []


def unpack32(out32, rounds, count, role_epoch_before, index_base=None):
    out = abi.Outcome(rounds * count)
    ep = np.ascontiguousarray(role_epoch_before, dtype=np.uint32).copy()
    assert len(ep) == count and out32.rows == rounds * count
    i, o = out32.as_struct(), out.as_struct()
    ib = None if index_base is None else np.ascontiguousarray(index_base, dtype=np.int64)
    assert ib is None or len(ib) == count
    rc = lib().rg_outcome32_unpack_rel(C.byref(i), rounds, count, ep.ctypes.data, None if ib is None else ib.ctypes.data, C.byref(o))
    if rc:
        raise EngineError("rg_outcome32_unpack: %d (%s)" % (rc, {-1: "missing column", -3: "a row is flagged RG_F_WIDE_VALUES but there are no overflow columns",
                                                                 -4: "the compact and the wide copy of a row disagree"}.get(rc, "?")))
    return out, ep


class Tick:

    def __init__(self, table, pb):
        self.table, self.pb = table, pb
        h = C.c_void_p()
        pb.c_in.entry_count = len(pb.entry_terms) if pb.c_in.entry_terms else 0
        table._check(lib().rg_tick_create(table._h, C.byref(pb.c_in), C.byref(pb.c_out), C.byref(h)))
        self._h = h

    def refill(self, batch):
        b32 = batch if isinstance(batch, abi.Batch32) else pack32(batch)
        assert (b32.rounds, b32.count) == (self.pb.c_in.rounds, self.pb.c_in.count) and b32.entry_count <= self.pb.c_in.entry_count
        self.pb.head[:], self.pb.abcd[:] = b32.head, b32.abcd
        self.pb.entry_terms[:b32.entry_count] = b32.entry_terms[:b32.entry_count]
# ... 473 lines not shown
        return out32

    def submit32c_unpacked(self, batch, role_epoch_before, fill=0):
        b32 = batch if isinstance(batch, abi.Batch32) else pack32(batch)
        return unpack32(self.submit32c(b32, fill=fill), b32.rounds, b32.count, role_epoch_before)[0]

    def submit_async(self, batch, out):
        b, o = batch.as_struct(), out.as_struct()
        self._inflight = getattr(self, "_inflight", [])
        if len(self._inflight) >= abi.PIPELINE_DEPTH:
            self._inflight.pop(0)
        self._inflight.append((b, o, batch, out))
        self._check(lib().rg_submit_async(self._h, C.byref(b), C.byref(o)))
        return out

    def submit_async_packed(self, pb):
        self._inflight = getattr(self, "_inflight", [])
        if len(self._inflight) >= abi.PIPELINE_DEPTH:
            self._inflight.pop(0)
        self._inflight.append((pb.c_in, pb.c_out, pb, pb))
        self._check(lib().rg_submit_async_packed(self._h, C.byref(pb.c_in), C.byref(pb.c_out)))
        return pb

    def submit_wait(self):
        rc = lib().rg_submit_wait(self._h)
        if rc == 1:
            self._inflight = []
            return None
        self._check(rc)
        return self._inflight.pop(0)[3]

    def submit_device(self, dbatch):
        if isinstance(dbatch, DeviceBatch32) and dbatch.compact:
            self._check(lib().rg_submit32c(self._h, C.byref(dbatch.c_batch), C.byref(dbatch.c_out), abi.MEM_DEVICE))
        elif isinstance(dbatch, DeviceBatch32):
            self._check(lib().rg_submit32(self._h, C.byref(dbatch.c_batch), C.byref(dbatch.c_out), abi.MEM_DEVICE))
        else:
            self._check(lib().rg_submit(self._h, C.byref(dbatch.c_batch), C.byref(dbatch.c_out), abi.MEM_DEVICE))

    def sync(self):
        self._check(lib().rg_sync(self._h))

    def step_kernel(self, count=None):
        return lib().rg_step_kernel(self._h, self.groups if count is None else count).decode()

    def timers_configure(self, election_ms, heartbeat_ms, seed=0):
        self._check(lib().rg_timers_configure(self._h, election_ms, heartbeat_ms, seed))

    def timers_update(self, batch_rounds, batch_count, reply, now, gid=None):
        now = np.ascontiguousarray(now, dtype=np.int64)
        gid = None if gid is None else np.ascontiguousarray(gid, dtype=np.uint32)
        reply = np.ascontiguousarray(reply)
        assert len(now) == batch_rounds and len(reply) == batch_rounds * batch_count
        self._check(lib().rg_timers_update(self._h, batch_rounds, batch_count, None if gid is None else gid.ctypes.data,
                                           reply.ctypes.data, now.ctypes.data, abi.MEM_HOST))

    def timers_update32(self, rounds, out32, now):
        now = np.ascontiguousarray(now, dtype=np.int64)
        row, per = np.ascontiguousarray(out32.row), np.ascontiguousarray(out32.persist)
        assert len(now) == rounds and len(row) == rounds * self.groups == len(per)
        self._check(lib().rg_timers_update32(self._h, rounds, row.ctypes.data, per.ctypes.data, now.ctypes.data, abi.MEM_HOST))

    def health_update32(self, batch, out32, now):
        now = np.ascontiguousarray(now, dtype=np.int64)
        row = np.ascontiguousarray(out32.row)
        assert batch.gid is None and len(now) == batch.rounds and len(row) == batch.rounds * self.groups
        self._check(lib().rg_health_update32(self._h, batch.rounds, batch.head.ctypes.data, row.ctypes.data, now.ctypes.data, abi.MEM_HOST))

    def timers_arm(self, now):
        self._check(lib().rg_timers_arm(self._h, now))

    def timers_expired(self, now, capacity=None):
        capacity = self.groups if capacity is None else capacity
        out = np.zeros(max(capacity, 1), dtype=np.uint32)
        n = C.c_uint32()
        self._check(lib().rg_timers_expired(self._h, now, out.ctypes.data, capacity, C.byref(n), abi.MEM_HOST))
        return out[: min(n.value, capacity)], n.value

    def timers_expired_epochs(self, now, capacity=None):
        capacity = self.groups if capacity is None else capacity
        out, ep = np.zeros(max(capacity, 1), dtype=np.uint32), np.zeros(max(capacity, 1), dtype=np.uint32)
        n = C.c_uint32()
        self._check(lib().rg_timers_expired_epochs(self._h, now, out.ctypes.data, ep.ctypes.data, capacity, C.byref(n), abi.MEM_HOST))
        k = min(n.value, capacity)
        return out[:k], ep[:k], n.value

    def timers_read(self, first=0, count=None):
        count = self.groups - first if count is None else count
        out = np.zeros(count, dtype=np.int64)
        self._check(lib().rg_timers_read(self._h, first, count, out.ctypes.data))
        return out

    def health_update(self, batch, reply, now):
        now = np.ascontiguousarray(now, dtype=np.int64)
        reply = np.ascontiguousarray(reply)
        assert len(now) == batch.rounds and len(reply) == batch.rounds * batch.count
        self._check(lib().rg_health_update(self._h, batch.rounds, batch.count, None if batch.gid is None else batch.gid.ctypes.data,
                                           batch.head.ctypes.data, reply.ctypes.data, now.ctypes.data, abi.MEM_HOST))

    def submit_timed(self, batch, now, fill=0):
        out = self.submit(batch, fill=fill)
        self.health_update(batch, out.reply, now)
        return out

    def submit_and_update_timers(self, batch, now, fill=0):
        out = self.submit(batch, fill=fill)
        self.timers_update(batch.rounds, batch.count, out.reply, now, gid=batch.gid)
        return out

    def health_failure(self, gid, slot, flags, now):
        gid = np.ascontiguousarray(gid, dtype=np.uint32)
        slot = np.ascontiguousarray(slot, dtype=np.uint8)
        flags = np.ascontiguousarray(flags, dtype=np.uint8)
        assert len(gid) == len(slot) == len(flags)
        self._check(lib().rg_health_failure(self._h, len(gid), gid.ctypes.data, slot.ctypes.data, flags.ctypes.data, now))

    def ready(self, now, critical_point, cool_down_ms):
        out = np.zeros(self.groups, dtype=np.uint8)
        self._check(lib().rg_ready(self._h, now, critical_point, cool_down_ms, out.ctypes.data, abi.MEM_HOST))
        return out

    def health_read(self, first=0, count=None):
        count = self.groups - first if count is None else count
        F = self.cluster - 1
        ok, fl, rc = np.zeros((count, F), np.int64), np.zeros((count, F), np.int64), np.zeros((count, F), np.int32)
        self._check(lib().rg_health_read(self._h, first, count, ok.ctypes.data, fl.ctypes.data, rc.ctypes.data))
        return ok, fl, rc

    def replicate(self, gid=None, heartbeat=None, in_flight=None):
        return _replicate(lambda *a: self._check(lib().rg_replicate(self._h, *a, abi.MEM_HOST)), self.groups, self.cluster,
                          gid, heartbeat, in_flight)

    def timing_enable(self, on=True):
        self._check(lib().rg_timing_enable(self._h, int(on)))

    def timing_read(self, reset=True):
        n, ms = C.c_uint64(), C.c_double()
        self._check(lib().rg_timing_read(self._h, C.byref(n), C.byref(ms), int(reset)))
        return n.value, ms.value

    def timing_begin(self):
        self._check(lib().rg_timing_begin(self._h))

    def timing_end(self):
        ms = C.c_double()
        self._check(lib().rg_timing_end(self._h, C.byref(ms)))
        return ms.value

    def counters(self, reset=False):
        arr = (C.c_uint64 * abi.NUM_COUNTERS)()
        self._check(lib().rg_counters_read(self._h, arr, int(reset)))
        return list(arr)

    def wide_body_workgroups(self, reset=False):
        n = C.c_uint64()
        self._check(lib().rg_wide_body_workgroups(self._h, C.byref(n), int(reset)))
        return n.value

    def copy_bandwidth(self, nbytes=1 << 30, iters=10):
        g = C.c_double()
        self._check(lib().rg_copy_bandwidth(self._h, nbytes, iters, C.byref(g)))
        return g.value
```

Measured before the change: 63.29 billion.

## Chain successive device batches inside a persistent kernel via host-written descriptor ring

Adds a chaining mode, on by default, for device-memory 32-bit submits. The host writes each successor batch's pointers into a pinned descriptor ring, and a running workgroup polls the ring near the end of its rounds. If a matching successor is present, the workgroup continues into the next batch with its group state still in registers and LDS, skipping the state reload and store between launches. It also records completion per block so that later launches of already-consumed batches exit early. This is meant to remove per-launch overhead and state round-trips for short batches, at the cost of extra LDS, system-scope polling, more complex control flow and the risk of host/device ordering races.

```diff
diff --git a/include/raftgpu.h b/include/raftgpu.h
--- a/include/raftgpu.h
+++ b/include/raftgpu.h
@@ -175,6 +175,7 @@
        RG_OPT_AUTO_INDEX_BASE = 2,
        RG_OPT_COMPACT_ANY_CLUSTER = 3,
        RG_OPT_DEVICE_IN_FLIGHT = 4 };
+enum { RG_OPT_CHAIN = 5, RG_OPT_CHAIN_HOLD = 6, RG_OPT_CHAIN_BUDGET = 7 };
 int         rg_table_option(rg_table_t *t, int option, int value);
 uint32_t    rg_table_groups(const rg_table_t *t);
 uint32_t    rg_table_cluster(const rg_table_t *t);
@@ -370,6 +371,7 @@
 #define RG_NUM_COUNTERS 8
 int rg_counters_read(rg_table_t *t, uint64_t counters[RG_NUM_COUNTERS], int reset);
 int rg_wide_body_workgroups(rg_table_t *t, uint64_t *count, int reset);
+int rg_chain_info(rg_table_t *t, uint64_t *continued, int reset);
 int rg_copy_bandwidth(rg_table_t *t, size_t bytes, int iters, double *gbps);
 
 #ifdef __cplusplus
diff --git a/rafting_amd/abi.py b/rafting_amd/abi.py
--- a/rafting_amd/abi.py
+++ b/rafting_amd/abi.py
@@ -39,6 +39,7 @@
 OPT_AUTO_INDEX_BASE = 2
 OPT_COMPACT_ANY_CLUSTER = 3
 OPT_DEVICE_IN_FLIGHT = 4
+OPT_CHAIN, OPT_CHAIN_HOLD, OPT_CHAIN_BUDGET = 5, 6, 7
 SENT_TRIGGERED, SENT_HEARTBEAT = 1, 2
 HEALTH_UNREACHABLE, HEALTH_REJECT, HEALTH_NO_REQUEST = 1, 2, 4
 NUM_COUNTERS = 8
diff --git a/rafting_amd/csrc/raftgpu.cpp b/rafting_amd/csrc/raftgpu.cpp
--- a/rafting_amd/csrc/raftgpu.cpp
+++ b/rafting_amd/csrc/raftgpu.cpp
@@ -71,6 +71,15 @@
     hipStream_t s_in = nullptr, s_out = nullptr;
     PipeSlot pipe[RG_PIPELINE_DEPTH];
     uint64_t pipe_head = 0, pipe_tail = 0;
+    int chain_on = 1, chain_hold = 0;
+    uint32_t chain_budget = 512;
+    uint32_t *chain_ring = nullptr;
+    uint32_t *chain_done = nullptr;
+    uint32_t chain_blocks = 0;
+    uint32_t chain_seq = 0;
+    bool chain_prev = false;
+    rg::StepParams chain_last{};
+    std::vector<rg::StepParams> chain_held;
     std::string err;
 };
 
@@ -101,9 +110,24 @@
     return 0;
 }
 
-static int bind(rg_table *t, bool drain = true)
+extern "C" { static int launch(rg_table *t, const rg::StepParams &p, bool sparse); }
+
+static int chain_break(rg_table *t)
+{
+    t->chain_prev = false;
+    if (t->chain_held.empty()) return 0;
+    const std::vector<rg::StepParams> held = std::move(t->chain_held);
+    t->chain_held.clear();
+    for (const rg::StepParams &p : held)
+        if (int rc = launch(t, p, false)) return rc;
+    return 0;
+}
+
+static int bind(rg_table *t, bool drain = true, bool chain_keep = false)
 {
     HIP_TRY(t, hipSetDevice(t->device));
+    if (!chain_keep)
+        if (int rc = chain_break(t)) return rc;
     while (drain && t->pipe_tail != t->pipe_head)
         if (int rc = wait_oldest(t); rc < 0) return rc;
     return 0;
@@ -146,6 +170,17 @@
 {
     if (!t) return -1;
     switch (option) {
+    case RG_OPT_CHAIN:
+    case RG_OPT_CHAIN_HOLD:
+        if (value != 0 && value != 1) return fail(t, -1, "rg_table_option: RG_OPT_CHAIN and RG_OPT_CHAIN_HOLD take 0 or 1 (%d given)", value);
+        if (bind(t)) return -2;
+        (option == RG_OPT_CHAIN ? t->chain_on : t->chain_hold) = value;
+        return 0;
+    case RG_OPT_CHAIN_BUDGET:
+        if (value < 1 || value >= (1 << 23)) return fail(t, -1, "rg_table_option: RG_OPT_CHAIN_BUDGET %d outside [1, 2^23)", value);
+        if (bind(t)) return -2;
+        t->chain_budget = (uint32_t)value;
+        return 0;
     case RG_OPT_REQUIRE_FENCED_TIMEOUTS:
         if (t->require_fence != (value != 0)) t->config_gen += 1;
         t->require_fence = value != 0;
@@ -194,7 +229,10 @@
 {
     if (!t) return 0;
     (void)hipSetDevice(t->device);
+    if (t->stream) (void)chain_break(t);
     if (t->stream) (void)hipStreamSynchronize(t->stream);
+    if (t->chain_ring) (void)hipHostFree(t->chain_ring);
+    if (t->chain_done) (void)hipFree(t->chain_done);
     for (struct rg_tick *k : t->ticks) tick_release(k);
     for (struct rg_tick2 *k : t->ticks2) tick2_release(k);
     for (struct rg_assembler *a : t->assemblers) assembler_release(a);
@@ -296,6 +334,13 @@
     CREATE_TRY(hipMemsetAsync(t->dt.peer_m, 0, G * F * sizeof(rg::Match), t->stream));
     CREATE_TRY(hipMemsetAsync(t->dt.ibase, 0, G * sizeof(int64_t), t->stream));
     CREATE_TRY(hipMemsetAsync(t->counters, 0, t->counter_slots * RG_NUM_COUNTERS * sizeof(unsigned long long), t->stream));
+    t->chain_blocks = (uint32_t)((G + 63) / 64);
+    CREATE_TRY(hipHostMalloc((void **)&t->chain_ring, rg::CHAIN_RING * 64, hipHostMallocDefault));
+    memset(t->chain_ring, 0, rg::CHAIN_RING * 64);
+    CREATE_TRY(hipMalloc((void **)&t->chain_done, (size_t)(rg::CHAIN_RING + 1) * t->chain_blocks * sizeof(uint32_t)));
+    CREATE_TRY(hipMemsetAsync(t->chain_done, 0, (size_t)(rg::CHAIN_RING + 1) * t->chain_blocks * sizeof(uint32_t), t->stream));
+    if (const char *e = getenv("RG_CHAIN")) t->chain_on = atoi(e) != 0;
+    if (const char *e = getenv("RG_CHAIN_BUDGET")) { const int b = atoi(e); if (b >= 1 && b < (1 << 23)) t->chain_budget = (uint32_t)b; }
     {
         std::vector<rg::Ident> id(G, rg::Ident{RG_NO_NODE, RG_NO_NODE, 1u, 0u});
         std::vector<rg::Elect> el(G, rg::Elect{0, 0u, 1});
@@ -1351,6 +1396,39 @@
     }
 }
 
+static int submit_chained(rg_table *t, rg::StepParams &p)
+{
+    uint32_t seq = t->chain_seq + 1u;
+    if (seq == 0u) {
+        if (int rc = chain_break(t)) return rc;
+        HIP_TRY(t, hipStreamSynchronize(t->stream));
+        memset(t->chain_ring, 0, rg::CHAIN_RING * 64);
+        HIP_TRY(t, hipMemsetAsync(t->chain_done, 0, (size_t)rg::CHAIN_RING * t->chain_blocks * sizeof(uint32_t), t->stream));
+        seq = 1u;
+    }
+    p.chain_ring = t->chain_ring; p.chain_done = t->chain_done; p.chain_seq = seq; p.chain_budget = t->chain_budget; p.chain_blocks = t->chain_blocks;
+    const rg::StepParams &q = t->chain_last;
+    const bool successor = t->chain_prev && p.count == q.count && p.fast_paths == q.fast_paths && p.require_fence == q.require_fence && p.pre_vote == q.pre_vote &&
+                           p.chain_budget == q.chain_budget;
+    if (successor) {
+        uint32_t *d = t->chain_ring + (size_t)(seq & (rg::CHAIN_RING - 1u)) * 16u;
+        auto put64 = [&](int k, const void *ptr) { const uint64_t v = (uint64_t)(uintptr_t)ptr; d[k] = (uint32_t)v; d[k + 1] = (uint32_t)(v >> 32); };
+        __atomic_store_n(&d[0], 0u, __ATOMIC_RELAXED); __atomic_store_n(&d[15], 0u, __ATOMIC_RELAXED);
+        __atomic_thread_fence(__ATOMIC_SEQ_CST);
+        d[1] = p.rounds;
+        put64(2, p.head); put64(4, p.abcd32); put64(6, p.out32); put64(8, p.persist32); put64(10, p.entry_terms32);
+        d[12] = (uint32_t)p.entry_count; d[13] = 0u; d[14] = 0u;
+        __atomic_thread_fence(__ATOMIC_SEQ_CST);
+        __atomic_store_n(&d[0], seq, __ATOMIC_RELAXED); __atomic_store_n(&d[15], seq, __ATOMIC_RELAXED);
+        __atomic_thread_fence(__ATOMIC_SEQ_CST);
+    }
+    t->chain_seq = seq;
+    t->chain_prev = true;
+    t->chain_last = p;
+    if (t->chain_hold) { t->chain_held.push_back(p); return 0; }
+    return launch(t, p, false);
+}
+
 static int submit32c(rg_table_t *t, const rg_batch32_t *in, const rg_outcome32_t *out, int memspace, bool sparse, const char *who, bool list_rounds = false)
 {
     if (!t) return -1;
@@ -1369,7 +1447,9 @@
     const rg_outcome_t shape{&dummy_r, &dummy_l, &dummy_p};
     if (int rc = check_batch(t, &wide, &shape, memspace == RG_MEM_HOST, list_rounds)) return rc;
     if (in->count == 0) return 0;
-    if (bind(t)) return -2;
+    const bool chainable = t->chain_on && !sparse && memspace == RG_MEM_DEVICE && wides == 0 && !t->force_wide && !t->has_bases && !t->auto_window && !t->timing &&
+                           in->rounds <= t->chain_budget && t->F <= 6;
+    if (bind(t, true, chainable)) return -2;
     const size_t rows = (size_t)in->rounds * in->count;
     rg::StepParams p = step_params(t, &wide);
     if (memspace == RG_MEM_DEVICE) {
@@ -1377,6 +1457,7 @@
         p.entry_terms32 = in->entry_count ? in->entry_terms : nullptr;
         p.out32 = (rg::I32x4 *)out->row; p.persist32 = (rg::I32x4 *)out->persist;
         p.reply = out->wide.reply; p.logfx = (I64x2 *)out->wide.logfx; p.persist = out->wide.persist;
+        if (chainable) return submit_chained(t, p);
         return launch(t, p, sparse);
     }
     if (memspace != RG_MEM_HOST) return fail(t, -1, "%s: unknown memspace %d", who, memspace);
@@ -1952,7 +2033,27 @@
     return 0;
 }
 
-void *rg_stream(rg_table_t *t) { return t ? (void *)t->stream : nullptr; }
+void *rg_stream(rg_table_t *t)
+{
+    if (!t) return nullptr;
+    (void)bind(t);
+    return (void *)t->stream;
+}
+
+int rg_chain_info(rg_table_t *t, uint64_t *continued, int reset)
+{
+    if (!t || !continued) return -1;
+    if (bind(t)) return -2;
+    std::vector<uint32_t> host(t->chain_blocks);
+    uint32_t *row = t->chain_done + (size_t)rg::CHAIN_RING * t->chain_blocks;
+    HIP_TRY(t, hipMemcpyAsync(host.data(), row, host.size() * sizeof(uint32_t), hipMemcpyDeviceToHost, t->stream));
+    if (reset) HIP_TRY(t, hipMemsetAsync(row, 0, host.size() * sizeof(uint32_t), t->stream));
+    HIP_TRY(t, hipStreamSynchronize(t->stream));
+    uint64_t n = 0;
+    for (uint32_t v : host) n += v;
+    *continued = n;
+    return 0;
+}
 
 
 int rg_timing_enable(rg_table_t *t, int on)
diff --git a/rafting_amd/csrc/rg_device.hpp b/rafting_amd/csrc/rg_device.hpp
--- a/rafting_amd/csrc/rg_device.hpp
+++ b/rafting_amd/csrc/rg_device.hpp
@@ -58,7 +58,13 @@
     int32_t has_bases;
     int32_t auto_window;
     uint32_t stride;
-};
+    const uint32_t *chain_ring;
+    uint32_t *chain_done;
+    uint32_t chain_seq;
+    uint32_t chain_budget;
+    uint32_t chain_blocks;
+};
+constexpr uint32_t CHAIN_RING = 64;
 
 struct ReplicateParams {
     DevTable t;
diff --git a/rafting_amd/csrc/rg_step.hpp b/rafting_amd/csrc/rg_step.hpp
--- a/rafting_amd/csrc/rg_step.hpp
+++ b/rafting_amd/csrc/rg_step.hpp
@@ -415,6 +415,7 @@
 
 template <int F, bool EV32, int NO = 2>
 struct SplitLds {
+    static constexpr int CHAIN_WORDS = 24;
     static constexpr int EVF = EV32 ? (int)EV_D + 1 : (int)EV_FIELDS;
     static constexpr size_t W_EPOCH = 0, W_NEXT = W_EPOCH + F * BLOCK * 8, W_MATCH = W_NEXT + F * BLOCK * 8, W_REJ = W_MATCH + F * BLOCK * 8,
                             W_EV = W_REJ + F * BLOCK * 4, W_OUT = W_EV + 2 * EVF * BLOCK * 8, W_AUTO = W_OUT + 2 * OUT_FIELDS * BLOCK * 8,
@@ -425,7 +426,8 @@
                             N_O0 = N_EVQ + NEV * BLOCK * 16, N_O1 = N_O0 + NO * BLOCK * 16, N_BAIL = N_O1 + NO * BLOCK * 16,
                             N_LUTC = N_BAIL + 16, N_LUTM = N_LUTC + 256 * 4, N_LUTE = N_LUTM + 128 * 4,
                             N_BASE = N_LUTE + 128 * 2, N_LUTS = N_BASE + BLOCK * 8,
-                            N_END = N_LUTS + 64 * 4;
+                            N_CHAIN = N_LUTS + 64 * 4,
+                            N_END = N_CHAIN + CHAIN_WORDS * 4;
     static constexpr size_t BYTES = EV32 ? (W_END > N_END ? W_END : N_END) : W_END;
 };
 
@@ -610,6 +612,18 @@
 
 struct Row32 { U32x2 h; I32x4 q; };
 
+enum { CD_SEQ0 = 0, CD_ROUNDS, CD_HEAD, CD_ABCD = 4, CD_OUT = 6, CD_PERSIST = 8, CD_TERMS = 10, CD_ECOUNT = 12, CD_VERDICT = 13, CD_SEQ1 = 15, CD_WORDS = 16 };
+enum { CH_TAKE = CD_WORDS, CH_TERMS = CD_WORDS + 4, CH_ECOUNT = CD_WORDS + 6, CHAIN_LDS_WORDS = CD_WORDS + 8 };
+enum { TAKE_GO = 1, TAKE_STOP = 2 };
+__device__ __forceinline__ uint32_t uniform_word(const uint32_t *w) { const uint32_t v = *w; return __builtin_amdgcn_readfirstlane(v); }
+#ifndef RG_SYSTEM_LOAD
+#ifdef __HIP_MEMORY_SCOPE_SYSTEM
+#define RG_SYSTEM_LOAD(p) __hip_atomic_load((p), __ATOMIC_RELAXED, __HIP_MEMORY_SCOPE_SYSTEM)
+#else
+#define RG_SYSTEM_LOAD(p) (*(p))
+#endif
+#endif
+
 constexpr int CW_AUXC = 18;
 template <int F = 0>
 __device__ __forceinline__ uint32_t class_entry(const StepParams &p, uint32_t idx)
@@ -667,13 +681,17 @@
     uint32_t *sh_lutc = reinterpret_cast<uint32_t *>(smem + L::N_LUTC), *sh_lutm = reinterpret_cast<uint32_t *>(smem + L::N_LUTM);
     uint16_t *sh_lute = reinterpret_cast<uint16_t *>(smem + L::N_LUTE);
     uint32_t *sh_luts = reinterpret_cast<uint32_t *>(smem + L::N_LUTS);
+    constexpr bool CHAIN = !SPARSE && IOW == 1 && RPB == 1 && F <= 6;
+    constexpr bool IO_CHAIN = CHAIN && OUT32;
+    static_assert(L::CHAIN_WORDS == (int)CHAIN_LDS_WORDS, "LDS of the chain words");
+    uint32_t *sh_chain = reinterpret_cast<uint32_t *>(smem + L::N_CHAIN);
 
     const uint32_t lane = threadIdx.x & (BLOCK - 1);
     const bool io_wave = __builtin_amdgcn_readfirstlane(threadIdx.x) >= (uint32_t)BLOCK;
     const uint32_t i = blockIdx.x * BLOCK + lane;
     const bool active = i < p.count;
     const uint32_t ir = active ? i : p.count - 1u;
-    const uint32_t last_round = p.rounds - 1u;
+    uint32_t rounds = p.rounds, last_round = rounds - 1u, seq = (io_wave ? IO_CHAIN : CHAIN) ? p.chain_seq : 0u;
 
     if (io_wave) {
         RG_HWID_BEGIN(1);
@@ -689,7 +707,7 @@
         int64_t io_base = 0;
         if constexpr (!OUT32) io_base = (p.has_bases != 0) ? p.t.ibase[SPARSE ? p.gid[ir] : ir] : 0;
         auto fetch = [&](uint32_t r, Row32 &x) {
-            const uint64_t rb = (uint64_t)(r < p.rounds ? r : last_round) * round_rows;
+            const uint64_t rb = (uint64_t)(r < rounds ? r : last_round) * round_rows;
             x.h = nt_load_at<U32x2>(b_head + rb * 8u, irm);
             x.q = nt_load_at<I32x4>(b_q + rb * 16u, irm);
         };
@@ -730,8 +748,14 @@
             }
             tally.add_packed_lut(RG_HDR_KIND(hdr), flags, status, sh_luts);
         };
+        uint32_t desc = 0u, used = 0u;
+        auto look = [&]() {
+            desc = RG_SYSTEM_LOAD(reinterpret_cast<const RG_GLOBAL_AS uint32_t *>(reinterpret_cast<uint64_t>(p.chain_ring)) + (((seq + 1u) & (CHAIN_RING - 1u)) * (uint32_t)CD_WORDS + (lane & 15u)));
+        };
         Row32 buf[4];
+        for (;;) {
         uint32_t hdr_m1 = 0u, hdr_0, hdr_1;
+        if constexpr (IO_CHAIN) { if (seq != 0u && rounds <= 8u) look(); }
         if (do_pub) {
             Row32 e0, e1;
             fetch(0, e0); fetch(1, e1); fetch(2, buf[2]); fetch(3, buf[3]); fetch(4, buf[0]); fetch(5, buf[1]);
@@ -742,18 +766,22 @@
             for (int k = 0; k < 4; k++) { buf[k].h = U32x2{0u, 0u}; buf[k].q = I32x4{0, 0, 0, 0}; }
         }
         lds_barrier();
-        { const uint32_t seen0 = *sh_bail; if (__builtin_amdgcn_readfirstlane(seen0) == 1u) return false; }
+        {
+            const uint32_t seen0 = *sh_bail, take = sh_chain[CH_TAKE];
+            if (seq != 0u && __builtin_amdgcn_readfirstlane(take) == (uint32_t)TAKE_STOP) return true;
+            if (__builtin_amdgcn_readfirstlane(seen0) == 1u) return false;
+        }
         bool bailed = false;
         uint32_t seen = 0u;
         RG_PROBE_BEGIN();
         if constexpr (RPB == 2) {
             uint32_t hk[4] = {hdr_0, hdr_1, 0u, 0u};
-            for (uint32_t r0 = 0; r0 < p.rounds && !bailed; r0 += 4u) {
+            for (uint32_t r0 = 0; r0 < rounds && !bailed; r0 += 4u) {
                 if ((r0 & 127u) == 124u) tally.spill();
 #pragma unroll
                 for (int k = 0; k < 4; k++) {
                     const uint32_t r = r0 + (uint32_t)k;
-                    if (r >= p.rounds) break;
+                    if (r >= rounds) break;
                     Row32 &x = buf[(k + 2) & 3];
                     publish((r + 2u) & 3u, x);
                     RG_PROBE_MARK(0);
@@ -772,7 +800,7 @@
             }
             if (bailed) return false;
             { const uint32_t mark = __builtin_amdgcn_readfirstlane(seen); if (mark != 0u) return false; }
-            for (uint32_t q = p.rounds >= 2u ? p.rounds - 2u : 0u; q < p.rounds; q++) {
+            for (uint32_t q = rounds >= 2u ? rounds - 2u : 0u; q < rounds; q++) {
                 const uint32_t i = q & 3u;
                 retire(q, i == 0u ? hk[0] : (i == 1u ? hk[1] : (i == 2u ? hk[2] : hk[3])));
             }
@@ -786,12 +814,26 @@
 #endif
             return true;
         }
-        for (uint32_t r0 = 0; r0 < p.rounds && !bailed; r0 += 4u) {
+        for (uint32_t r0 = 0; r0 < rounds && !bailed; r0 += 4u) {
             if ((r0 & 127u) == 124u) tally.spill();
+            if constexpr (IO_CHAIN) {
+                if (seq != 0u && r0 + 12u >= rounds) {
+                    if (r0 + 8u < rounds) look();
+                    if (r0 + 4u >= rounds) {
+                        if (lane < (uint32_t)CD_WORDS) sh_chain[lane] = desc;
+                        __builtin_amdgcn_wave_barrier();
+                        const uint32_t s0 = uniform_word(sh_chain + CD_SEQ0), s1 = uniform_word(sh_chain + CD_SEQ1),
+                                       nr = uniform_word(sh_chain + CD_ROUNDS);
+                        const bool go = (s0 == seq + 1u) & (s1 == seq + 1u) & (nr - 1u < p.chain_budget) & (used + rounds + nr <= p.chain_budget) &
+                                        (seq + 1u - p.chain_seq < CHAIN_RING);
+                        if (lane == 0u) sh_chain[CD_VERDICT] = go ? 1u : 0u;
+                    }
+                }
+            }
 #pragma unroll
             for (int k = 0; k < 4; k++) {
                 const uint32_t r = r0 + (uint32_t)k;
-                if (r >= p.rounds) break;
+                if (r >= rounds) break;
                 Row32 &x = buf[(k + 2) & 3];
                 if (do_pub) publish((r + 2u) & 3u, x);
                 RG_PROBE_MARK(0);
@@ -810,8 +852,8 @@
                 seen = *sh_bail;
             }
         }
-        if (bailed) return false;
-        { const uint32_t mark = __builtin_amdgcn_readfirstlane(seen); if (mark != 0u) return false; }
+        if (bailed) return used != 0u;
+        { const uint32_t mark = __builtin_amdgcn_readfirstlane(seen); if (mark != 0u) return used != 0u; }
         if constexpr (IOW == 1) retire(last_round, hdr_m1);
         else if (do_ret) retire(last_round, (uint32_t)sh_evh[last_round & 3u][lane].w);
         tally.spill();
@@ -822,7 +864,18 @@
 #else
         if (do_ret) tally.flush(p, lane, active);
 #endif
-        return true;
+        if constexpr (!IO_CHAIN) return true;
+        else {
+            if (seq == 0u || uniform_word(sh_chain + CD_VERDICT) == 0u) return true;
+            auto word = [&](int k) { return (uint64_t)uniform_word(sh_chain + k); };
+            b_head = word(CD_HEAD) | (word(CD_HEAD + 1) << 32); b_q = word(CD_ABCD) | (word(CD_ABCD + 1) << 32);
+            b_reply = word(CD_OUT) | (word(CD_OUT + 1) << 32); b_persist = word(CD_PERSIST) | (word(CD_PERSIST + 1) << 32);
+            used += rounds;
+            rounds = (uint32_t)word(CD_ROUNDS); last_round = rounds - 1u;
+            seq += 1u;
+            tally = Tally{};
+        }
+        }
     }
 
     __builtin_amdgcn_s_setprio(3);
@@ -834,6 +887,8 @@
     pe.rec = sh_rec + lane; pe.mv = sh_mv + lane * 4; pe.overflow = false; pe.base = 0;
     const bool FAST = p.fast_paths != 0;
     bool in_domain, any_base;
+    uint32_t done_word = 0u;
+    if (seq != 0u) done_word = p.chain_done[(size_t)(seq & (CHAIN_RING - 1u)) * p.chain_blocks + blockIdx.x];
     {
         const int64_t base = (p.has_bases != 0) ? p.t.ibase[gi] : 0;
         any_base = __builtin_amdgcn_ballot_w64(base != 0) != 0;
@@ -850,14 +905,18 @@
         in_domain = in_domain & stage_peers<F>(p.t, gi, g64.prepared, pe);
     }
     bool bailed = __builtin_amdgcn_ballot_w64(!in_domain) != 0;
-    if (lane == 0) *sh_bail = bailed ? 1u : 0u;
+    bool stop = seq != 0u && __builtin_amdgcn_readfirstlane(done_word) == seq;
+    if (lane == 0) {
+        *sh_bail = bailed ? 1u : 0u;
+        sh_chain[CH_TAKE] = stop ? (uint32_t)TAKE_STOP : (uint32_t)TAKE_GO;
+        sh_chain[CH_TAKE + 1] = seq;
+        sh_chain[CH_TERMS] = 0u; sh_chain[CH_TERMS + 1] = 0u; sh_chain[CH_ECOUNT] = p.entry_terms32 != nullptr ? (uint32_t)p.entry_count : 0u;
+    }
     bool blocked = false;
     int32_t flush_max = 0;
-    lds_barrier();
-    if (bailed) return false;
     RG_PROBE_BEGIN();
 #ifdef RG_EVENT_PREFETCH
-    I32x4 h_next = sh_evh[0][lane], q_next = sh_evq[0][lane];
+    I32x4 h_next, q_next;
 #endif
     auto round = [&](const uint32_t r) {
 #ifdef RG_EVENT_PREFETCH
@@ -888,10 +947,17 @@
                 pe.base = base;
                 Group g64 = group_to_abs(widen(g), base);
                 Stepper<F, PeersNarrow<F>> st(p, g64, pe);
-                const Entries en = entries_of<true>(p, hdr, aux, 0, 0, 0, 0);
+                Entries en = entries_of<true>(p, hdr, aux, 0, 0, 0, 0);
+                uint64_t ecount = p.entry_count;
+                if constexpr (CHAIN) {
+                    const int64_t off = (int64_t)((uint64_t)sh_chain[CH_TERMS] | ((uint64_t)sh_chain[CH_TERMS + 1] << 32));
+                    ecount = sh_chain[CH_ECOUNT];
+                    en.t32 = ecount != 0u ? reinterpret_cast<const int32_t *>(reinterpret_cast<const char *>(p.entry_terms32) + off) + aux : nullptr;
+                }
                 const uint32_t ix = index_fields(kind);
                 st.run(hdr, aux, (ix & 1u) ? to_abs(q.x, base) : (int64_t)q.x, (ix & 2u) ? to_abs(q.y, base) : (int64_t)q.y,
-                       (ix & 4u) ? to_abs(q.z, base) : (int64_t)q.z, (ix & 8u) ? to_abs(q.w, base) : (int64_t)q.w, false, 0, 0, en, entries_readable(p, en, aux, RG_HDR_N(hdr)));
+                       (ix & 4u) ? to_abs(q.z, base) : (int64_t)q.z, (ix & 8u) ? to_abs(q.w, base) : (int64_t)q.w, false, 0, 0, en,
+                       en.same | ((en.t32 != nullptr) & ((uint64_t)aux + RG_HDR_N(hdr) <= ecount)));
                 g64 = group_to_rel(g64, base);
                 st.fx.log_from = to_rel(st.fx.log_from, base);
                 bail = !fits32(g64, STATE_LIMIT) | !small_fields_fit(g64) | pe.overflow | ((base != 0) & (g64.epoch_index <= 0)) |
@@ -922,8 +988,15 @@
             RG_PROBE_MARK(3);
         }
     };
+    for (;;) {
+    lds_barrier();
+    if (stop) return true;
+    if (bailed) return false;
+#ifdef RG_EVENT_PREFETCH
+    h_next = sh_evh[0][lane]; q_next = sh_evq[0][lane];
+#endif
     if constexpr (RPB == 2) {
-        for (uint32_t r = 0; r < p.rounds; r++) {
+        for (uint32_t r = 0; r < rounds; r++) {
             round(r);
             if (bailed) break;
             if ((r & 1u) != 0u || r == last_round) {
@@ -934,34 +1007,71 @@
         if (bailed) lds_barrier();
     } else {
 #ifdef RG_EVENT_PREFETCH
-    { uint32_t r = 0; do { round(r); r++; } while (!bailed & (r < p.rounds)); }
+    { uint32_t r = 0; do { round(r); r++; } while (!bailed & (r < rounds)); }
 #else
-    for (uint32_t r = 0; r < p.rounds; r++) {
+    for (uint32_t r = 0; r < rounds; r++) {
         round(r);
         if (bailed) break;
     }
 #endif
     }
-    if (bailed) return false;
+    if constexpr (CHAIN) seq = uniform_word(sh_chain + CH_TAKE + 1);
+    if (bailed) return seq != (CHAIN ? p.chain_seq : 0u);
     RG_PROBE_FLUSH(4);
     RG_HWID_END(0);
-    if (active) {
-        Group g64 = widen(g);
-        pe.base = 0;
-        if (any_base) {
-            const int64_t base = *sh_base;
-            pe.base = base;
-            g64 = group_to_abs(g64, base);
-        }
-        uint32_t gi_out = gi;
-        RG_FRESH_VGPR(gi_out);
-        store_group(p.t, gi_out, g64, pe, F);
-        if (p.auto_window != 0) {
-            const int64_t base = *sh_base;
-            advance_base(p, gi_out, base, to_abs(flush_max, base));
-        }
-    }
-    return true;
+    uint32_t gi_out = gi;
+    RG_FRESH_VGPR(gi_out);
+    if (!CHAIN || seq == 0u) {
+        if (active) {
+            Group g64 = widen(g);
+            pe.base = 0;
+            if (any_base) {
+                const int64_t base = *sh_base;
+                pe.base = base;
+                g64 = group_to_abs(g64, base);
+            }
+            store_group(p.t, gi_out, g64, pe, F);
+            if (p.auto_window != 0) {
+                const int64_t base = *sh_base;
+                advance_base(p, gi_out, base, to_abs(flush_max, base));
+            }
+        }
+        return true;
+    }
+    if constexpr (CHAIN) {
+        if (active) {
+            pe.base = 0;
+            store_group(p.t, gi_out, widen(g), pe, F);
+        }
+        if (seq != p.chain_seq && lane == 0u) {
+            p.chain_done[(size_t)(seq & (CHAIN_RING - 1u)) * p.chain_blocks + blockIdx.x] = seq;
+            p.chain_done[(size_t)CHAIN_RING * p.chain_blocks + blockIdx.x] += 1u;
+        }
+        if (uniform_word(sh_chain + CD_VERDICT) == 0u) return true;
+        g.log_dirty = 0; g.peers_dirty = 0;
+        g.s1 = g.rc > 1 ? g.s1 : 0; g.s2 = g.rc > 2 ? g.s2 : 0; g.s3 = g.rc > 3 ? g.s3 : 0;
+        uint32_t w = (uint32_t)g.term | (uint32_t)g.commit | (uint32_t)g.epoch_index | (uint32_t)g.epoch_term | (uint32_t)g.first | (uint32_t)g.last | (uint32_t)g.elected_term |
+                     (uint32_t)g.s0 | (uint32_t)g.s1 | (uint32_t)g.s2 | (uint32_t)g.s3 | (uint32_t)g.t0 | (uint32_t)g.t1 | (uint32_t)g.t2 | (uint32_t)g.t3 |
+                     g.role_epoch | g.elected_epoch | (uint32_t)g.votes | (uint32_t)(g.leader + 1) | (uint32_t)(g.voted_for + 1);
+        if (g.prepared < 0) {
+#pragma unroll
+            for (int j = 0; j < F; j++) { const I32x4 rec = pe.rec[j * BLOCK]; w |= (uint32_t)rec.x | (uint32_t)rec.y | (uint32_t)rec.z; }
+        }
+        const bool fits = (w < EV_LIMIT) & ((uint32_t)g.role <= (uint32_t)RG_LEADER) & !pe.overflow;
+        stop = __builtin_amdgcn_ballot_w64(!fits) != 0;
+        seq += 1u;
+        rounds = uniform_word(sh_chain + CD_ROUNDS);
+        blocked = false; flush_max = 0; pe.overflow = false;
+        g.nallow = FAST ? 0 : -1;
+        g.recache();
+        if (lane == 0u) {
+            sh_chain[CH_TAKE] = stop ? (uint32_t)TAKE_STOP : (uint32_t)TAKE_GO;
+            sh_chain[CH_TAKE + 1] = seq;
+            const uint64_t terms = (uint64_t)sh_chain[CD_TERMS] | ((uint64_t)sh_chain[CD_TERMS + 1] << 32), off = terms - reinterpret_cast<uint64_t>(p.entry_terms32);
+            sh_chain[CH_TERMS] = (uint32_t)off; sh_chain[CH_TERMS + 1] = (uint32_t)(off >> 32); sh_chain[CH_ECOUNT] = terms != 0u ? sh_chain[CD_ECOUNT] : 0u;
+        }
+    }
+    }
 }
 
 #ifndef RG_NOTE_FALLBACK
diff --git a/rafting_amd/engine.py b/rafting_amd/engine.py
--- a/rafting_amd/engine.py
+++ b/rafting_amd/engine.py
@@ -27,7 +27,7 @@
         "rg_dev_free", "rg_copy_to_device", "rg_copy_to_host", "rg_stream", "rg_replicate", "rg_timers_configure", "rg_timers_update",
         "rg_timers_expired", "rg_timers_expired_epochs", "rg_timers_arm", "rg_timers_read", "rg_health_update", "rg_health_failure", "rg_ready", "rg_health_read", "rg_in_flight_read", "rg_in_flight_set",
         "rg_timing_enable",
-        "rg_timing_read", "rg_timing_begin", "rg_timing_end", "rg_counters_read", "rg_wide_body_workgroups", "rg_copy_bandwidth",
+        "rg_timing_read", "rg_timing_begin", "rg_timing_end", "rg_counters_read", "rg_wide_body_workgroups", "rg_chain_info", "rg_copy_bandwidth",
     ]
 
 
@@ -152,6 +152,7 @@
         L.rg_timing_end.argtypes = [vp, C.POINTER(C.c_double)]
         L.rg_counters_read.argtypes = [vp, C.POINTER(C.c_uint64), i32]
         L.rg_wide_body_workgroups.argtypes = [vp, C.POINTER(C.c_uint64), i32]
+        L.rg_chain_info.argtypes = [vp, C.POINTER(C.c_uint64), i32]
         L.rg_copy_bandwidth.argtypes = [vp, C.c_size_t, i32, C.POINTER(C.c_double)]
         if L.rg_abi_version() != abi.ABI_VERSION:
             raise EngineError("libraftgpu.so ABI %d != binding ABI %d" % (L.rg_abi_version(), abi.ABI_VERSION))
@@ -931,6 +932,11 @@
         self._check(lib().rg_counters_read(self._h, arr, int(reset)))
         return list(arr)
 
+    def chain_info(self, reset=False):
+        n = C.c_uint64()
+        self._check(lib().rg_chain_info(self._h, C.byref(n), int(reset)))
+        return n.value
+
     def wide_body_workgroups(self, reset=False):
         n = C.c_uint64()
         self._check(lib().rg_wide_body_workgroups(self._h, C.byref(n), int(reset)))
```

New measurement: 25.11 billion. 0.397x the previous value.
